# WasifurRahman/BERT_multimodal_transformer

Measured on AMD Instinct MI355X. Metric: train samples/sec MAG-BERT MOSI seq_len=50, higher is better.
Workload: dtype bf16; 1 GPU; MAG-BERT bert-base-uncased, MOSI dims (V=47, A=74), batch 48/GPU, seq_len 50, full optimizer step (fwd+MSE+bwd+HF-AdamW+schedule+zero_grad; inputs resident in HBM), dropout on, random-init weights; global_batch=48, seq_len=50, parallelism=dp1, step_call=mb_bert_train_step, hipGraph replay

## Files before the change

bert_multimodal_transformer_amd/_lib.py:

```python
import ctypes as C
import os

_HERE = os.path.dirname(os.path.abspath(__file__))
LIB_PATH = os.path.join(os.environ.get("MB_LIB_DIR") or os.path.join(_HERE, "lib"), "libmagbert_hip.so")

DT_F32, DT_BF16 = 0, 1
GEMM_NT, GEMM_NN, GEMM_TN = 0, 1, 2
EPI_BIAS, EPI_BIAS_GELU, EPI_BIAS_DROP_RES, EPI_ADD_RES, EPI_DGELU, EPI_ACCUM_F32, EPI_BIAS_F32 = range(7)
EPI_BIAS_RELU, EPI_BIAS_SWISH, EPI_BIAS_GELU_NEW, EPI_BIAS_MISH = 7, 8, 9, 10
ACT_GELU, ACT_RELU, ACT_SWISH, ACT_GELU_NEW, ACT_MISH = range(5)
ACTIVATIONS = {"gelu": ACT_GELU, "relu": ACT_RELU, "swish": ACT_SWISH, "silu": ACT_SWISH, "gelu_new": ACT_GELU_NEW, "mish": ACT_MISH}
ACT_EPILOGUE = {ACT_GELU: EPI_BIAS_GELU, ACT_RELU: EPI_BIAS_RELU, ACT_SWISH: EPI_BIAS_SWISH, ACT_GELU_NEW: EPI_BIAS_GELU_NEW,
                ACT_MISH: EPI_BIAS_MISH}


def activation_code(name, field):
    if isinstance(name, str) and name in ACTIVATIONS:
        return ACTIVATIONS[name]
    raise NotImplementedError("%s=%r: the feed-forward activations built are %s (and silu = swish)"
                              % (field, name, ", ".join(n for n in ACTIVATIONS if n != "silu")))


class DropKey(C.Structure):
    _fields_ = [("k0", C.c_uint32), ("k1", C.c_uint32), ("thresh", C.c_uint32), ("scale", C.c_float)]


class BertEngineConfig(C.Structure):
    _fields_ = [("vocab_size", C.c_int), ("hidden_size", C.c_int), ("num_layers", C.c_int), ("num_heads", C.c_int),
                ("intermediate_size", C.c_int), ("max_position", C.c_int), ("type_vocab", C.c_int),
                ("num_labels", C.c_int), ("visual_dim", C.c_int), ("acoustic_dim", C.c_int), ("pad_token_id", C.c_int),
                ("layer_norm_eps", C.c_float), ("mag_layer_norm_eps", C.c_float), ("beta_shift", C.c_float),
                ("hidden_dropout", C.c_float), ("attn_dropout", C.c_float), ("mag_dropout", C.c_float),
                ("dtype", C.c_int), ("max_batch", C.c_int), ("max_seq", C.c_int), ("injection_index", C.c_int),
                ("hidden_act", C.c_int)]
    POSITIONAL = tuple(n for n, _ in _fields_ if n != "injection_index") + ("injection_index",)

    def __init__(self, *args, **kw):
        if len(args) > len(self.POSITIONAL):
            raise TypeError("too many initializers")
        super().__init__()
        for name, value in zip(self.POSITIONAL, args):
            setattr(self, name, value)
        for name, value in kw.items():
            if name not in self.POSITIONAL:
                raise TypeError("BertEngineConfig has no field %r" % name)
            setattr(self, name, value)


class XlnetEngineConfig(C.Structure):
    _fields_ = [("vocab_size", C.c_int), ("d_model", C.c_int), ("n_layer", C.c_int), ("n_head", C.c_int), ("d_inner", C.c_int),
                ("num_labels", C.c_int), ("visual_dim", C.c_int), ("acoustic_dim", C.c_int), ("injection_index", C.c_int),
                ("layer_norm_eps", C.c_float), ("mag_layer_norm_eps", C.c_float), ("beta_shift", C.c_float),
                ("dropout", C.c_float), ("summary_last_dropout", C.c_float), ("mag_dropout", C.c_float),
                ("dtype", C.c_int), ("max_batch", C.c_int), ("max_seq", C.c_int), ("ff_activation", C.c_int)]


_vp, _i, _f, _sz, _u64, _u32 = C.c_void_p, C.c_int, C.c_float, C.c_size_t, C.c_uint64, C.c_uint32
_dk = C.POINTER(DropKey)

PROTOTYPES = {
    "mb_error_string": (C.c_char_p, [_i]),
    "mb_version": (_i, []),
    "mb_make_dropkey": (None, [_u64, _u64, _u32, _f, _dk]),
    "mb_gemm": (_i, [_i, _i, _i, _i, _i, _i, _vp, _i, _vp, _i, _vp, _i, _vp, _vp, _vp, _vp, _i, _f, _dk, _i, _i, _vp]),
    "mb_gemm_grouped_wgrad": (_i, [_i, _i, _vp, _vp, _i, _vp, _vp, _vp, _vp, _vp, _vp, _i, _vp]),
    "mb_narrow": (_i, [_i, _vp, _vp, _sz, _vp]),
    "mb_widen": (_i, [_i, _vp, _vp, _sz, _vp]),
    "mb_layernorm_forward": (_i, [_i, _vp, _vp, _vp, _f, _vp, _vp, _vp, _i, _i, _dk, _vp]),
    "mb_layernorm_backward": (_i, [_i, _vp, _vp, _vp, _vp, _vp, _vp, _vp, _vp, _vp, _vp, _i, _i, _dk, _dk, _vp]),
    "mb_embed_forward": (_i, [_i, _vp, _vp, _vp, _vp, _vp, _vp, _vp, _f, _vp, _vp, _vp, _i, _i, _i, _dk, _vp]),
    "mb_embed_backward": (_i, [_i, _vp, _vp, _vp, _vp, _vp, _vp, _vp, _vp, _vp, _vp, _vp, _vp, _vp, _vp, _vp, _i, _i, _i,
                               _i, _dk, _vp]),
    "mb_attention_forward": (_i, [_i, _vp, _vp, _vp, _i, _i, _i, _dk, _vp]),
    "mb_attention_backward": (_i, [_i, _vp, _vp, _vp, _vp, _i, _i, _i, _dk, _vp]),
    "mb_attention_resident_forward": (_i, [_i, _vp, _vp, _vp, _i, _i, _i, _dk, _vp, _vp, _vp]),
    "mb_attention_resident_backward": (_i, [_i, _vp, _vp, _vp, _vp, _vp, _i, _i, _i, _dk, _vp, _vp]),
    "mb_attention_tiled_stats_bytes": (_sz, [_i, _i, _i]),
    "mb_attention_tiled_forward": (_i, [_i, _vp, _vp, _vp, _vp, _i, _i, _i, _dk, _vp, _vp, _vp]),
    "mb_attention_tiled_backward": (_i, [_i, _vp, _vp, _vp, _vp, _vp, _vp, _vp, _i, _i, _i, _dk, _vp, _vp]),
    "mb_mag_workspace_bytes": (_sz, [_i, _i, _i, _i, _i]),
    "mb_mag_forward": (_i, [_i] + [_vp] * 13 + [_f, _dk, _vp, _vp, _i, _i, _i, _i, _vp]),
    "mb_mag_backward": (_i, [_i] + [_vp] * 11 + [_f, _dk] + [_vp] * 14 + [_i, _i, _i, _i, _vp]),
    "mb_adamw_step": (_i, [_vp, _vp, _vp, _vp, _vp, _sz, _sz, _sz, _sz, _f, _f, _f, _f, _f, _i, _i, _f, _i, _vp]),
    "mb_bert_create": (_i, [C.POINTER(BertEngineConfig), C.POINTER(_vp)]),
    "mb_bert_destroy": (None, [_vp]),
    "mb_bert_num_tensors": (_i, [_vp]),
    "mb_bert_tensor_info": (_i, [_vp, _i, C.c_char_p, _i, C.POINTER(_sz), C.POINTER(_sz), C.POINTER(_i),
                                 C.POINTER(C.c_int64), C.POINTER(_i)]),
    "mb_bert_param_count": (_sz, [_vp]),
    "mb_bert_decay_count": (_sz, [_vp]),
    "mb_bert_shadow_range": (None, [_vp, C.POINTER(_sz), C.POINTER(_sz)]),
    "mb_bert_workspace_bytes": (_sz, [_vp]),
    "mb_bert_bind": (_i, [_vp, _vp, _vp, _vp, _vp, _sz]),
    "mb_bert_sync_weights": (_i, [_vp, _vp]),
    "mb_bert_forward": (_i, [_vp, _vp, _vp, _vp, _vp, _vp, _vp, _i, _i, _i, _u64, _u64, _vp, _vp, _vp, _vp]),
    "mb_bert_backward": (_i, [_vp, _vp, _vp, _f, _i, _i, _vp]),
    "mb_bert_sequence_output": (_vp, [_vp]),
    "mb_bert_pooled_output": (_vp, [_vp]),
    "mb_bert_hidden_state": (_vp, [_vp, _i]),
    "mb_bert_set_attention_output": (_i, [_vp, _vp]),
    "mb_debug_gemm_ex": (_i, [_i, _i, _i, _i, _i, _i, _vp, _i, _vp, _i, _vp, _i, _vp, _vp, _vp, _vp, _i, _f, _dk, _i, _i,
                              _i, _sz, _i, _i, _vp, _i, _vp, _vp, _vp, _vp, _vp, _sz, _i, _i, _f, _f, _f, _f, _f, _i, _i, _f, _vp,
                              C.POINTER(_i), _vp]),
    "mb_debug_gemm_grouped_ex": (_i, [_i, _i, _vp, _vp, _i, _vp, _vp, _vp, _vp, _vp, _vp, _vp, _vp, _i, _i, _vp, _vp, _vp, _vp, _vp,
                                      _sz, _i, _i, _f, _f, _f, _f, _f, _i, _i, _f, _vp, _vp]),
    "mb_debug_gemm_last_kernel": (_i, [C.c_char_p, _i]),
    "mb_debug_gemm_trace": (_i, [_vp, _i]),
    "mb_debug_attention_trace": (_i, [_vp, _i]),
    "mb_xlnet_attention_probs": (_vp, [_vp, _i, C.POINTER(_i)]),
    "mb_xlnet_attention_probs_into": (_i, [_vp, _i, _vp, _vp]),
    "mb_xlnet_attention_tiled_stats_bytes": (_sz, [_i, _i, _i]),
    "mb_xlnet_attention_tiled_scratch_bytes": (_sz, [_i, _i, _i, _i]),
    "mb_xlnet_attention_tiled_forward": (_i, [_i] + [_vp] * 10 + [_i, _i, _i, _dk, _vp, _vp, _i, _vp, _vp]),
    "mb_xlnet_attention_tiled_backward": (_i, [_i] + [_vp] * 19 + [_i, _i, _i, _dk, _vp, _vp, _vp]),
    "mb_xlnet_attention_forward": (_i, [_i] + [_vp] * 11 + [_i, _i, _i, _dk, _vp, _vp, _i, _vp]),
    "mb_xlnet_attention_backward": (_i, [_i] + [_vp] * 20 + [_i, _i, _i, _dk, _vp, _vp, _vp]),
    "mb_xlnet_set_head_mask": (_i, [_vp, _vp]),
    "mb_xlnet_set_perm_mask": (_i, [_vp, _vp]),
    "mb_xlnet_set_mems": (_i, [_vp, _vp, _i]),
    "mb_xlnet_query_stream_scratch_bytes": (_sz, [_vp, _i, _i, _i]),
    "mb_xlnet_query_stream_state_bytes": (_sz, [_vp, _i, _i]),
    "mb_xlnet_query_stream": (_i, [_vp, _vp, _i, _vp, _sz, _vp, _vp]),
    "mb_bert_mark_grads_zero": (_i, [_vp, _i]),
    "mb_xlnet_mark_grads_zero": (_i, [_vp, _i]),
    "mb_bert_distrust_word_stamps": (_i, [_vp]),
    "mb_bert_word_skip_updates": (_sz, [_vp]),
    "mb_bert_materialize_grads": (_i, [_vp, _vp]),
    "mb_xlnet_materialize_grads": (_i, [_vp, _vp]),
    "mb_bert_grads_stale": (_i, [_vp]),
    "mb_xlnet_grads_stale": (_i, [_vp]),
    "mb_bert_set_head_mask": (_i, [_vp, _vp]),
    "mb_bert_set_inputs_embeds": (_i, [_vp, _vp]),
    "mb_bert_set_position_ids": (_i, [_vp, _vp]),
    "mb_bert_inputs_embeds_grad": (_vp, [_vp]),
    "mb_bert_backward_outputs": (_i, [_vp, _vp, _vp, _vp]),
    "mb_bert_stage_grad_ranges": (_i, [_vp, _i, C.POINTER(_sz), C.POINTER(_sz), _i]),
    "mb_bert_train_step": (_i, [_vp, _vp, _vp, _vp, _vp, _vp, _vp, _i, _i, _u64, _u64, _vp, _vp, _vp, _vp, _vp, _f, _f, _f, _f, _f,
                                _i, _i, _f, _f, _i, _vp]),
    "mb_bert_stage_forward": (_i, [_vp, _vp, _vp, _vp, _vp, _vp, _vp, _i, _i, _u64, _u64, _vp, _vp, _vp, _i, _vp]),
    "mb_bert_stage_backward": (_i, [_vp, _f, _i, _i, _vp]),
    "mb_bert_staged_input_ids": (_vp, [_vp]),
    "mb_bert_load_batch": (_i, [_vp, _vp, _vp, _vp, _vp, _vp, _vp, _i, _i, C.POINTER(_vp), _vp]),
    "mb_bert_graph_stats": (_i, [_vp, C.POINTER(_sz), C.POINTER(_sz)]),
    "mb_bert_set_profiling": (_i, [_vp, _i]),
    "mb_bert_profile_wgrad_us": (_i, [_vp, C.POINTER(_f)]),
    "mb_bert_profile_adamw_us": (_i, [_vp, C.POINTER(_f)]),
    "mb_xlnet_set_inputs_embeds": (_i, [_vp, _vp]),
    "mb_xlnet_inputs_embeds_grad": (_vp, [_vp]),
    "mb_xlnet_model_output": (_vp, [_vp, _vp]),
    "mb_xlnet_backward_outputs": (_i, [_vp, _vp, _vp]),
    "mb_xlnet_set_profiling": (_i, [_vp, _i]),
    "mb_xlnet_profile_wgrad_us": (_i, [_vp, C.POINTER(_f)]),
    "mb_xlnet_profile_adamw_us": (_i, [_vp, C.POINTER(_f)]),
    "mb_xlnet_create": (_i, [C.POINTER(XlnetEngineConfig), C.POINTER(_vp)]),
    "mb_xlnet_destroy": (None, [_vp]),
    "mb_xlnet_num_tensors": (_i, [_vp]),
    "mb_xlnet_tensor_info": (_i, [_vp, _i, C.c_char_p, _i, C.POINTER(_sz), C.POINTER(_sz), C.POINTER(_i),
                                  C.POINTER(C.c_int64), C.POINTER(_i)]),
    "mb_xlnet_param_count": (_sz, [_vp]),
    "mb_xlnet_decay_count": (_sz, [_vp]),
    "mb_xlnet_shadow_range": (None, [_vp, C.POINTER(_sz), C.POINTER(_sz)]),
    "mb_xlnet_workspace_bytes": (_sz, [_vp]),
    "mb_xlnet_bind": (_i, [_vp, _vp, _vp, _vp, _vp, _sz]),
    "mb_xlnet_sync_weights": (_i, [_vp, _vp]),
    "mb_xlnet_forward": (_i, [_vp, _vp, _vp, _vp, _vp, _vp, _vp, _i, _i, _i, _u64, _u64, _vp, _vp, _vp, _vp]),
    "mb_xlnet_backward": (_i, [_vp, _vp, _vp, _f, _i, _i, _vp]),
    "mb_xlnet_sequence_output": (_vp, [_vp]),
    "mb_xlnet_hidden_state": (_vp, [_vp, _i]),
    "mb_xlnet_train_step": (_i, [_vp, _vp, _vp, _vp, _vp, _vp, _vp, _i, _i, _u64, _u64, _vp, _vp, _vp, _vp, _vp, _f, _f, _f, _f, _f,
                                 _i, _i, _f, _f, _i, _vp]),
    "mb_xlnet_load_batch": (_i, [_vp, _vp, _vp, _vp, _vp, _vp, _vp, _i, _i, C.POINTER(_vp), _vp]),
    "mb_xlnet_graph_stats": (_i, [_vp, C.POINTER(_sz), C.POINTER(_sz)]),
    "mb_xlnet_trainable_count": (_sz, [_vp]),
    "mb_bert_set_update_map": (_i, [_vp, _i, _i, _vp, _vp]),
    "mb_bert_set_update_decay": (_i, [_vp, _i, _vp]),
    "mb_bert_set_update_values": (_i, [_vp, _i, _vp, _vp, _vp, _vp, _vp, _vp]),
    "mb_bert_update_stats": (_i, [_vp, C.POINTER(_sz), C.POINTER(_sz), C.POINTER(_i)]),
    "mb_bert_set_update_frozen": (_i, [_vp, _i, _vp]),
    "mb_bert_freeze_stats": (_i, [_vp, C.POINTER(_sz), C.POINTER(_i), C.POINTER(_i)]),
    "mb_xlnet_set_update_frozen": (_i, [_vp, _i, _vp]),
    "mb_xlnet_freeze_stats": (_i, [_vp, C.POINTER(_sz), C.POINTER(_i), C.POINTER(_i)]),
    "mb_xlnet_set_update_map": (_i, [_vp, _i, _i, _vp, _vp]),
    "mb_xlnet_set_update_decay": (_i, [_vp, _i, _vp]),
    "mb_xlnet_set_update_values": (_i, [_vp, _i, _vp, _vp, _vp, _vp, _vp, _vp]),
    "mb_xlnet_update_stats": (_i, [_vp, C.POINTER(_sz), C.POINTER(_sz), C.POINTER(_i)]),
    "mb_grad_clip_scratch_bytes": (_sz, [_sz]),
    "mb_grad_clip_coef": (_i, [_vp, _sz, _f, _f, _vp, _vp, _vp]),
    "mb_bert_set_grad_clip": (_i, [_vp, _f]),
    "mb_bert_grad_clip_stats": (_i, [_vp, C.POINTER(_f), C.POINTER(_f), _vp]),
    "mb_xlnet_set_grad_clip": (_i, [_vp, _f]),
    "mb_xlnet_grad_clip_stats": (_i, [_vp, C.POINTER(_f), C.POINTER(_f), _vp]),
    "mb_xlnet_stage_grad_ranges": (_i, [_vp, _i, C.POINTER(_sz), C.POINTER(_sz), _i]),
    "mb_comm_unique_id": (_i, [_vp]),
    "mb_comm_create_rccl": (_i, [_vp, _i, _i, C.POINTER(_vp)]),
    "mb_comm_create_callbacks": (_i, [_i, _i, _vp, _vp, _vp, C.POINTER(_vp)]),
    "mb_comm_destroy": (None, [_vp]),
    "mb_comm_rank": (_i, [_vp]),
    "mb_comm_world": (_i, [_vp]),
    "mb_comm_stream": (_vp, [_vp]),
    "mb_comm_scratch_bytes": (_sz, [_i, _i, _sz, _i, _i, _i]),
    "mb_comm_bind_scratch": (_i, [_vp, _vp, _sz, _i, _sz, _i, _i, _i]),
    "mb_comm_all_reduce": (_i, [_vp, _vp, _sz, _vp]),
    "mb_comm_exchange_rows": (_i, [_vp, _vp, _vp, _i, _vp]),
    "mb_comm_set_row_exchange": (_i, [_vp, _i]),
    "mb_comm_set_sharding": (_i, [_vp, _i]),
    "mb_comm_sharding": (_i, [_vp]),
    "mb_comm_join": (_i, [_vp, _vp]),
    "mb_comm_gather_shards": (_i, [_vp, _vp, _i, _vp]),
    "mb_comm_shard_slices": (_i, [_vp, C.POINTER(_sz), _i]),
    "mb_comm_set_timing": (_i, [_vp, _i]),
    "mb_comm_exposed_ms": (_i, [_vp, C.POINTER(_f)]),
    "mb_comm_stats": (_i, [_vp, C.POINTER(_sz), C.POINTER(_sz)]),
    "mb_comm_last_error": (C.c_char_p, []),
    "mb_bert_train_step_dp": (_i, [_vp, _vp, _vp, _vp, _vp, _vp, _vp, _i, _i, _u64, _u64, _vp, _vp, _vp, _vp, _vp, _f, _f, _f, _f, _f,
                                   _i, _i, _f, _f, _i, _vp, _vp]),
    "mb_xlnet_train_step_dp": (_i, [_vp, _vp, _vp, _vp, _vp, _vp, _vp, _i, _i, _u64, _u64, _vp, _vp, _vp, _vp, _vp, _f, _f, _f, _f, _f,
                                    _i, _i, _f, _f, _i, _vp, _vp]),
}

ALL_REDUCE_CB = C.CFUNCTYPE(C.c_int, C.c_void_p, C.c_void_p, C.c_size_t, C.c_int, C.c_void_p)
ALL_GATHER_CB = C.CFUNCTYPE(C.c_int, C.c_void_p, C.c_void_p, C.c_size_t, C.c_void_p)

_lib = None


class MagbertError(RuntimeError):
    pass


def lib():
    global _lib
    if _lib is None:
        if not os.path.exists(LIB_PATH):
            raise MagbertError(
                "libmagbert_hip.so not found at %s -- build it with `python -c 'import __graft_entry__ as g; g.build()'` "
                "(hipcc --offload-arch=gfx950).  There is no CPU fallback." % LIB_PATH)
        h = C.CDLL(LIB_PATH)
        for name, (res, args) in PROTOTYPES.items():
            fn = getattr(h, name)
            fn.restype = res
            fn.argtypes = args
        _lib = h
    return _lib


def check(code):
    if code != 0:
        msg = lib().mb_error_string(code).decode()
        if code == 1005 or 2000 <= code < 2100:
            msg += ": " + (lib().mb_comm_last_error() or b"").decode()
        raise MagbertError("%s (code %d)" % (msg, code))


def ptr(t):
    return None if t is None else C.c_void_p(t.data_ptr())


def make_dropkey(seed, step, site, p):
    k = DropKey()
    lib().mb_make_dropkey(int(seed) & (2**64 - 1), int(step), int(site), float(p), C.byref(k))
    return k


def no_drop():
    return DropKey(0, 0, 0, 1.0)
```

bert_multimodal_transformer_amd/csrc/engine.hip:

```cpp
#include "dp_step.h"

struct LayerOff { size_t wqkv, wo, w1, w2, bqkv, bo, ln1w, ln1b, b1, b2, ln2w, ln2b; };
struct LayerWs { size_t qkv, ctx, s1, st1, y1, u, g, s2, st2, stats; };

struct mb_bert_engine : StepMixin {
    mb_bert_config c;
    std::vector<TensorInfo> tensors;
    std::vector<LayerOff> lo;
    size_t word, pos, type, emb_lnw, emb_lnb, wp, bp, wc, bc;
    size_t mag_whv, mag_wha, mag_wv, mag_wa, mag_bhv, mag_bha, mag_bv, mag_ba, mag_lnw, mag_lnb;
    size_t n_params, n_decay, sh_begin, sh_end;
    size_t n_update_end() const { return n_params; }
    int n_layers() const { return c.num_layers; }
    size_t layer_begin(int l) const { return lo[l].wqkv; }
    size_t layers_end() const { return wp; }
    int width() const { return c.hidden_size; }
    size_t layer_end(int l) const { return l + 1 < c.num_layers ? lo[l + 1].wqkv : wp; }
    bool embed_all_frozen() const { return range_frozen(word, mag_whv) && range_frozen(emb_lnw, bp); }
    WordSkip word_skip(char* w) const {
        if (!(stamp_off != 0 && stamp_enable && idcnt_enable)) return {};
        return WordSkip{stamp_table(w), stamp_state(w), word, word + (size_t)c.vocab_size * c.hidden_size, (uint32_t)c.hidden_size};
    }
    MagWs mw;
    size_t ws_mag, ws_emb, ws_emb_st, ws_head_z, ws_head_pooled, ws_logits;
    std::vector<size_t> ws_x;
    size_t ws_pre = 0;
    int mag_nblk = 0;
    std::vector<LayerWs> lw;
    size_t ws_ds[2], ws_dzd[2], ws_ds2[2], ws_dzd2[2], ws_du[2], ws_dqkv[2];
    size_t ws_dxa, ws_dxb, ws_dctx, ws_dsum, ws_dz, ws_lnp_a, ws_lnp_b;
    size_t lnp_stride = 0;
    int lnp_nblk = 0;
    size_t ws_ids, ws_seg, ws_mask, ws_labels;
    size_t ws_bytes;
    float* P = nullptr; float* G = nullptr; char* SH = nullptr; char* ws = nullptr;
    const int64_t* ids = nullptr; const int64_t* seg = nullptr; const int64_t* mask = nullptr;
    int B = 0, L = 0, training = 0;
    int padT = -1;
    int prefetch = 1;
    int pf_qkv = 0;
    RideOpts ride_opts;
    int ride_blocks = 0;
    float* ride_m = nullptr; float* ride_v = nullptr;
    size_t ride_cursor = 0;
    long ride_params = 0;
    int group_wgrad = 256;
    bool grouped = false;
    float* attn_out = nullptr;
    const float* head_mask = nullptr;
    const float* emb_in = nullptr;
    const int64_t* pos_ids = nullptr;
    bool ran_forward = false;

    bool ws_zeroed = false;
    uint64_t seed = 0, step = 0;
    float* logits = nullptr;

    size_t add(const std::string& name, std::vector<int64_t> shape, int decay, size_t& cursor) {
        TensorInfo t;
        t.name = name; t.ndim = (int)shape.size(); t.decay = decay; t.numel = 1;
        for (int i = 0; i < 4; ++i) t.shape[i] = i < t.ndim ? shape[i] : 1;
        for (auto s : shape) t.numel *= (size_t)s;
        t.off = cursor;
        cursor = align_up(cursor + t.numel, 64);
        tensors.push_back(t);
        return t.off;
    }
    const void* W(size_t off) const {
        return c.dtype == DT_BF16 ? (const void*)(SH + off * 2) : (const void*)(P + off);
    }
    DropKey key(uint32_t site, float p) const { return step_key(ws, training != 0, seed, step, site, p); }
    float* attn_stats(const LayerWs& w) const { return c.max_seq > 128 ? (float*)(ws + w.stats) : nullptr; }
};

static void build_layout(mb_bert_engine* e) {
    const mb_bert_config& c = e->c;
    const int64_t H = c.hidden_size, I = c.intermediate_size, V = c.visual_dim, A = c.acoustic_dim;
    size_t cur = 0;
    e->lo.resize(c.num_layers);
    char buf[128];
    auto nm = [&](int l, const char* s) { snprintf(buf, sizeof buf, "bert.encoder.layer.%d.%s", l, s); return std::string(buf); };
    e->sh_begin = 0;
    for (int l = 0; l < c.num_layers; ++l) {
        LayerOff& o = e->lo[l];
        o.wqkv = e->add(nm(l, "attention.self.query.weight"), {H, H}, 1, cur);
        e->add(nm(l, "attention.self.key.weight"), {H, H}, 1, cur);
        e->add(nm(l, "attention.self.value.weight"), {H, H}, 1, cur);
        o.wo = e->add(nm(l, "attention.output.dense.weight"), {H, H}, 1, cur);
        o.w1 = e->add(nm(l, "intermediate.dense.weight"), {I, H}, 1, cur);
        o.w2 = e->add(nm(l, "output.dense.weight"), {H, I}, 1, cur);
    }
    e->wp = e->add("bert.pooler.dense.weight", {H, H}, 1, cur);
    e->sh_end = cur;
    e->word = e->add("bert.embeddings.word_embeddings.weight", {c.vocab_size, H}, 1, cur);
    e->pos = e->add("bert.embeddings.position_embeddings.weight", {c.max_position, H}, 1, cur);
    e->type = e->add("bert.embeddings.token_type_embeddings.weight", {c.type_vocab, H}, 1, cur);
    e->mag_whv = e->add("bert.MAG.W_hv.weight", {H, V + H}, 1, cur);
    e->mag_wha = e->add("bert.MAG.W_ha.weight", {H, A + H}, 1, cur);
    e->mag_wv = e->add("bert.MAG.W_v.weight", {H, V}, 1, cur);
    e->mag_wa = e->add("bert.MAG.W_a.weight", {H, A}, 1, cur);
    e->wc = e->add("classifier.weight", {c.num_labels, H}, 1, cur);
    e->n_decay = cur;
    for (int l = 0; l < c.num_layers; ++l) {
        LayerOff& o = e->lo[l];
        o.bqkv = e->add(nm(l, "attention.self.query.bias"), {H}, 0, cur);
        e->add(nm(l, "attention.self.key.bias"), {H}, 0, cur);
        e->add(nm(l, "attention.self.value.bias"), {H}, 0, cur);
        o.bo = e->add(nm(l, "attention.output.dense.bias"), {H}, 0, cur);
        o.ln1w = e->add(nm(l, "attention.output.LayerNorm.weight"), {H}, 0, cur);
        o.ln1b = e->add(nm(l, "attention.output.LayerNorm.bias"), {H}, 0, cur);
        o.b1 = e->add(nm(l, "intermediate.dense.bias"), {I}, 0, cur);
        o.b2 = e->add(nm(l, "output.dense.bias"), {H}, 0, cur);
        o.ln2w = e->add(nm(l, "output.LayerNorm.weight"), {H}, 0, cur);
        o.ln2b = e->add(nm(l, "output.LayerNorm.bias"), {H}, 0, cur);
    }
    e->emb_lnw = e->add("bert.embeddings.LayerNorm.weight", {H}, 0, cur);
    e->emb_lnb = e->add("bert.embeddings.LayerNorm.bias", {H}, 0, cur);
    e->bp = e->add("bert.pooler.dense.bias", {H}, 0, cur);
    e->mag_bhv = e->add("bert.MAG.W_hv.bias", {H}, 0, cur);
    e->mag_bha = e->add("bert.MAG.W_ha.bias", {H}, 0, cur);
    e->mag_bv = e->add("bert.MAG.W_v.bias", {H}, 0, cur);
    e->mag_ba = e->add("bert.MAG.W_a.bias", {H}, 0, cur);
    e->mag_lnw = e->add("bert.MAG.LayerNorm.weight", {H}, 0, cur);
    e->mag_lnb = e->add("bert.MAG.LayerNorm.bias", {H}, 0, cur);
    e->bc = e->add("classifier.bias", {c.num_labels}, 0, cur);
    e->n_params = cur;

    const size_t es = esize(c.dtype);
    const size_t T = align_up((size_t)c.max_batch * c.max_seq, 64);
    Carver w;
    e->mw.init(c.dtype, (int)T, (int)H, (int)V, (int)A);
    e->ws_mag = w.take(e->mw.bytes);
    e->pk_vis = e->ws_mag + e->mw.vp; e->pk_aco = e->ws_mag + e->mw.ap; e->pk_Vp = e->mw.Vp; e->pk_Ap = e->mw.Ap; e->pk_dtype = c.dtype;
    e->ws_emb = w.take(T * H * es);
    e->ws_emb_st = w.take(2 * T * 4);
    e->ws_x.resize(c.num_layers + 1);
    for (int l = 0; l <= c.num_layers; ++l) e->ws_x[l] = w.take(T * H * es);
    e->ws_pre = c.injection_index >= 1 ? w.take(T * H * es) : 0;
    e->lw.resize(c.num_layers);
    for (int l = 0; l < c.num_layers; ++l) {
        LayerWs& x = e->lw[l];
        x.qkv = w.take(T * 3 * H * es); x.ctx = w.take(T * H * es); x.s1 = w.take(T * H * es); x.st1 = w.take(2 * T * 4);
        x.y1 = w.take(T * H * es); x.u = w.take(T * I * es); x.g = w.take(T * I * es); x.s2 = w.take(T * H * es);
        x.st2 = w.take(2 * T * 4);
        x.stats = c.max_seq > 128 ? w.take(tiled_stats_floats(c.max_batch, c.max_seq, c.num_heads) * 4) : 0;
    }
    e->ws_head_z = w.take((size_t)c.max_batch * H * 4);
    e->ws_head_pooled = w.take((size_t)c.max_batch * H * 4);
    e->ws_logits = w.take((size_t)c.max_batch * c.num_labels * 4);
    e->ws_dxa = w.take(T * H * es); e->ws_dxb = w.take(T * H * es);
    for (int k = 0; k < 2; ++k) {
        e->ws_ds[k] = w.take(T * H * es); e->ws_dzd[k] = w.take(T * H * es); e->ws_ds2[k] = w.take(T * H * es);
        e->ws_dzd2[k] = w.take(T * H * es); e->ws_du[k] = w.take(T * I * es); e->ws_dqkv[k] = w.take(T * 3 * H * es);
    }
    e->ws_dctx = w.take(T * H * es); e->ws_dsum = w.take(T * H * 4); e->ws_dz = w.take((size_t)c.max_batch * H * es);
    e->lnp_stride = ln_partials_floats((int)T, (int)H);
    {
        const size_t emb = (size_t)c.max_seq * ((c.max_batch + 7) / 8) * 3 * H;
        if (emb > e->lnp_stride) e->lnp_stride = emb;
    }
    e->ws_lnp_a = w.take(e->lnp_stride * 4 * (c.num_layers + 2)); e->ws_lnp_b = w.take(e->lnp_stride * 4 * (c.num_layers + 2));
    e->carve_step(w, T, (int)V, (int)A, c.max_batch, c.num_labels, SITE_LAYER0 + 4 * c.num_layers);
    e->idcnt_off = w.take((size_t)c.vocab_size * 4);
    e->idcnt_enable = env_on("MB_EMBED_UNIQUE", true);
    e->stamp_rows = (size_t)c.vocab_size;
    e->stamp_off = w.take(((size_t)c.vocab_size + 2) * 4);
    e->stamp_enable = env_on("MB_ADAMW_SKIP_ZERO_ROWS", true);
    e->one_sweep = env_on("MB_ADAMW_ONE_SWEEP", true);
    if (e->deterministic) {
        e->det_begin = e->wp; e->det_end = e->n_params;
        e->ws_det = w.take((e->det_end - e->det_begin) * sizeof(long long));
    }
    e->ws_bytes = w.off;
}

static int prepare_pass(mb_bert_engine* e, int T, hipStream_t st) {
    const mb_bert_config& c = e->c;
    const int H = c.hidden_size, I = c.intermediate_size, dt = c.dtype;
    char* ws = e->ws;
    const int Tp = (int)align_up((size_t)T, 64);
    if (!e->ws_zeroed) { CK((int)hipMemsetAsync(ws, 0, e->ws_bytes, st)); e->ws_zeroed = true; e->padT = T; }
    if (e->padT != T && Tp > T) {
        const size_t es = esize(dt);
        auto zp = [&](size_t off, size_t cols) {
            return (int)hipMemsetAsync(ws + off + (size_t)T * cols * es, 0, (size_t)(Tp - T) * cols * es, st);
        };
        CK(zp(e->ws_emb, H));
        if (c.injection_index >= 1) CK(zp(e->ws_pre, H));
        CK(mag_clear_pad_rows(dt, ws + e->ws_mag, e->mw, T, H, st));
        for (int k = 0; k < 2; ++k) {
            CK(zp(e->ws_ds[k], H)); CK(zp(e->ws_dzd[k], H)); CK(zp(e->ws_ds2[k], H)); CK(zp(e->ws_dzd2[k], H));
            CK(zp(e->ws_du[k], I)); CK(zp(e->ws_dqkv[k], 3 * H));
        }
        for (int l = 0; l <= c.num_layers; ++l) CK(zp(e->ws_x[l], H));
        for (int l = 0; l < c.num_layers; ++l) { CK(zp(e->lw[l].ctx, H)); CK(zp(e->lw[l].y1, H)); CK(zp(e->lw[l].g, I)); }
    }
    e->padT = T;
    return MB_OK;
}

static AdamArgs adam_scalars(float lr, float beta1, float beta2, float eps, float weight_decay, int step, int correct_bias, float grad_scale) {
    AdamArgs a;
    a.lr = lr; a.beta1 = beta1; a.beta2 = beta2; a.eps = eps; a.weight_decay = weight_decay; a.grad_scale = grad_scale;
    double ss = lr;
    if (correct_bias) ss = (double)lr * sqrt(1.0 - pow((double)beta2, (double)step)) / (1.0 - pow((double)beta1, (double)step));
    a.step_size = (float)ss;
    return a;
}
static int debug_ride(AdamRide& r, float* p, float* g, float* m, float* v, void* shadow, size_t n4, int blocks, int zero_grad, const AdamArgs& a,
                      void* adam_dev, hipStream_t st) {
    r = AdamRide{};
    if (blocks == 0) return MB_OK;
    if (blocks < 0 || !p || !g || !m || !v || !adam_dev) return MB_ERR_ARG;
    if ((((uintptr_t)p | (uintptr_t)g | (uintptr_t)m | (uintptr_t)v) & 15) || ((uintptr_t)shadow & 7) || ((uintptr_t)adam_dev & 3)) return MB_ERR_SHAPE;
    CK((int)hipMemcpyAsync(adam_dev, &a, sizeof(AdamArgs), hipMemcpyHostToDevice, st));
    CK((int)hipStreamSynchronize(st));
    r.p = p; r.g = g; r.m = m; r.v = v; r.shadow = (bf16*)shadow; r.n4 = n4; r.dyn = (const AdamArgs*)adam_dev; r.blocks = blocks;
    r.zero_grad = zero_grad;
    return MB_OK;
}

extern "C" {

const char* mb_error_string(int code) {
    switch (code) {
        case MB_OK: return "ok";
        case MB_ERR_SHAPE: return "magbert: unsupported shape or alignment";
        case MB_ERR_MODE: return "magbert: unsupported layout/epilogue combination";
        case MB_ERR_DTYPE: return "magbert: unsupported dtype";
        case MB_ERR_ARG: return "magbert: invalid argument";
        case MB_ERR_COMM: return "magbert: gradient exchange unavailable (mb_comm_last_error())";
        default:
            if (code >= 2000 && code < 2100) return "magbert: RCCL call failed (mb_comm_last_error())"; return hipGetErrorString((hipError_t)code);
    }
}
int mb_version(void) { return 100; }

void mb_make_dropkey(uint64_t seed, uint64_t step, uint32_t site, float p, mb_dropkey* out) {
    DropKey k = make_key(seed, step, site, p);
    out->k0 = k.k0; out->k1 = k.k1; out->thresh = k.thresh; out->scale = k.scale;
}

static int abi_epilogue(int& epilogue, int layout, GemmArgs& a) {
    if (epilogue < MB_EPI_RELU || epilogue > MB_EPI_MISH) return MB_OK;
    if (layout != GEMM_NT) return MB_ERR_MODE;
    a.act = ACT_RELU + (epilogue - MB_EPI_RELU);
    epilogue = EPI_BIAS_ACT;
    return MB_OK;
}

int mb_gemm(int dtype, int layout, int epilogue, int M, int N, int K, const void* A, int lda, const void* B, int ldb,
            void* C, int ldc, void* C2, float* Cf, const float* bias, const void* R, int ldr, float alpha,
            const mb_dropkey* drop, int splits, int tile, void* stream) {
    GemmArgs a = {};
    a.A = A; a.B = B; a.M = M; a.N = N; a.K = K; a.lda = lda; a.ldb = ldb; a.C = C; a.ldc = ldc; a.C2 = C2; a.Cf = Cf;
    a.bias = bias; a.R = R; a.ldr = ldr; a.alpha = alpha; a.drop = dk(drop); a.kchunk = K; a.colsum = nullptr;
    if (epilogue == EPI_DGELU) { a.colsum = Cf; a.Cf = nullptr; }
    if (int e = abi_epilogue(epilogue, layout, a)) return e;
    return gemm_launch(dtype, layout, epilogue, a, splits, tile, (hipStream_t)stream);
}

int mb_debug_gemm_ex(int dtype, int layout, int epilogue, int M, int N, int K, const void* A, int lda, const void* B, int ldb,
                     void* C, int ldc, void* C2, float* Cf, const float* bias, const void* R, int ldr, float alpha,
                     const mb_dropkey* drop, int splits, int tile, int bseg, size_t bseg_stride, int cvalid, int overwrite,
                     long long* colsum_shadow, int fold, float* rp, float* rg, float* rm, float* rv, void* rshadow, size_t n4, int blocks,
                     int zero_grad, float lr, float beta1, float beta2, float eps, float weight_decay, int step, int correct_bias,
                     float grad_scale, void* adam_dev, int* ride_tiles, void* stream) {
    hipStream_t st = (hipStream_t)stream;
    GemmArgs a = {};
    a.A = A; a.B = B; a.M = M; a.N = N; a.K = K; a.lda = lda; a.ldb = ldb; a.C = C; a.ldc = ldc; a.C2 = C2; a.Cf = Cf;
    a.bias = bias; a.R = R; a.ldr = ldr; a.alpha = alpha; a.drop = dk(drop); a.kchunk = K; a.colsum = nullptr;
    if (epilogue == EPI_DGELU) { a.colsum = Cf; a.Cf = nullptr; }
    if (int e = abi_epilogue(epilogue, layout, a)) return e;
    a.bseg = bseg; a.bseg_stride = bseg_stride; a.cvalid = cvalid; a.overwrite = overwrite;
    if (colsum_shadow) {
        if (!a.colsum) return MB_ERR_ARG;
        a.acc = GradAcc{colsum_shadow, a.colsum};
    }
    if (ride_tiles) *ride_tiles = 0;
    AdamRide ride;
    if (int e = debug_ride(ride, rp, rg, rm, rv, rshadow, n4, blocks, zero_grad,
                           adam_scalars(lr, beta1, beta2, eps, weight_decay, step, correct_bias, grad_scale), adam_dev, st)) return e;
    if (ride.blocks > 0) {
        if (layout != GEMM_NN || splits > 1 || tile != 0) return MB_ERR_MODE;
        int per_cu = 0;
        const int tiles = gemm_nn_ride_tiles(dtype, epilogue, a, &per_cu);
        if (ride_tiles) *ride_tiles = tiles;
        CK(gemm_nn_ride_launch(dtype, epilogue, a, ride, st));
    } else {
        CK(gemm_launch(dtype, layout, epilogue, a, splits, tile, st));
    }
    if (colsum_shadow && fold) CK(grad_fold(a.acc, a.colsum, 0, (size_t)N, st));
    return MB_OK;
}

int mb_debug_gemm_grouped_ex(int dtype, int count, const int* M, const int* N, int K, const void* const* dY, const int* ldy,
                             const void* const* X, const int* ldx, float* const* dW, const int* ldw, const int* cvalid,
                             const int* overwrite, int tile, int stages, float* rp, float* rg, float* rm, float* rv, void* rshadow,
                             size_t n4, int blocks, int zero_grad, float lr, float beta1, float beta2, float eps, float weight_decay,
                             int step, int correct_bias, float grad_scale, void* adam_dev, void* stream) {
    hipStream_t st = (hipStream_t)stream;
    if (count < 1 || count > MB_MAX_GROUP || !M || !N || !dY || !X || !dW || !ldy || !ldx || !ldw) return MB_ERR_ARG;
    if (stages != 0 && stages != 4 && stages != 5) return MB_ERR_ARG;
    GemmArgs g[MB_MAX_GROUP];
    for (int i = 0; i < count; ++i) {
        g[i] = wgrad_args(M[i], N[i], K, dY[i], ldy[i], X[i], ldx[i], dW[i], ldw[i]);
        g[i].cvalid = cvalid ? cvalid[i] : 0;
        g[i].overwrite = overwrite ? overwrite[i] : 0;
    }
    if (!gemm_grouped_tn_ok(dtype, g, count, tile)) return MB_ERR_SHAPE;
    AdamRide ride;
    if (int e = debug_ride(ride, rp, rg, rm, rv, rshadow, n4, blocks, zero_grad,
                           adam_scalars(lr, beta1, beta2, eps, weight_decay, step, correct_bias, grad_scale), adam_dev, st)) return e;
    return gemm_grouped_tn_launch(dtype, g, count, tile, st, stages, ride.blocks > 0 ? &ride : nullptr);
}

int mb_debug_gemm_last_kernel(char* out, int cap) { return gemm_last_kernel(out, cap); }

int mb_debug_gemm_trace(unsigned long long* host_out, int max_blocks) { return gemm_trace_fetch(host_out, max_blocks); }
int mb_debug_attention_trace(unsigned long long* host_out, int max_blocks) { return attention_trace_fetch(host_out, max_blocks); }
int mb_gemm_grouped_wgrad(int dtype, int count, const int* M, const int* N, int K, const void* const* dY, const int* ldy,
                          const void* const* X, const int* ldx, float* const* dW, const int* ldw, int tile, void* stream) {
    if (count < 1 || count > MB_MAX_GROUP || !M || !N || !dY || !X || !dW || !ldy || !ldx || !ldw) return MB_ERR_ARG;
    GemmArgs g[MB_MAX_GROUP];
    for (int i = 0; i < count; ++i) g[i] = wgrad_args(M[i], N[i], K, dY[i], ldy[i], X[i], ldx[i], dW[i], ldw[i]);
    if (!gemm_grouped_tn_ok(dtype, g, count, tile)) return MB_ERR_SHAPE;
    return gemm_grouped_tn_launch(dtype, g, count, tile, (hipStream_t)stream);
}

int mb_narrow(int dtype, const float* src, void* dst, size_t n, void* stream) {
    if (!src || !dst) return MB_ERR_ARG;
    if (n % 4) return MB_ERR_SHAPE;
    return convert(dtype, src, dst, n, (hipStream_t)stream);
}
int mb_widen(int dtype, const void* src, float* dst, size_t n, void* stream) {
    if (!src || !dst) return MB_ERR_ARG;
    return widen(dtype, src, dst, n, (hipStream_t)stream);
}

int mb_layernorm_forward(int dtype, const void* x, const float* gamma, const float* beta, float eps, void* y, float* mean,
                         float* rstd, int rows, int H, const mb_dropkey* drop, void* stream) {
    return ln_forward(dtype, x, gamma, beta, eps, y, mean, rstd, rows, H, dk(drop), (hipStream_t)stream);
}
int mb_layernorm_backward(int dtype, const void* dy, const void* x, const float* gamma, const float* mean,
                          const float* rstd, void* dx, void* dx_drop, float* dgamma, float* dbeta, float* dbias, int rows,
                          int H, const mb_dropkey* drop_out, const mb_dropkey* drop_in, void* stream) {
    return ln_backward(dtype, dy, x, gamma, mean, rstd, dx, dx_drop, dgamma, dbeta, dbias, rows, H, dk(drop_out),
                       dk(drop_in), (hipStream_t)stream);
}
int mb_embed_forward(int dtype, const int64_t* ids, const int64_t* seg, const float* word, const float* pos,
                     const float* type, const float* gamma, const float* beta, float eps, void* out, float* mean,
                     float* rstd, int B, int L, int H, const mb_dropkey* drop, void* stream) {
    return embed_ln_forward(dtype, ids, seg, word, pos, type, gamma, beta, eps, out, mean, rstd, B, L, H, dk(drop),
                            (hipStream_t)stream);
}
int mb_embed_backward(int dtype, const void* dout, const int64_t* ids, const int64_t* seg, const float* word,
                      const float* pos, const float* type, const float* gamma, const float* mean, const float* rstd,
                      float* dsum_ws, float* dword, float* dpos, float* dtype_, float* dgamma, float* dbeta, int B, int L,
                      int H, int pad_id, const mb_dropkey* drop, void* stream) {
    return embed_ln_backward(dtype, dout, ids, seg, word, pos, type, gamma, mean, rstd, dsum_ws, dword, dpos, dtype_,
                             dgamma, dbeta, B, L, H, pad_id, dk(drop), (hipStream_t)stream);
}
int mb_attention_forward(int dtype, const void* qkv, const int64_t* mask, void* ctx, int B, int L, int nh,
                         const mb_dropkey* drop, void* stream) {
    if (L > 128) return MB_ERR_SHAPE;
    return attention_forward(dtype, qkv, mask, ctx, B, L, nh, dk(drop), (hipStream_t)stream);
}
int mb_attention_backward(int dtype, const void* qkv, const int64_t* mask, const void* dctx, void* dqkv, int B, int L,
                          int nh, const mb_dropkey* drop, void* stream) {
    static float* trace_dbias = nullptr;
    static int trace_on = -1;
    if (trace_on < 0) {
        const char* v = getenv("MB_ATTN_TRACE");
        trace_on = v ? atoi(v) : 0;
        if (trace_on && (hipMalloc(&trace_dbias, (size_t)3 * 64 * 64 * sizeof(float)) != hipSuccess ||
                         hipMemset(trace_dbias, 0, (size_t)3 * 64 * 64 * sizeof(float)) != hipSuccess)) trace_dbias = nullptr;
    }
    if (L > 128) return MB_ERR_SHAPE;
    return attention_backward(dtype, qkv, mask, nullptr, dctx, dqkv, (trace_on && nh <= 64) ? trace_dbias : nullptr, B, L, nh, dk(drop),
                              (hipStream_t)stream);
}
static int resident_check(int dtype, int B, int L, int nh, const DropKey& drop) {
    if (B < 1 || L < 1 || L > 128 || nh < 1 || (int64_t)B * nh > 0x7fffffff) return MB_ERR_SHAPE;
    if (drop.thresh != 0u && (uint64_t)B * nh * L * L >= ((uint64_t)1 << 32)) return MB_ERR_SHAPE;
    if (dtype != DT_BF16 && dtype != DT_F32) return MB_ERR_DTYPE;
    return MB_OK;
}
int mb_attention_resident_forward(int dtype, const void* qkv, const int64_t* mask, void* ctx, int B, int L, int nh,
                                  const mb_dropkey* drop, const float* head_scale, float* probs, void* stream) {
    if (int e = resident_check(dtype, B, L, nh, dk(drop))) return e;
    if (!qkv || !mask || !ctx) return MB_ERR_ARG;
    return attention_forward(dtype, qkv, mask, ctx, B, L, nh, dk(drop), (hipStream_t)stream, probs, head_scale);
}
int mb_attention_resident_backward(int dtype, const void* qkv, const int64_t* mask, const void* dctx, void* dqkv, float* dbias, int B,
                                   int L, int nh, const mb_dropkey* drop, const float* head_scale, void* stream) {
    if (int e = resident_check(dtype, B, L, nh, dk(drop))) return e;
    if (!qkv || !mask || !dctx || !dqkv) return MB_ERR_ARG;
    return attention_backward(dtype, qkv, mask, nullptr, dctx, dqkv, dbias, B, L, nh, dk(drop), (hipStream_t)stream, head_scale);
}
size_t mb_attention_tiled_stats_bytes(int B, int L, int nh) {
    return (B < 1 || L < 1 || nh < 1) ? 0 : tiled_stats_floats(B, L, nh) * sizeof(float);
}
int mb_attention_tiled_forward(int dtype, const void* qkv, const int64_t* mask, void* ctx, float* stats, int B, int L, int nh,
                               const mb_dropkey* drop, const float* head_scale, float* probs, void* stream) {
    return attention_tiled_forward(dtype, qkv, mask, ctx, stats, B, L, nh, dk(drop), (hipStream_t)stream, probs, head_scale);
}
int mb_attention_tiled_backward(int dtype, const void* qkv, const int64_t* mask, const void* ctx, const void* dctx, float* stats,
                                void* dqkv, float* dbias, int B, int L, int nh, const mb_dropkey* drop, const float* head_scale,
                                void* stream) {
    return attention_tiled_backward(dtype, qkv, mask, ctx, dctx, stats, dqkv, dbias, B, L, nh, dk(drop), (hipStream_t)stream, head_scale);
}

size_t mb_mag_workspace_bytes(int dtype, int T, int H, int V, int A) {
    MagWs w;
    w.init(dtype, T, H, V, A);
    return w.bytes;
}
int mb_mag_forward(int dtype, const void* text, const float* visual, const float* acoustic, const float* W_hv,
                   const float* b_hv, const float* W_ha, const float* b_ha, const float* W_v, const float* b_v,
                   const float* W_a, const float* b_a, const float* ln_w, const float* ln_b, float beta_shift,
                   const mb_dropkey* drop, void* out, void* ws, int T, int H, int V, int A, void* stream) {
    if (H % 256 || H < 256 || H > 1024 || V < 1 || A < 1) return MB_ERR_SHAPE;
    MagWs w;
    w.init(dtype, T, H, V, A);
    return mag_fwd_impl(dtype, text, visual, acoustic, W_hv, b_hv, W_ha, b_ha, W_v, b_v, W_a, b_a, ln_w, ln_b, 1e-5f,
                        beta_shift, dk(drop), out, (char*)ws, w, T, H, V, A, true, (hipStream_t)stream);
}
int mb_mag_backward(int dtype, const void* d_out, const void* text, const float* W_hv, const float* b_hv,
                    const float* W_ha, const float* b_ha, const float* W_v, const float* b_v, const float* W_a,
                    const float* b_a, const float* ln_w, float beta_shift, const mb_dropkey* drop, void* ws, void* d_text,
                    float* d_visual, float* d_acoustic, float* dW_hv, float* db_hv, float* dW_ha, float* db_ha,
                    float* dW_v, float* db_v, float* dW_a, float* db_a, float* dln_w, float* dln_b, int T, int H, int V,
                    int A, void* stream) {
    (void)W_hv; (void)W_ha; (void)W_v; (void)W_a;
    if (H % 256 || H < 256 || H > 1024) return MB_ERR_SHAPE;
    MagWs w;
    w.init(dtype, T, H, V, A);
    return mag_bwd_impl(dtype, d_out, text, b_hv, b_ha, b_v, b_a, ln_w, beta_shift, dk(drop), (char*)ws, w, d_text,
                        d_visual, d_acoustic, dW_hv, db_hv, dW_ha, db_ha, dW_v, db_v, dW_a, db_a, dln_w, dln_b, T, H, V, A,
                        false, (hipStream_t)stream);
}

int mb_adamw_step(float* p, float* g, float* m, float* v, void* shadow, size_t n, size_t n_decay, size_t sh_begin,
                  size_t sh_end, float lr, float beta1, float beta2, float eps, float weight_decay, int step,
                  int correct_bias, float grad_scale, int zero_grad, void* stream) {
    const AdamArgs a = adam_scalars(lr, beta1, beta2, eps, weight_decay, step, correct_bias, grad_scale);
    return adamw_step(p, g, m, v, shadow, n, n_decay, sh_begin, sh_end, a, zero_grad, (hipStream_t)stream);
}

size_t mb_grad_clip_scratch_bytes(size_t n) { return (size_t)grad_norm_blocks(n) * sizeof(double); }
int mb_grad_clip_coef(const float* g, size_t n, float max_norm, float grad_scale, void* scratch, float* out2, void* stream) {
    if (!scratch || !out2) return MB_ERR_ARG;
    CK(grad_sumsq(g, n, (double*)scratch, (hipStream_t)stream));
    return grad_clip_finalize((const double*)scratch, grad_norm_blocks(n), nullptr, max_norm, grad_scale, out2, ClipTables{}, (hipStream_t)stream);
}

int mb_bert_create(const mb_bert_config* cfg, mb_bert_engine** out) {
    if (!cfg || !out) return MB_ERR_ARG;
    const int Hc = cfg->hidden_size;
    if ((Hc != 256 && Hc != 512 && Hc != 768 && Hc != 1024) || cfg->num_heads * 64 != Hc || cfg->num_layers < 1) return MB_ERR_SHAPE;
    if (cfg->intermediate_size % 128 || cfg->max_seq < 1 || cfg->max_seq > 512 || cfg->max_batch < 1) return MB_ERR_SHAPE;
    if (cfg->max_seq > cfg->max_position || cfg->num_labels < 1) return MB_ERR_SHAPE;
    if (cfg->dtype != DT_F32 && cfg->dtype != DT_BF16) return MB_ERR_DTYPE;
    if (cfg->hidden_act < ACT_GELU || cfg->hidden_act > ACT_MISH) return MB_ERR_ARG;
    if (cfg->injection_index < 0 || cfg->injection_index >= cfg->num_layers) return MB_ERR_ARG;
    mb_bert_engine* e = new mb_bert_engine();
    e->c = *cfg;
    e->read_env();
    e->ride_opts.read_env();
    e->group_wgrad = env_int("MB_GROUP_WGRAD", e->group_wgrad);
    e->ride_blocks = env_int("MB_ADAMW_RIDE_BLOCKS", e->ride_blocks);
    e->ride_params = env_long("MB_ADAMW_RIDE_PARAMS", e->ride_params);
    e->prefetch = env_int("MB_PREFETCH", e->prefetch);
    e->pf_qkv = env_int("MB_PF_QKV", e->pf_qkv);
    if (e->group_wgrad == 256 && (cfg->dtype != DT_BF16 || cfg->hidden_size % 256 != 0 || cfg->intermediate_size % 256 != 0)) e->group_wgrad = 128;
    e->grouped = (e->group_wgrad == 64 || e->group_wgrad == 128 || e->group_wgrad == 256) && cfg->hidden_size % e->group_wgrad == 0 &&
                 cfg->intermediate_size % e->group_wgrad == 0;

    build_layout(e);
    e->ow_covers = e->grouped;
    e->stale_begin = e->lo[0].wqkv; e->stale_end = e->wp;
    *out = e;
    return MB_OK;
}
void mb_bert_destroy(mb_bert_engine* e) {
    if (!e) return;
    e->destroy_prof();
    e->drop_graphs();
    e->free_class_table();
    e->free_clip_buf();
    delete e;
}
int mb_bert_num_tensors(const mb_bert_engine* e) { return (int)e->tensors.size(); }
int mb_bert_tensor_info(const mb_bert_engine* e, int i, char* name, int name_cap, size_t* offset, size_t* numel, int* ndim,
                        int64_t* shape4, int* decay) {
    if (i < 0 || i >= (int)e->tensors.size()) return MB_ERR_ARG;
    const TensorInfo& t = e->tensors[i];
    if (name && name_cap > 0) { strncpy(name, t.name.c_str(), name_cap - 1); name[name_cap - 1] = 0; }
    if (offset) *offset = t.off;
    if (numel) *numel = t.numel;
    if (ndim) *ndim = t.ndim;
    if (shape4) for (int k = 0; k < 4; ++k) shape4[k] = t.shape[k];
    if (decay) *decay = t.decay;
    return MB_OK;
}
size_t mb_bert_param_count(const mb_bert_engine* e) { return e->n_params; }
size_t mb_bert_decay_count(const mb_bert_engine* e) { return e->n_decay; }
void mb_bert_shadow_range(const mb_bert_engine* e, size_t* b, size_t* en) { *b = e->sh_begin; *en = e->sh_end; }
size_t mb_bert_workspace_bytes(const mb_bert_engine* e) { return e->ws_bytes; }

int mb_bert_bind(mb_bert_engine* e, float* params, float* grads, void* shadow, void* workspace, size_t ws_bytes) {
    if (!params || !workspace || ws_bytes < e->ws_bytes) return MB_ERR_ARG;
    if (e->c.dtype == DT_BF16 && !shadow) return MB_ERR_ARG;
    e->P = params; e->G = grads; e->SH = (char*)shadow; e->ws = (char*)workspace;
    e->grads_zero = false;
    e->frz_dirty = true;
    e->stamp_live = e->word_zero = false; e->sweep_no = 1;
    e->ws_zeroed = false; e->padT = -1;
    e->drop_graphs();
    char* mws = e->ws + e->ws_mag;
    e->pkw = {e->P + e->mag_whv, e->P + e->mag_wha, e->P + e->mag_wv, e->P + e->mag_wa, mws + e->mw.We, mws + e->mw.Wv, mws + e->mw.Wa,
              MagDims{0, e->c.hidden_size, e->c.visual_dim, e->c.acoustic_dim, e->mw.Vp, e->mw.Ap}, e->c.dtype};
    return MB_OK;
}

int mb_bert_sync_weights(mb_bert_engine* e, void* stream) {
    hipStream_t st = (hipStream_t)stream;
    if (!e->P) return MB_ERR_ARG;
    if (e->c.dtype == DT_BF16)
        CK(convert(DT_BF16, e->P + e->sh_begin, e->SH + e->sh_begin * 2, e->sh_end - e->sh_begin, st));
    const mb_bert_config& c = e->c;
    MagDims d = {0, c.hidden_size, c.visual_dim, c.acoustic_dim, e->mw.Vp, e->mw.Ap};
    char* mws = e->ws + e->ws_mag;
    CK(mag_pack_weights(c.dtype, e->P + e->mag_whv, e->P + e->mag_wha, e->P + e->mag_wv, e->P + e->mag_wa, mws + e->mw.We,
                        mws + e->mw.Wv, mws + e->mw.Wa, d, st));
    return MB_OK;
}

static int bert_forward_range(mb_bert_engine* e, const int64_t* input_ids, const float* visual, const float* acoustic,
                              const int64_t* attention_mask, const int64_t* token_type_ids, const float* labels, int B, int L,
                              int training, uint64_t seed, uint64_t step, float* logits, float* loss, float* loss_run, void* stream,
                              int l0, int l1, bool first, bool last) {
    hipStream_t st = (hipStream_t)stream;
    const mb_bert_config& c = e->c;
    if (!e->P || !e->ws) return MB_ERR_ARG;
    if (B < 1 || B > c.max_batch || L < 1 || L > c.max_seq) return MB_ERR_SHAPE;
    if ((!input_ids && !e->emb_in) || !visual || !acoustic || !attention_mask || !token_type_ids || !logits) return MB_ERR_ARG;
    const int dt = c.dtype, H = c.hidden_size, I = c.intermediate_size, T = B * L, nh = c.num_heads;
    if (e->emb_in) input_ids = nullptr;
    e->ids = input_ids; e->seg = token_type_ids; e->mask = attention_mask; e->ran_forward = true;
    e->B = B; e->L = L; e->training = training; e->seed = seed; e->step = step; e->logits = logits;
    float* P = e->P;
    char* ws = e->ws;
    if (first && !e->capturing) CK(prepare_pass(e, T, st));
    const int inj = c.injection_index;
    if (first) CK(embed_ln_forward(dt, input_ids, token_type_ids, e->emb_in ? e->emb_in : P + e->word, P + e->pos, P + e->type, P + e->emb_lnw, P + e->emb_lnb,
                        c.layer_norm_eps, ws + (inj >= 1 ? e->ws_x[0] : e->ws_emb), (float*)(ws + e->ws_emb_st), (float*)(ws + e->ws_emb_st) + T, B, L,
                        H, e->key(SITE_EMB, c.hidden_dropout), st, e->pos_ids));
    auto mag = [&](const char* text, char* out) -> int {
        return mag_fwd_impl(dt, text, visual, acoustic, P + e->mag_whv, P + e->mag_bhv, P + e->mag_wha, P + e->mag_bha,
                            P + e->mag_wv, P + e->mag_bv, P + e->mag_wa, P + e->mag_ba, P + e->mag_lnw, P + e->mag_lnb,
                            c.mag_layer_norm_eps, c.beta_shift, e->key(SITE_MAG, c.mag_dropout), out, ws + e->ws_mag,
                            e->mw, T, H, c.visual_dim, c.acoustic_dim, !(e->in_step && e->packed_w), st, true, e->in_step && e->packed);
    };
    if (first && inj == 0) CK(mag(ws + e->ws_emb, ws + e->ws_x[0]));
    for (int l = l0; l < l1; ++l) {
        const LayerOff& o = e->lo[l];
        const LayerWs& w = e->lw[l];
        if (l == inj && inj >= 1) CK(mag(ws + e->ws_pre, ws + e->ws_x[l]));
        const char* x = ws + e->ws_x[l];
        CK(gemm(dt, GEMM_NT, EPI_BIAS, T, 3 * H, H, x, H, e->W(o.wqkv), H, ws + w.qkv, 3 * H, nullptr, nullptr, P + o.bqkv,
                nullptr, 0, kNoDrop, 1, 0, st));
        CK(attention_forward(dt, ws + w.qkv, attention_mask, ws + w.ctx, B, L, nh,
                             e->key(SITE_LAYER0 + 4 * l + 0, c.attn_dropout), st,
                             e->attn_out ? e->attn_out + (size_t)l * B * nh * L * L : nullptr,
                             e->head_mask ? e->head_mask + (size_t)l * nh : nullptr, e->attn_stats(w)));
        CK(gemm(dt, GEMM_NT, EPI_BIAS_DROP_RES, T, H, H, ws + w.ctx, H, e->W(o.wo), H, ws + w.s1, H, nullptr, nullptr,
                P + o.bo, x, H, e->key(SITE_LAYER0 + 4 * l + 1, c.hidden_dropout), 1, 0, st));
        const size_t wes = dt == DT_BF16 ? 2 : 4;
        const Prefetch pf1 = {e->prefetch ? e->W(o.w1) : nullptr, (size_t)2 * I * H * wes, nullptr};
        const Prefetch pf2 = {(e->prefetch && l + 1 < c.num_layers && (l + 1 < l1 || last)) ? e->W(e->lo[l + 1].wqkv) : nullptr, (size_t)4 * H * H * wes, nullptr};
        CK(ln_forward(dt, ws + w.s1, P + o.ln1w, P + o.ln1b, c.layer_norm_eps, ws + w.y1, (float*)(ws + w.st1),
                      (float*)(ws + w.st1) + T, T, H, kNoDrop, st, pf1));
        CK(gemm(dt, GEMM_NT, ffn_act_mode(c.hidden_act), T, I, H, ws + w.y1, H, e->W(o.w1), H, ws + w.u, I, ws + w.g, nullptr, P + o.b1,
                nullptr, 0, kNoDrop, 1, 0, st, 0, 0, GradAcc{}, c.hidden_act));
        CK(gemm(dt, GEMM_NT, EPI_BIAS_DROP_RES, T, H, I, ws + w.g, I, e->W(o.w2), I, ws + w.s2, H, nullptr, nullptr,
                P + o.b2, ws + w.y1, H, e->key(SITE_LAYER0 + 4 * l + 2, c.hidden_dropout), 1, 0, st));
        CK(ln_forward(dt, ws + w.s2, P + o.ln2w, P + o.ln2b, c.layer_norm_eps, ws + (l + 1 == inj ? e->ws_pre : e->ws_x[l + 1]), (float*)(ws + w.st2),
                      (float*)(ws + w.st2) + T, T, H, kNoDrop, st, pf2));
    }
    if (!last) return MB_OK;
    float* z = (float*)(ws + e->ws_head_z);
    CK(gemm(dt, GEMM_NT, EPI_BIAS_F32, B, H, H, ws + e->ws_x[c.num_layers], L * H, e->W(e->wp), H, nullptr, H, nullptr, z,
            P + e->bp, nullptr, 0, kNoDrop, 1, 64, st));
    if (loss && !(e->in_step && e->loss_cleared)) CK(zero_fill(loss, 4, st));
    CK(head_forward(z, P + e->wc, P + e->bc, labels, (float*)(ws + e->ws_head_pooled), logits, loss, loss_run, B, H,
                    c.num_labels, e->key(SITE_HEAD, c.hidden_dropout), st));
    return MB_OK;
}

int mb_bert_forward(mb_bert_engine* e, const int64_t* input_ids, const float* visual, const float* acoustic,
                    const int64_t* attention_mask, const int64_t* token_type_ids, const float* labels, int B, int L,
                    int training, uint64_t seed, uint64_t step, float* logits, float* loss, float* loss_run, void* stream) {
    return bert_forward_range(e, input_ids, visual, acoustic, attention_mask, token_type_ids, labels, B, L, training, seed, step, logits,
                              loss, loss_run, stream, 0, e->c.num_layers, true, true);
}

int mb_bert_backward(mb_bert_engine* e, const float* dlogits, const float* labels, float loss_scale, int stage_begin,
                     int stage_end, void* stream) {
    hipStream_t st = (hipStream_t)stream;
    const mb_bert_config& c = e->c;
    if (!e->G || !e->ran_forward) return MB_ERR_ARG;
    if (!e->in_step) e->stamp_live = e->word_zero = false;
    const int dt = c.dtype, H = c.hidden_size, I = c.intermediate_size, B = e->B, L = e->L, T = B * L, nh = c.num_heads;
    const int NL = c.num_layers;
    const int Tk = (int)align_up((size_t)T, 64);
    auto take_ride = [&](int l, size_t budget, int blocks) -> AdamRide {
        AdamRide r = {};
        if (!e->ride_m || !e->ride_v || l + 1 >= e->c.num_layers || blocks < 8 || e->ride_cursor <= e->lo[l + 1].wqkv) return r;
        size_t floor = e->lo[l + 1].wqkv;
        const AdamArgs* dyn = e->adam_state(e->ws);
        if (e->n_classes > 0) {
            size_t sb = 0; int cl = 0;
            if (!e->ride_segment(e->ride_cursor, floor, &sb, &cl)) return r;
            floor = std::max(floor, sb); dyn = e->class_state(e->ws) + cl;
        }
        size_t take = std::min(e->ride_cursor - floor, budget) / 1024 * 1024;
        const size_t re = e->ride_cursor, rb = re - take;
        const bool sh_ok = e->c.dtype != DT_BF16 || (e->sh_begin <= rb && re <= e->sh_end);
        if (take == 0 || rb % 4 || !sh_ok) return r;
        const bool keep = e->keep_in_step() && e->stale_begin <= rb && re <= e->stale_end;
        r = AdamRide{e->P + rb, e->G + rb, e->ride_m + rb, e->ride_v + rb, e->c.dtype == DT_BF16 ? (bf16*)(e->SH + rb * 2) : nullptr,
                     take / 4, dyn, blocks / 8 * 8, keep ? 0 : 1};
        e->ride_cursor = rb;
        return r;
    };
    if (stage_begin < 0) stage_begin = 0;
    if (stage_end > NL + 2) stage_end = NL + 2;
    if (stage_begin == 0) CK(e->begin_backward_pass(e->G, st));
    float* P = e->P; float* G = e->G;
    char* ws = e->ws;
    const bool hd = e->training && c.hidden_dropout > 0.f;
    const GradAcc acc = e->acc_of(ws, G);
    for (int stage = stage_begin; stage < stage_end; ++stage) {
        if (stage == 0) {
            CK(head_backward(dt, dlogits, e->logits, labels, loss_scale, (const float*)(ws + e->ws_head_pooled), P + e->wc,
                             ws + e->ws_dz, G + e->wc, G + e->bc, B, H, c.num_labels, e->key(SITE_HEAD, c.hidden_dropout),
                             st, acc, G + e->bp, ws + e->ws_dxa, (size_t)T * H * esize(dt)));
            const char* xf = ws + e->ws_x[NL];
            CK(gemm(dt, GEMM_TN, EPI_ACCUM_F32, H, H, B, ws + e->ws_dz, H, xf, L * H, nullptr, H, nullptr, G + e->wp, nullptr,
                    nullptr, 0, kNoDrop, 1, 64, st));
            CK(gemm(dt, GEMM_NN, EPI_ADD_RES, B, H, H, ws + e->ws_dz, H, e->W(e->wp), H, ws + e->ws_dxa, L * H, nullptr,
                    nullptr, nullptr, nullptr, 0, kNoDrop, 1, 64, st));
        } else if (stage <= NL) {
            const int l = NL - stage;
            const LayerOff& o = e->lo[l];
            const LayerWs& w = e->lw[l];
            char* dx = ws + e->ws_dxa;
            char* dy1 = ws + e->ws_dxb;
            const int par = l & 1;
            char* dsA = ws + e->ws_ds[par];
            char* dzdA = hd ? ws + e->ws_dzd[par] : dsA;
            char* dsB = ws + e->ws_ds2[par];
            char* dzdB = hd ? ws + e->ws_dzd2[par] : dsB;
            char* du = ws + e->ws_du[par];
            char* dqkv = ws + e->ws_dqkv[par];
            int nblk = 0;
            float* lnp_a = (float*)(ws + e->ws_lnp_a) + (size_t)l * e->lnp_stride;
            float* lnp_b = (float*)(ws + e->ws_lnp_b) + (size_t)l * e->lnp_stride;
            const bool defer_ln = e->in_step && !e->stage_mode && NL + 2 <= MB_LN_MAX_LAYERS;
            CK(ln_backward_partials(dt, dx, ws + w.s2, P + o.ln2w, (const float*)(ws + w.st2), (const float*)(ws + w.st2) + T, dsA,
                                    hd ? dzdA : nullptr, lnp_a, &nblk, T, H, e->key(SITE_LAYER0 + 4 * l + 2, c.hidden_dropout), st,
                                    Prefetch{e->prefetch ? e->W(o.w1) : nullptr, (size_t)2 * I * H * (dt == DT_BF16 ? 2 : 4), nullptr}));
            GemmArgs wg[4] = {wgrad_args(H, I, Tk, dzdA, H, ws + w.g, I, G + o.w2, I),
                              wgrad_args(I, H, Tk, du, I, ws + w.y1, H, G + o.w1, H),
                              wgrad_args(H, H, Tk, dzdB, H, ws + w.ctx, H, G + o.wo, H),
                              wgrad_args(3 * H, H, Tk, dqkv, 3 * H, ws + e->ws_x[l], H, G + o.wqkv, H)};
            const bool grouped = e->grouped;
            const bool wfrozen = e->skipping() && e->unwritten(o.wqkv, e->layer_end(l));
            if (wfrozen) ++e->frz_wgrad_skipped;
            if (grouped)
                for (GemmArgs& a : wg) a.overwrite = e->ow_pass ? 1 : 0;
            auto dgrad_ride = [&](int mode, int Mo, int No, int Ko, const void* dY, int ldy, const void* Wt, int ldw, void* dX, int ldx, const void* R, int ldr,
                                  float* colsum) -> int {
                return dgrad_with_riders(dt, mode, Mo, No, Ko, dY, ldy, Wt, ldw, dX, ldx, R, ldr, colsum, kNoDrop, acc, st, grouped && e->ride_m != nullptr,
                                         e->ride_opts, e->cu_count(), [&](size_t budget, int blocks) { return take_ride(l, budget, blocks); });
            };
            int wtile = e->group_wgrad;
            if (grouped && wtile == 256 && !gemm_grouped_tn_ok(dt, wg, 4, 256)) wtile = 128;
            if (grouped && !gemm_grouped_tn_ok(dt, wg, 4, wtile)) return MB_ERR_SHAPE;
            if (!grouped && !wfrozen) CK(wgrad(dt, H, I, Tk, dzdA, H, ws + w.g, I, G + o.w2, I, st));
            CK(dgrad_ride(EPI_DGELU, T, I, H, dzdA, H, e->W(o.w2), I, du, I, ws + w.u, I, G + o.b1));
            if (!grouped && !wfrozen) CK(wgrad(dt, I, H, Tk, du, I, ws + w.y1, H, G + o.w1, H, st));
            CK(dgrad_ride(EPI_ADD_RES, T, H, I, du, I, e->W(o.w1), H, dy1, H, dsA, H, nullptr));
            Prefetch pf_attn = {e->prefetch ? e->W(o.wqkv) : nullptr, (size_t)4 * H * H * (dt == DT_BF16 ? 2 : 4), nullptr};
            if (e->prefetch && e->pf_qkv > 0) {
                const size_t es = dt == DT_BF16 ? 2 : 4, qb = (size_t)T * 3 * H * es;
                pf_attn.p2 = ws + w.qkv;
                pf_attn.bytes2 = (w.ctx - w.qkv) - qb <= 4096 ? (w.ctx - w.qkv) + (size_t)T * H * es : qb;
                pf_attn.stride2 = (uint32_t)e->pf_qkv;
            }
            CK(ln_backward_partials(dt, dy1, ws + w.s1, P + o.ln1w, (const float*)(ws + w.st1), (const float*)(ws + w.st1) + T, dsB,
                                    hd ? dzdB : nullptr, lnp_b, &nblk, T, H, e->key(SITE_LAYER0 + 4 * l + 1, c.hidden_dropout), st,
                                    pf_attn));
            if (!grouped && !wfrozen) CK(wgrad(dt, H, H, Tk, dzdB, H, ws + w.ctx, H, G + o.wo, H, st));
            e->lnp_nblk = nblk;
            if (!defer_ln) {
                float* const dst6[6] = {G + o.ln2w, G + o.ln2b, G + o.b2, G + o.ln1w, G + o.ln1b, G + o.bo};
                CK(ln_reduce_partials(lnp_a, lnp_b, nblk, H, dst6, st, acc));
            }
            CK(gemm(dt, GEMM_NN, EPI_ADD_RES, T, H, H, dzdB, H, e->W(o.wo), H, ws + e->ws_dctx, H, nullptr, nullptr, nullptr,
                    nullptr, 0, kNoDrop, 1, 0, st));
            AdamRide ra = {};
            if (e->ride_opts.attn && grouped && e->ride_m && L <= 128) {
                int free_slots = attention_backward_free_slots(dt, L, B * nh, e->cu_count());
                if (e->ride_opts.attn_blocks > 0 && free_slots > 0) free_slots = e->ride_opts.attn_blocks;
                const int blocks = std::min(free_slots, 2 * e->cu_count()) / 8 * 8;
                if (blocks >= 8) {
                    const size_t budget = e->ride_opts.attn_params > 0 ? (size_t)e->ride_opts.attn_params
                                                                  : (L > 64 ? (size_t)blocks * 20480 : (size_t)1650 * (size_t)T);
                    ra = take_ride(l, budget / 1024 * 1024, blocks);
                }
            }
            CK(attention_backward(dt, ws + w.qkv, e->mask, ws + w.ctx, ws + e->ws_dctx, dqkv, G + o.bqkv, B, L, nh,
                                  e->key(SITE_LAYER0 + 4 * l + 0, c.attn_dropout), st,
                                  e->head_mask ? e->head_mask + (size_t)l * nh : nullptr, acc, ra.blocks ? &ra : nullptr,
                                  e->attn_stats(w)));
            AdamRide ride = {};
            if (grouped && !wfrozen) {
                int tiles = 0;
                const int bm = wtile == 256 ? 256 : wtile, bn = wtile == 256 ? 128 : wtile;
                for (const GemmArgs& a : wg) tiles += (a.M / bm) * (a.N / bn);
                const int slots = e->cu_count() * (wtile == 256 ? 1 : wtile == 128 ? 2 : 0);
                const size_t budget = e->ride_params > 0 ? (size_t)e->ride_params : std::min((size_t)1000 * (size_t)Tk, (size_t)1100000 + (size_t)590 * (size_t)Tk);
                ride = take_ride(l, budget, e->ride_blocks > 0 ? e->ride_blocks : (slots - tiles) / 8 * 8);
            }
            if (grouped) {
                if (e->prof) CK((int)hipEventRecord(e->pev[2 * l], st));
                if (!wfrozen) CK(gemm_grouped_tn_launch(dt, wg, 4, wtile, st, 0, ride.blocks ? &ride : nullptr));
                if (e->prof) CK((int)hipEventRecord(e->pev[2 * l + 1], st));
            } else if (!wfrozen) {
                CK(wgrad(dt, 3 * H, H, Tk, dqkv, 3 * H, ws + e->ws_x[l], H, G + o.wqkv, H, st));
            }
            CK(dgrad_ride(EPI_ADD_RES, T, H, 3 * H, dqkv, 3 * H, e->W(o.wqkv), H, dx, H, dsB, H, nullptr));
            if (l == c.injection_index && l >= 1) {
                int mblk = 0;
                CK(mag_bwd_impl(dt, dx, ws + e->ws_pre, P + e->mag_bhv, P + e->mag_bha, P + e->mag_bv, P + e->mag_ba,
                                P + e->mag_lnw, c.beta_shift, e->key(SITE_MAG, c.mag_dropout), ws + e->ws_mag, e->mw, dx, nullptr,
                                nullptr, G + e->mag_whv, G + e->mag_bhv, G + e->mag_wha, G + e->mag_bha, G + e->mag_wv,
                                G + e->mag_bv, G + e->mag_wa, G + e->mag_ba, G + e->mag_lnw, G + e->mag_lnb, T, H, c.visual_dim,
                                c.acoustic_dim, true, st, acc, true, (float*)(ws + e->ws_lnp_a) + (size_t)NL * e->lnp_stride,
                                (float*)(ws + e->ws_lnp_b) + (size_t)NL * e->lnp_stride, &mblk, e->ow_pass));
                e->mag_nblk = mblk;
                if (!defer_ln) {
                    float* const m6[6] = {G + e->mag_bhv, G + e->mag_bha, G + e->mag_bv, G + e->mag_ba, G + e->mag_lnw, G + e->mag_lnb};
                    CK(ln_reduce_partials((const float*)(ws + e->ws_lnp_a) + (size_t)NL * e->lnp_stride,
                                          (const float*)(ws + e->ws_lnp_b) + (size_t)NL * e->lnp_stride, mblk, H, m6, st, acc));
                }
            }
        } else {
            const bool mag_here = c.injection_index == 0;
            char* dx = ws + e->ws_dxa;
            char* de = mag_here ? ws + e->ws_dxb : dx;
            const bool defer_ln = e->in_step && !e->stage_mode && NL + 2 <= MB_LN_MAX_LAYERS && NL > 0;
            float* mpa = (float*)(ws + e->ws_lnp_a) + (size_t)NL * e->lnp_stride;
            float* mpb = (float*)(ws + e->ws_lnp_b) + (size_t)NL * e->lnp_stride;
            int mblk = e->mag_nblk;
            if (mag_here)
            CK(mag_bwd_impl(dt, dx, ws + e->ws_emb, P + e->mag_bhv, P + e->mag_bha, P + e->mag_bv, P + e->mag_ba,
                            P + e->mag_lnw, c.beta_shift, e->key(SITE_MAG, c.mag_dropout), ws + e->ws_mag, e->mw, de, nullptr,
                            nullptr, G + e->mag_whv, G + e->mag_bhv, G + e->mag_wha, G + e->mag_bha, G + e->mag_wv,
                            G + e->mag_bv, G + e->mag_wa, G + e->mag_ba, G + e->mag_lnw, G + e->mag_lnb, T, H, c.visual_dim,
                            c.acoustic_dim, true, st, acc, true, mpa, mpb, &mblk, e->ow_pass));
            int eblk = 0;
            const bool word_frozen = e->skipping() && e->unwritten(e->word, e->pos);
            const bool emb_frozen = e->skipping() && e->unwritten(e->word, e->mag_whv) && e->unwritten(e->emb_lnw, e->bp);
            if (emb_frozen) e->frz_embed_skipped = 1;
            else
            CK(embed_ln_backward(dt, de, e->ids, e->seg, e->ids ? P + e->word : e->emb_in, P + e->pos, P + e->type, P + e->emb_lnw,
                                 (const float*)(ws + e->ws_emb_st), (const float*)(ws + e->ws_emb_st) + T,
                                 (float*)(ws + e->ws_dsum), (e->ids && !word_frozen) ? G + e->word : nullptr, G + e->pos, G + e->type, G + e->emb_lnw,
                                 G + e->emb_lnb, B, L, H, c.pad_token_id, e->key(SITE_EMB, c.hidden_dropout), st, e->pos_ids, acc,
                                 (float*)(ws + e->ws_lnp_a) + (size_t)(NL + 1) * e->lnp_stride, &eblk,
                                 (float*)(ws + e->ws_lnp_b) + (size_t)(NL + 1) * e->lnp_stride,
                                 (e->in_step && e->counted && e->ids && !e->emb_in) ? (int*)(ws + e->idcnt_off) : nullptr));
            {
                const int first = defer_ln ? 0 : NL;
                LnReduceDst dst = {};
                for (int k = first; k < NL; ++k) {
                    const LayerOff& ok = e->lo[k];
                    float* const d6[6] = {G + ok.ln2w, G + ok.ln2b, G + ok.b2, G + ok.ln1w, G + ok.ln1b, G + ok.bo};
                    for (int q = 0; q < 6; ++q) dst.d[k - first][q] = d6[q];
                }
                float* const m6[6] = {G + e->mag_bhv, G + e->mag_bha, G + e->mag_bv, G + e->mag_ba, G + e->mag_lnw, G + e->mag_lnb};
                if (mag_here || defer_ln) for (int q = 0; q < 6; ++q) dst.d[NL - first][q] = m6[q];
                dst.nblk[NL - first] = mblk; dst.nblk[NL + 1 - first] = eblk;
                if (!emb_frozen) { dst.d[NL + 1 - first][0] = G + e->emb_lnw; dst.d[NL + 1 - first][1] = G + e->emb_lnb; }
                if (e->pos_ids == nullptr && !emb_frozen) {
                    dst.d[NL + 1 - first][2] = G + e->type; dst.d[NL + 1 - first][3] = G + e->type + H;
                }
                CK(ln_reduce_partials_layers((const float*)(ws + e->ws_lnp_a) + (size_t)first * e->lnp_stride,
                                             (const float*)(ws + e->ws_lnp_b) + (size_t)first * e->lnp_stride, e->lnp_stride, NL + 2 - first,
                                             e->lnp_nblk, H, dst, st, acc));
            }
            CK(grad_fold(acc, G, e->det_begin, e->det_end, st));
        }
    }
    return MB_OK;
}


static int enqueue_step(mb_bert_engine* e, int B, int L, float* logits, float* loss, float* loss_run, float* m, float* v,
                        float loss_scale, hipStream_t st) {
    char* ws = e->ws;
    const int NL = e->c.num_layers;
    const float* lab = (const float*)(ws + e->ws_in_lab);
    float* keep_attn = e->attn_out;
    e->attn_out = nullptr;
    struct Restore { mb_bert_engine* e; float* p; ~Restore() { e->attn_out = p; } } restore{e, keep_attn};
    if (e->head_mask || e->emb_in || e->pos_ids) return MB_ERR_MODE;
    CK(mb_bert_forward(e, (const int64_t*)(ws + e->ws_in_ids), (const float*)(ws + e->ws_in_vis), (const float*)(ws + e->ws_in_aco),
                       (const int64_t*)(ws + e->ws_in_mask), (const int64_t*)(ws + e->ws_in_seg), lab, B, L, 1, 0, 0, logits, loss,
                       loss_run, st));
    const bool clip = e->clip_step && m && v;
    const bool ride = e->ride_opts.ride && m && v && e->grouped && NL > 1 && e->lo[0].wqkv == 0 && !e->prof &&
                      (e->group_wgrad == 128 || e->group_wgrad == 256) && !clip;
    e->ride_m = ride ? m : nullptr; e->ride_v = ride ? v : nullptr;
    e->ride_cursor = e->wp;
    e->begin_step_marks();
    if (e->skipping()) {
        for (int l = 0; l < NL; ++l) if (e->range_frozen(e->lo[l].wqkv, e->layer_end(l))) e->note_unwritten(e->lo[l].wqkv, e->layer_end(l));
        if (e->embed_all_frozen()) { e->note_unwritten(e->word, e->mag_whv); e->note_unwritten(e->emb_lnw, e->bp); }
        else if (e->range_frozen(e->word, e->pos)) e->note_unwritten(e->word, e->pos);
    }
    const int rb = mb_bert_backward(e, nullptr, lab, loss_scale, 0, NL + 2, st);
    e->ride_m = e->ride_v = nullptr;
    CK(rb);
    if (m && v) CK(enqueue_update(e, m, v, ride, clip, st));
    return MB_OK;
}

int mb_bert_set_update_map(mb_bert_engine* e, int n_classes, int n_segments, const size_t* boundaries, const int* classes) {
    if (!e) return MB_ERR_ARG;
    return e->set_update_map(e->tensors, e->n_params, n_classes, n_segments, boundaries, classes);
}
int mb_bert_set_update_decay(mb_bert_engine* e, int n_segments, const uint8_t* no_decay) {
    if (!e) return MB_ERR_ARG;
    return e->set_update_decay(n_segments, no_decay);
}
int mb_bert_set_update_values(mb_bert_engine* e, int n_classes, const float* lr, const float* beta1, const float* beta2, const float* eps,
                              const float* weight_decay, const int* correct_bias) {
    if (!e) return MB_ERR_ARG;
    return e->set_update_values(n_classes, lr, beta1, beta2, eps, weight_decay, correct_bias);
}
int mb_bert_set_update_frozen(mb_bert_engine* e, int n_segments, const uint8_t* frozen) {
    if (!e) return MB_ERR_ARG;
    return e->set_update_frozen(n_segments, frozen);
}
int mb_bert_freeze_stats(const mb_bert_engine* e, size_t* frozen_elems, int* wgrad_launches_skipped, int* embed_skipped) {
    if (!e) return MB_ERR_ARG;
    return e->freeze_stats(frozen_elems, wgrad_launches_skipped, embed_skipped);
}
int mb_bert_update_stats(const mb_bert_engine* e, size_t* ridden, size_t* swept, int* segments) {
    if (!e) return MB_ERR_ARG;
    return e->update_stats(ridden, swept, segments);
}
int mb_bert_set_grad_clip(mb_bert_engine* e, float max_norm) {
    if (!e) return MB_ERR_ARG;
    return e->set_grad_clip(max_norm);
}
int mb_bert_grad_clip_stats(mb_bert_engine* e, float* norm, float* coef, void* stream) {
    if (!e) return MB_ERR_ARG;
    return e->grad_clip_stats(norm, coef, (hipStream_t)stream);
}

int mb_bert_train_step(mb_bert_engine* e, const int64_t* input_ids, const float* visual, const float* acoustic,
                       const int64_t* attention_mask, const int64_t* token_type_ids, const float* labels, int B, int L,
                       uint64_t seed, uint64_t step, float* logits, float* loss, float* loss_run, float* m, float* v, float lr,
                       float beta1, float beta2, float eps, float weight_decay, int opt_step, int correct_bias, float grad_scale,
                       float loss_scale, int mode, void* stream) {
    hipStream_t st = (hipStream_t)stream;
    if (!e || !e->P || !e->G || !e->ws) return MB_ERR_ARG;
    const mb_bert_config& c = e->c;
    if (B < 1 || B > c.max_batch || L < 1 || L > c.max_seq) return MB_ERR_SHAPE;
    if (!input_ids || !visual || !acoustic || !attention_mask || !token_type_ids || !labels || !logits || !loss) return MB_ERR_ARG;
    if ((m == nullptr) != (v == nullptr) || (mode != 1 && mode != 2)) return MB_ERR_ARG;
    const int T = B * L;
    char* ws = e->ws;
    e->training = 1;
    CK(prepare_pass(e, T, st));
    return train_step_impl(e, ws, c.visual_dim, c.acoustic_dim, c.num_labels, input_ids, visual, acoustic, attention_mask, token_type_ids,
                           labels, B, L, seed, step, logits, loss, loss_run, m, v, lr, beta1, beta2, eps, weight_decay, opt_step,
                           correct_bias, grad_scale, loss_scale, mode, e->prof, st,
                           [&](int, float* lg, float* ls, float* lr_, float* m_, float* v_, float sc, hipStream_t s) {
                               return enqueue_step(e, B, L, lg, ls, lr_, m_, v_, sc, s);
                           });
}

int mb_bert_train_step_dp(mb_bert_engine* e, const int64_t* input_ids, const float* visual, const float* acoustic,
                          const int64_t* attention_mask, const int64_t* token_type_ids, const float* labels, int B, int L,
                          uint64_t seed, uint64_t step, float* logits, float* loss, float* loss_run, float* m, float* v, float lr,
                          float beta1, float beta2, float eps, float weight_decay, int opt_step, int correct_bias, float grad_scale,
                          float loss_scale, int mode, void* stream, mb_comm* comm) {
    hipStream_t st = (hipStream_t)stream;
    if (e && e->n_classes > 0) return MB_ERR_MODE;
    if (e && e->clip_max > 0.f) return MB_ERR_MODE;
    if (!e || !e->P || !e->G || !e->ws || !comm) return MB_ERR_ARG;
    const mb_bert_config& c = e->c;
    if (B < 1 || B > c.max_batch || L < 1 || L > c.max_seq) return MB_ERR_SHAPE;
    if (!input_ids || !visual || !acoustic || !attention_mask || !token_type_ids || !labels || !logits || !loss) return MB_ERR_ARG;
    if (!m || !v || (mode != 1 && mode != 2)) return MB_ERR_ARG;
    if (!e->grouped) return MB_ERR_MODE;
    char* ws = e->ws;
    const float* lab = (const float*)(ws + e->ws_in_lab);
    return train_step_dp(
        e, input_ids, visual, acoustic, attention_mask, token_type_ids, labels, B, L, seed, step, logits, loss, loss_run, m, v, lr, beta1, beta2,
        eps, weight_decay, opt_step, correct_bias, grad_scale, loss_scale, mode, st, comm,
        [&](int T, hipStream_t s) { return prepare_pass(e, T, s); },
        [&](int l0, int l1, bool first, bool last, float* lg, float* ls, float* lr_, hipStream_t s) {
            float* keep_attn = e->attn_out;
            e->attn_out = nullptr;
            struct Restore { mb_bert_engine* e; float* p; ~Restore() { e->attn_out = p; } } restore{e, keep_attn};
            if (e->head_mask || e->emb_in || e->pos_ids) return (int)MB_ERR_MODE;
            return bert_forward_range(e, (const int64_t*)(ws + e->ws_in_ids), (const float*)(ws + e->ws_in_vis), (const float*)(ws + e->ws_in_aco),
                                      (const int64_t*)(ws + e->ws_in_mask), (const int64_t*)(ws + e->ws_in_seg), lab, B, L, 1, 0, 0, lg, ls, lr_, s,
                                      l0, l1, first, last);
        },
        [&](int stage_begin, int stage_end, float loss_scale_, hipStream_t s) {
            return mb_bert_backward(e, nullptr, lab, loss_scale_, stage_begin, stage_end, s);
        });
}

int mb_bert_stage_forward(mb_bert_engine* e, const int64_t* input_ids, const float* visual, const float* acoustic,
                          const int64_t* attention_mask, const int64_t* token_type_ids, const float* labels, int B, int L,
                          uint64_t seed, uint64_t step, float* logits, float* loss, float* loss_run, int mode, void* stream) {
    hipStream_t st = (hipStream_t)stream;
    if (!e || !e->P || !e->G || !e->ws) return MB_ERR_ARG;
    const mb_bert_config& c = e->c;
    if (B < 1 || B > c.max_batch || L < 1 || L > c.max_seq) return MB_ERR_SHAPE;
    if (!input_ids || !visual || !acoustic || !attention_mask || !token_type_ids || !labels || !logits || !loss) return MB_ERR_ARG;
    if (mode != 1 && mode != 2) return MB_ERR_ARG;
    if (e->head_mask || e->emb_in || e->pos_ids) return MB_ERR_MODE;
    if (e->prof) mode = 2;
    char* ws = e->ws;
    e->training = 1;
    CK(prepare_pass(e, B * L, st));
    PrologueArgs pa = {};
    e->fill_copies(pa, ws, input_ids, visual, acoustic, attention_mask, token_type_ids, labels, B, L, c.visual_dim, c.acoustic_dim, c.num_labels);
    pa.seed = seed; pa.step = step; pa.keys = e->key_state(ws); pa.nsites = e->nsites;
    CK(step_prologue(pa, st));
    float* keep_attn = e->attn_out;
    e->attn_out = nullptr;
    struct Restore { mb_bert_engine* e; float* p; ~Restore() { e->attn_out = p; } } restore{e, keep_attn};
    return e->run_stage_graph(B, L, -1, 0, logits, loss, loss_run, 0.f, mode, st, [&](hipStream_t s) {
        return mb_bert_forward(e, (const int64_t*)(ws + e->ws_in_ids), (const float*)(ws + e->ws_in_vis), (const float*)(ws + e->ws_in_aco),
                               (const int64_t*)(ws + e->ws_in_mask), (const int64_t*)(ws + e->ws_in_seg), (const float*)(ws + e->ws_in_lab), B, L, 1,
                               0, 0, logits, loss, loss_run, s);
    });
}
int mb_bert_stage_backward(mb_bert_engine* e, float loss_scale, int stage, int mode, void* stream) {
    hipStream_t st = (hipStream_t)stream;
    if (!e || !e->G || !e->ran_forward || !e->training) return MB_ERR_ARG;
    if (stage < 0 || stage > e->c.num_layers + 1 || (mode != 1 && mode != 2)) return MB_ERR_ARG;
    if (e->prof) mode = 2;
    if (stage == 0) CK(e->begin_backward_pass(e->G, st));
    const float* lab = (const float*)(e->ws + e->ws_in_lab);
    return e->run_stage_graph(e->B, e->L, stage, e->ow_pass ? 1 : 0, e->logits, nullptr, nullptr, loss_scale, mode, st, [&](hipStream_t s) {
        return mb_bert_backward(e, nullptr, lab, loss_scale, stage, stage + 1, s);
    });
}

const int64_t* mb_bert_staged_input_ids(const mb_bert_engine* e) { return (e && e->ws) ? (const int64_t*)(e->ws + e->ws_in_ids) : nullptr; }

int mb_bert_load_batch(mb_bert_engine* e, const int64_t* input_ids, const float* visual, const float* acoustic,
                       const int64_t* attention_mask, const int64_t* token_type_ids, const float* labels, int B, int L,
                       const void** staged6, void* stream) {
    hipStream_t st = (hipStream_t)stream;
    if (!e || !e->ws || !staged6) return MB_ERR_ARG;
    const mb_bert_config& c = e->c;
    if (B < 1 || B > c.max_batch || L < 1 || L > c.max_seq) return MB_ERR_SHAPE;
    if (!input_ids || !visual || !acoustic || !attention_mask || !token_type_ids) return MB_ERR_ARG;
    const int T = B * L;
    char* ws = e->ws;
    CK(prepare_pass(e, T, st));
    PrologueArgs pa = {};
    e->fill_copies(pa, ws, input_ids, visual, acoustic, attention_mask, token_type_ids, labels, B, L, c.visual_dim, c.acoustic_dim,
                   c.num_labels);
    CK(step_prologue(pa, st));
    e->staged(ws, labels != nullptr, staged6);
    return MB_OK;
}

int mb_bert_graph_stats(const mb_bert_engine* e, size_t* captures, size_t* launches) {
    if (!e) return MB_ERR_ARG;
    if (captures) *captures = e->graph_captures;
    if (launches) *launches = e->graph_launches;
    return MB_OK;
}

int mb_bert_set_profiling(mb_bert_engine* e, int on) {
    if (!e) return MB_ERR_ARG;
    return e->set_profiling(on, e->c.num_layers);
}
int mb_bert_profile_wgrad_us(mb_bert_engine* e, float* avg_us) {
    if (!e || !e->grouped) return MB_ERR_ARG;
    return e->prof_span_us(0, e->c.num_layers, avg_us);
}
int mb_bert_profile_adamw_us(mb_bert_engine* e, float* us) {
    if (!e) return MB_ERR_ARG;
    return e->prof_span_us(2 * e->c.num_layers, 1, us);
}

const void* mb_bert_hidden_state(const mb_bert_engine* e, int i) {
    if (!e || !e->ws || i < 0 || i > e->c.num_layers) return nullptr;
    return e->ws + e->ws_x[i];
}
int mb_bert_set_attention_output(mb_bert_engine* e, float* probs) {
    if (!e) return MB_ERR_ARG;
    e->attn_out = probs;
    return MB_OK;
}
int mb_bert_mark_grads_zero(mb_bert_engine* e, int known_zero) {
    if (!e) return MB_ERR_ARG;
    e->grads_zero = known_zero != 0;
    if (!known_zero) e->stamp_live = e->word_zero = false;
    if (!known_zero) e->frz_dirty = true;
    if (known_zero) e->grads_stale = false;
    return MB_OK;
}
int mb_bert_distrust_word_stamps(mb_bert_engine* e) {
    if (!e) return MB_ERR_ARG;
    e->stamp_live = e->word_zero = false;
    e->frz_dirty = true;
    return MB_OK;
}
size_t mb_bert_word_skip_updates(const mb_bert_engine* e) { return e ? e->skip_updates : 0; }
int mb_bert_materialize_grads(mb_bert_engine* e, void* stream) {
    if (!e) return MB_ERR_ARG;
    return e->materialize_grads(e->G, (hipStream_t)stream);
}
int mb_bert_grads_stale(const mb_bert_engine* e) { return e && e->grads_stale ? 1 : 0; }
int mb_bert_set_head_mask(mb_bert_engine* e, const float* head_mask) {
    if (!e) return MB_ERR_ARG;
    e->head_mask = head_mask;
    return MB_OK;
}
int mb_bert_set_inputs_embeds(mb_bert_engine* e, const float* inputs_embeds) {
    if (!e) return MB_ERR_ARG;
    e->emb_in = inputs_embeds;
    return MB_OK;
}
int mb_bert_set_position_ids(mb_bert_engine* e, const int64_t* position_ids) {
    if (!e) return MB_ERR_ARG;
    e->pos_ids = position_ids;
    return MB_OK;
}
const float* mb_bert_inputs_embeds_grad(const mb_bert_engine* e) {
    if (!e || !e->ws || !e->ran_forward) return nullptr;
    return (const float*)(e->ws + e->ws_dsum);
}
int mb_bert_backward_outputs(mb_bert_engine* e, const void* d_sequence_output, const void* d_pooler_preact, void* stream) {
    hipStream_t st = (hipStream_t)stream;
    if (!e || !e->G || !e->ran_forward) return MB_ERR_ARG;
    CK(e->begin_backward_pass(e->G, st));
    const mb_bert_config& c = e->c;
    const int dt = c.dtype, H = c.hidden_size, B = e->B, L = e->L, T = B * L, NL = c.num_layers;
    char* ws = e->ws;
    const size_t bytes = (size_t)T * H * esize(dt);
    if (d_sequence_output) CK((int)hipMemcpyAsync(ws + e->ws_dxa, d_sequence_output, bytes, hipMemcpyDeviceToDevice, st));
    else CK(zero_fill(ws + e->ws_dxa, bytes, st));
    if (d_pooler_preact) {
        const char* xf = ws + e->ws_x[NL];
        CK(gemm(dt, GEMM_TN, EPI_ACCUM_F32, H, H, B, d_pooler_preact, H, xf, L * H, nullptr, H, nullptr, e->G + e->wp, nullptr, nullptr, 0,
                kNoDrop, 1, 64, st));
        CK(colsum(dt, d_pooler_preact, H, e->G + e->bp, B, H, st, e->acc_of(ws, e->G)));
        CK(gemm(dt, GEMM_NN, EPI_ADD_RES, B, H, H, d_pooler_preact, H, e->W(e->wp), H, ws + e->ws_dxa, L * H, nullptr, nullptr, nullptr,
                ws + e->ws_dxa, L * H, kNoDrop, 1, 64, st));
    }
    return MB_OK;
}

const void* mb_bert_sequence_output(const mb_bert_engine* e) { return e->ws ? e->ws + e->ws_x[e->c.num_layers] : nullptr; }
const float* mb_bert_pooled_output(const mb_bert_engine* e) { return e->ws ? (const float*)(e->ws + e->ws_head_pooled) : nullptr; }

int mb_bert_stage_grad_ranges(const mb_bert_engine* e, int stage, size_t* offs, size_t* lens, int cap) {
    const int NL = e->c.num_layers;
    std::vector<std::pair<size_t, size_t>> r;
    auto span = [&](size_t a, size_t b) { r.push_back({a, b - a}); };
    if (stage == 0) {
        span(e->wp, e->sh_end);
        span(e->wc, e->n_decay);
        span(e->bp, e->mag_bhv);
        span(e->bc, e->n_params);
    } else if (stage <= NL) {
        const int l = NL - stage;
        const LayerOff& o = e->lo[l];
        span(o.wqkv, l + 1 < NL ? e->lo[l + 1].wqkv : e->wp);
        span(o.bqkv, l + 1 < NL ? e->lo[l + 1].bqkv : e->emb_lnw);
    } else if (stage == NL + 1) {
        span(e->word, e->wc);
        span(e->emb_lnw, e->bp);
        span(e->mag_bhv, e->bc);
    } else return -1;
    int n = 0;
    for (auto& p : r) { if (n < cap) { offs[n] = p.first; lens[n] = p.second; } ++n; }
    return n;
}

}
```

bert_multimodal_transformer_amd/csrc/head.hip:

```cpp
#include <algorithm>
#include "kernels.h"

namespace mb {

template <int CH>
__global__ void __launch_bounds__(256) head_fwd_kernel(const float* __restrict__ z, const float* __restrict__ Wc,
                                                       const float* __restrict__ bc, const float* __restrict__ labels,
                                                       float* __restrict__ pooled, float* __restrict__ logits, float* loss,
                                                       float* loss_run, int B, int nl, DropKey drop) {
    drop.resolve();
    constexpr int H = CH * 256;
    __shared__ float lsum[4];
    const int lane = threadIdx.x & 63, wave = threadIdx.x >> 6;
    const int b = blockIdx.x * 4 + wave;
    const bool valid = b < B;
    float mine = 0.f;
    if (valid) {
        f32x4 pd[CH];
#pragma unroll
        for (int c = 0; c < CH; ++c) {
            const int col = (c * 64 + lane) * 4;
            f32x4 t = *(const f32x4*)(z + (size_t)b * H + col);
#pragma unroll
            for (int r = 0; r < 4; ++r) t[r] = tanhf(t[r]);
            *(f32x4*)(pooled + (size_t)b * H + col) = t;
            const uint32_t idx = (uint32_t)b * H + col;
#pragma unroll
            for (int r = 0; r < 4; ++r) pd[c][r] = t[r] * drop_mult(drop, idx + r);
        }
        float mx = -3.0e38f, se = 0.f, tgt = 0.f;
        const int y = (labels && nl > 1) ? (int)labels[b] : -1;
        for (int k = 0; k < nl; ++k) {
            float s = 0.f;
#pragma unroll
            for (int c = 0; c < CH; ++c) {
                const f32x4 w = *(const f32x4*)(Wc + (size_t)k * H + (c * 64 + lane) * 4);
                const f32x4 t = pd[c] * w;
                s += (t[0] + t[1]) + (t[2] + t[3]);
            }
            s = wave_sum(s) + bc[k];
            if (lane == 0) {
                logits[(size_t)b * nl + k] = s;
                if (labels && nl == 1) {
                    const float d = s - labels[b];
                    mine += d * d / (float)B;
                } else if (labels) {
                    const float nm = fmaxf(mx, s);
                    se = se * __expf(mx - nm) + __expf(s - nm);
                    mx = nm;
                    if (k == y) tgt = s;
                }
            }
        }
        if (lane == 0 && labels && nl > 1) mine = (mx + __logf(se) - tgt) / (float)B;
    }
    if (labels == nullptr || (loss == nullptr && loss_run == nullptr)) return;
    if (lane == 0) lsum[wave] = mine;
    __syncthreads();
    if (threadIdx.x == 0) {
        const float t = (lsum[0] + lsum[1]) + (lsum[2] + lsum[3]);
        if (loss) atomicAdd(loss, t);
        if (loss_run) atomicAdd(loss_run, t);
    }
}

template <class T, int CH>
__global__ void __launch_bounds__(256) head_bwd_kernel(const float* __restrict__ dlogits, const float* __restrict__ logits,
                                                       const float* __restrict__ labels, float loss_scale,
                                                       const float* __restrict__ pooled, const float* __restrict__ Wc,
                                                       T* __restrict__ dz, float* dWc, float* dbc, int B, int nl,
                                                       DropKey drop, GradAcc acc, float* dbp, u32x4* __restrict__ zero_p,
                                                       size_t zero_n16, int nb) {
    if ((int)blockIdx.x >= nb) {
        const u32x4 z = {0u, 0u, 0u, 0u};
        for (size_t i = (size_t)(blockIdx.x - nb) * 256 + threadIdx.x; i < zero_n16; i += (size_t)(gridDim.x - nb) * 256) zero_p[i] = z;
        return;
    }
    drop.resolve();
    constexpr int H = CH * 256;
    __shared__ float wsum[4][H];
    __shared__ float bsum[4];
    const int lane = threadIdx.x & 63, wave = threadIdx.x >> 6;
    const int b = blockIdx.x * 4 + wave;
    const bool valid = b < B;
    const int bb = valid ? b : 0;
    f32x4 dpd[CH], pl[CH], dm[CH];
#pragma unroll
    for (int c = 0; c < CH; ++c) {
        const int col = (c * 64 + lane) * 4;
        dpd[c] = f32x4{0.f, 0.f, 0.f, 0.f};
        pl[c] = *(const f32x4*)(pooled + (size_t)bb * H + col);
        const uint32_t idx = (uint32_t)bb * H + col;
#pragma unroll
        for (int r = 0; r < 4; ++r) dm[c][r] = drop_mult(drop, idx + r);
    }
    float lse = 0.f;
    int y = -1;
    if (valid && !dlogits && nl > 1) {
        float mx = -3.0e38f;
        for (int k = 0; k < nl; ++k) mx = fmaxf(mx, logits[(size_t)b * nl + k]);
        float se = 0.f;
        for (int k = 0; k < nl; ++k) se += __expf(logits[(size_t)b * nl + k] - mx);
        lse = mx + __logf(se);
        y = (int)labels[b];
    }
    for (int k = 0; k < nl; ++k) {
        float dl = 0.f;
        if (valid) {
            if (dlogits) dl = dlogits[(size_t)b * nl + k];
            else if (nl == 1) dl = 2.0f * (logits[b] - labels[b]) / (float)B * loss_scale;
            else dl = (__expf(logits[(size_t)b * nl + k] - lse) - (k == y ? 1.0f : 0.0f)) / (float)B * loss_scale;
        }
#pragma unroll
        for (int c = 0; c < CH; ++c) {
            const int col = (c * 64 + lane) * 4;
            dpd[c] += dl * *(const f32x4*)(Wc + (size_t)k * H + col);
            if (dWc) *(f32x4*)(&wsum[wave][col]) = dl * pl[c] * dm[c];
        }
        if (lane == 0) bsum[wave] = dl;
        if (dWc || dbc) {
            __syncthreads();
            if (dWc)
                for (int col = threadIdx.x; col < H; col += 256)
                    grad_add(acc, dWc + (size_t)k * H + col, (wsum[0][col] + wsum[1][col]) + (wsum[2][col] + wsum[3][col]));
            if (dbc && threadIdx.x == 0) grad_add(acc, dbc + k, (bsum[0] + bsum[1]) + (bsum[2] + bsum[3]));
            __syncthreads();
        }
    }
#pragma unroll
    for (int c = 0; c < CH; ++c) {
        const int col = (c * 64 + lane) * 4;
        const f32x4 d = dpd[c] * dm[c] * (1.0f - pl[c] * pl[c]);
        if (valid) store4(dz + (size_t)b * H + col, d);
        if (dbp) *(f32x4*)(&wsum[wave][col]) = d;
    }
    if (dbp) {
        __syncthreads();
        for (int col = threadIdx.x; col < H; col += 256)
            grad_add(acc, dbp + col, (wsum[0][col] + wsum[1][col]) + (wsum[2][col] + wsum[3][col]));
    }
}

int head_forward(const float* z, const float* Wc, const float* bc, const float* labels, float* pooled, float* logits,
                 float* loss, float* loss_run, int B, int H, int nl, DropKey drop, hipStream_t st) {
    if (H != 256 && H != 512 && H != 768 && H != 1024) return MB_ERR_SHAPE;
    if (B <= 0) return MB_OK;
#define MB_HEAD_FWD(CH) hipLaunchKernelGGL((head_fwd_kernel<CH>), dim3((B + 3) / 4), dim3(256), 0, st, z, Wc, bc, labels, pooled, logits, loss, \
                                           loss_run, B, nl, drop)
    switch (H / 256) { case 1: MB_HEAD_FWD(1); break; case 2: MB_HEAD_FWD(2); break; case 3: MB_HEAD_FWD(3); break; default: MB_HEAD_FWD(4); break; }
#undef MB_HEAD_FWD
    return (int)hipGetLastError();
}

int head_backward(int dtype, const float* dlogits, const float* logits, const float* labels, float loss_scale,
                  const float* pooled, const float* Wc, void* dz, float* dWc, float* dbc, int B, int H, int nl,
                  DropKey drop, hipStream_t st, GradAcc acc, float* dbp, void* zero_p, size_t zero_bytes) {
    if (H != 256 && H != 512 && H != 768 && H != 1024) return MB_ERR_SHAPE;
    if (B <= 0) return MB_OK;
    if (!dlogits && !(logits && labels)) return MB_ERR_ARG;
    if (zero_bytes % 16 || ((uintptr_t)zero_p & 15)) return MB_ERR_SHAPE;
    const int nb = (B + 3) / 4;
    const size_t n16 = zero_p ? zero_bytes / 16 : 0;
    const int zb = n16 ? (int)std::min<size_t>((n16 + 1023) / 1024, 512) : 0;
    if (dtype != DT_BF16 && dtype != DT_F32) return MB_ERR_DTYPE;
#define MB_HEAD_BWD(T, CH) hipLaunchKernelGGL((head_bwd_kernel<T, CH>), dim3(nb + zb), dim3(256), 0, st, dlogits, logits, labels, loss_scale, \
                                              pooled, Wc, (T*)dz, dWc, dbc, B, nl, drop, acc, dbp, (u32x4*)zero_p, n16, nb)
#define MB_HEAD_BWD_CH(CH) do { if (dtype == DT_BF16) MB_HEAD_BWD(bf16, CH); else MB_HEAD_BWD(float, CH); } while (0)
    switch (H / 256) { case 1: MB_HEAD_BWD_CH(1); break; case 2: MB_HEAD_BWD_CH(2); break; case 3: MB_HEAD_BWD_CH(3); break; default: MB_HEAD_BWD_CH(4); break; }
#undef MB_HEAD_BWD_CH
#undef MB_HEAD_BWD
    return (int)hipGetLastError();
}

}
```

bert_multimodal_transformer_amd/csrc/kernels.h:

```cpp
#pragma once
#include <cstdio>
#include <cstdlib>
#include "common.h"

namespace mb {

enum {
    MB_OK = 0,
    MB_ERR_SHAPE = 1001,
    MB_ERR_MODE = 1002,
    MB_ERR_DTYPE = 1003,
    MB_ERR_ARG = 1004,
    MB_ERR_COMM = 1005,
};

inline void ck_trace(const char* expr, const char* file, int line, int code) {
    static int on = -1;
    if (on < 0) { const char* v = getenv("MB_CK_TRACE"); on = (v && atoi(v)) ? 1 : 0; }
    if (on) fprintf(stderr, "[magbert] %s:%d: %s -> %d\n", file, line, expr, code);
}

enum { GEMM_NT = 0,
       GEMM_NN = 1,
       GEMM_TN = 2 };

enum { EPI_BIAS = 0,
       EPI_BIAS_GELU = 1,
       EPI_BIAS_DROP_RES = 2,
       EPI_ADD_RES = 3,
       EPI_DGELU = 4,
       EPI_ACCUM_F32 = 5,
       EPI_BIAS_F32 = 6,
       EPI_BIAS_ACT = 7 };

struct AdamArgs {
    float lr, beta1, beta2, eps, weight_decay, step_size;
    float grad_scale;
};

struct GemmArgs {
    const void* A; const void* B;
    int M, N, K, lda, ldb;
    void* C; int ldc;
    int act;
    void* C2;
    float* Cf;
    const float* bias;
    float* colsum;
    const void* R; int ldr;
    float alpha;
    DropKey drop;
    int kchunk;
    int dbg;
    int reg_m, reg_n, tpr_m, tpr_n;
    int overwrite;
    int cvalid;
    unsigned long long* trace;
    int bseg; size_t bseg_stride;
    GradAcc acc;
};
int gemm_trace_fetch(unsigned long long* host_out, int max_blocks);
int gemm_last_kernel(char* out, int cap);

int gemm_launch(int dtype, int layout, int mode, const GemmArgs& a, int splits, int tile, hipStream_t st);

#define MB_MAX_GROUP 8
struct AdamRide {
    float *p, *g, *m, *v;
    bf16* shadow;
    size_t n4;
    const AdamArgs* dyn;
    int blocks;
    int zero_grad;
};
void gemm_log_ride(const AdamRide& r);
struct GroupedGemmArgs {
    GemmArgs g[MB_MAX_GROUP];
    int first[MB_MAX_GROUP + 1];
    int count;
    int chunk;
    AdamRide ride;
};
int gemm_nn_ride_tiles(int dtype, int mode, const GemmArgs& a, int* per_cu);
int gemm_nn_ride_launch(int dtype, int mode, const GemmArgs& a, const AdamRide& ride, hipStream_t st);
int gemm_grouped_tn_ok(int dtype, const GemmArgs* probs, int count, int tile);
int gemm_grouped_tn_launch(int dtype, const GemmArgs* probs, int count, int tile, hipStream_t st, int stages = 0,
                           const AdamRide* ride = nullptr);

int ln_forward(int dtype, const void* x, const float* gamma, const float* beta, float eps, void* y,
               float* mean, float* rstd, int rows, int H, DropKey drop, hipStream_t st,
               Prefetch pf = {nullptr, 0, nullptr});
int ln_backward(int dtype, const void* dy, const void* x, const float* gamma, const float* mean, const float* rstd,
                void* dx, void* dx_drop, float* dgamma, float* dbeta, float* dbias,
                int rows, int H, DropKey drop_out, DropKey drop_in, hipStream_t st);
int grad_fold(GradAcc acc, float* g, size_t begin, size_t end, hipStream_t st);
size_t ln_partials_floats(int rows, int H);
int ln_backward_partials(int dtype, const void* dy, const void* x, const float* gamma, const float* mean, const float* rstd,
                         void* dx, void* dx_drop, float* partials, int* nblk, int rows, int H, DropKey drop_in, hipStream_t st,
                         Prefetch pf = {nullptr, 0, nullptr});
int ln_reduce_partials(const float* partials_a, const float* partials_b, int nblk, int H, float* const* dst6, hipStream_t st, GradAcc acc = {});
#define MB_LN_MAX_LAYERS 32
struct LnReduceDst { float* d[MB_LN_MAX_LAYERS][6]; int nblk[MB_LN_MAX_LAYERS]; };
int ln_reduce_partials_layers(const float* partials_a, const float* partials_b, size_t layer_stride, int layers, int nblk, int H,
                              const LnReduceDst& dst, hipStream_t st, GradAcc acc = {});

int embed_ln_forward(int dtype, const int64_t* ids, const int64_t* seg, const float* word, const float* pos,
                     const float* type, const float* gamma, const float* beta, float eps, void* out,
                     float* mean, float* rstd, int B, int L, int H, DropKey drop, hipStream_t st,
                     const int64_t* pos_ids = nullptr);
int embed_ln_backward(int dtype, const void* dout, const int64_t* ids, const int64_t* seg, const float* word,
                      const float* pos, const float* type, const float* gamma, const float* mean, const float* rstd,
                      float* dsum_ws, float* dword, float* dpos, float* dtype_, float* dgamma, float* dbeta,
                      int B, int L, int H, int pad_id, DropKey drop, hipStream_t st, const int64_t* pos_ids = nullptr, GradAcc acc = {},
                      float* part = nullptr, int* nblk = nullptr,
                      float* part_b = nullptr,
                      int* id_count = nullptr);

int colsum(int dtype, const void* x, int ldx, float* out, int rows, int cols, hipStream_t st, GradAcc acc = {});

int pack_pad(int dtype, const float* src, int cols, void* dst, int cols_pad, int rows, hipStream_t st);
int convert(int dtype, const float* src, void* dst, size_t n, hipStream_t st);
int widen(int dtype, const void* src, float* dst, size_t n, hipStream_t st);

struct MagDims { int T, H, V, A, Vp, Ap; };
int mag_pack_weights(int dtype, const float* W_hv, const float* W_ha, const float* W_v, const float* W_a,
                     void* We, void* Wv, void* Wa, MagDims d, hipStream_t st);
int mag_unpack_wgrads(const float* dWe, const float* dWv, const float* dWa, float* dW_hv, float* dW_ha,
                      float* dW_v, float* dW_a, MagDims d, hipStream_t st);
int mag_gate_forward(int dtype, const void* e, const void* Ze, const void* Zv, const void* Za,
                     const float* b_hv, const float* b_ha, const float* b_v, const float* b_a,
                     const float* gamma, const float* beta, float ln_eps, float beta_shift,
                     void* out, float* mean, float* rstd, MagDims d, DropKey drop, hipStream_t st);
int mag_gate_backward(int dtype, const void* dout, const void* e, const void* Ze, const void* Zv, const void* Za,
                      const float* b_hv, const float* b_ha, const float* b_v, const float* b_a,
                      const float* gamma, const float* mean, const float* rstd, float beta_shift,
                      void* de, void* dZe, void* dZv, void* dZa,
                      float* db_hv, float* db_ha, float* db_v, float* db_a, float* dgamma, float* dbeta,
                      MagDims d, DropKey drop, hipStream_t st, GradAcc acc = {},
                      float* part_a = nullptr, float* part_b = nullptr, int* nblk = nullptr);

int attention_forward(int dtype, const void* qkv, const int64_t* mask, void* ctx, int B, int L, int nh,
                      DropKey drop, hipStream_t st, float* probs = nullptr, const float* head_scale = nullptr,
                      float* stats = nullptr);
int attention_backward(int dtype, const void* qkv, const int64_t* mask, const void* ctx, const void* dctx,
                       void* dqkv, float* dbias, int B, int L, int nh, DropKey drop, hipStream_t st,
                       const float* head_scale = nullptr, GradAcc acc = {},
                       const struct AdamRide* ride = nullptr,
                       float* stats = nullptr);
size_t tiled_stats_floats(int B, int L, int nh);
int attention_tiled_forward(int dtype, const void* qkv, const int64_t* mask, void* ctx, float* stats, int B, int L, int nh,
                            DropKey drop, hipStream_t st, float* probs = nullptr, const float* head_scale = nullptr);
int attention_tiled_backward(int dtype, const void* qkv, const int64_t* mask, const void* ctx, const void* dctx, float* stats,
                             void* dqkv, float* dbias, int B, int L, int nh, DropKey drop, hipStream_t st,
                             const float* head_scale = nullptr, GradAcc acc = {}, const struct AdamRide* ride = nullptr);
int attention_backward_free_slots(int dtype, int L, int nblk, int cus);
int attention_trace_fetch(unsigned long long* host_out, int max_blocks);

int xlnet_attention_forward(int dtype, const void* qkv, const void* kr, const float* r_w_bias, const float* r_r_bias,
                            const float* r_s_bias, const float* seg_embed, const int64_t* seg, const int64_t* mask, void* vec,
                            void* psave, int B, int L, int nh, DropKey drop, hipStream_t st, const float* head_scale = nullptr,
                            const uint8_t* perm = nullptr,
                            int gstream = 0,
                            float* stats = nullptr);
int xlnet_attention_backward(int dtype, const void* qkv, const void* kr, const float* r_w_bias, const float* r_r_bias,
                             const float* r_s_bias, const float* seg_embed, const int64_t* seg, const int64_t* mask,
                             const void* psave, const void* dvec, void* gsave, void* dqkv, void* dkr, float* d_rwb,
                             float* d_rrb, float* d_rsb, float* d_seg, int B, int L, int nh, DropKey drop, hipStream_t st,
                             const float* head_scale = nullptr,
                             GradAcc acc = {},
                             const struct AdamRide* ride_q = nullptr, const struct AdamRide* ride_kv = nullptr,
                             const void* vec = nullptr, const float* stats = nullptr, void* pdsave = nullptr,
                             const uint8_t* perm = nullptr);
int xlnet_attention_backward_free_slots(int dtype, int L, int nblk, int cus);
size_t xlnet_tiled_stats_floats(int B, int L, int nh);
size_t xlnet_tiled_scratch_elems(int B, int L, int nh);
int xlnet_attention_tiled_forward(int dtype, const void* qkv, const void* kr, const float* r_w_bias, const float* r_r_bias,
                                  const float* r_s_bias, const float* seg_embed, const int64_t* seg, const int64_t* mask, void* vec,
                                  float* stats, int B, int L, int nh, DropKey drop, hipStream_t st, const float* head_scale = nullptr,
                                  const uint8_t* perm = nullptr, int gstream = 0, float* probs = nullptr);
int xlnet_attention_tiled_backward(int dtype, const void* qkv, const void* kr, const float* r_w_bias, const float* r_r_bias,
                                   const float* r_s_bias, const float* seg_embed, const int64_t* seg, const int64_t* mask,
                                   const void* vec, const void* dvec, const float* stats, void* gsave, void* pdsave, void* dqkv, void* dkr,
                                   float* d_rwb, float* d_rrb, float* d_rsb, float* d_seg, int B, int L, int nh, DropKey drop,
                                   hipStream_t st, const float* head_scale = nullptr, const uint8_t* perm = nullptr, GradAcc acc = {});
int gather_drop_forward(int dtype, const int64_t* ids, const float* word, void* out, int rows, int H, DropKey drop, hipStream_t st);
int gather_drop_backward(int dtype, const void* dout, const int64_t* ids, float* dword, int rows, int H, DropKey drop, hipStream_t st, GradAcc acc = {});
int add_f32(float* dst, const float* src, size_t n, hipStream_t st);
int drop_rows(int dtype, const void* x, void* y, int rows, int H, DropKey drop, hipStream_t st);
int xlnet_pos_emb(int dtype, void* out, int B, int L, int H, DropKey drop, hipStream_t st);
int last_token_forward(int dtype, const void* x, void* xs, int B, int L, int H, DropKey drop, hipStream_t st);
int last_token_backward(int dtype, const void* dxs, void* dx, int B, int L, int H, DropKey drop, hipStream_t st);
int xlnet_broadcast_row(int dtype, const float* row, void* out, int rows, int H, hipStream_t st);
int xlnet_map_query(int dtype, const float* tm, const void* qg, const void* qkv_h, void* qkv_g, int B, int M, int L, int H, hipStream_t st);
int xlnet_unmap_vec(int dtype, const float* tm, const void* vec, void* vecg, int B, int M, int L, int H, hipStream_t st);

int head_forward(const float* z, const float* Wc, const float* bc, const float* labels, float* pooled,
                 float* logits, float* loss, float* loss_run, int B, int H, int nl, DropKey drop, hipStream_t st);
int head_backward(int dtype, const float* dlogits, const float* logits, const float* labels, float loss_scale,
                  const float* pooled, const float* Wc, void* dz, float* dWc, float* dbc,
                  int B, int H, int nl, DropKey drop, hipStream_t st, GradAcc acc = {}, float* dbp = nullptr,
                  void* zero_p = nullptr, size_t zero_bytes = 0);

int adamw_step(float* p, float* g, float* m, float* v, void* shadow, size_t n, size_t n_decay,
               size_t sh_begin, size_t sh_end, AdamArgs a, int zero_grad, hipStream_t st, const AdamArgs* dyn = nullptr,
               size_t keep_begin = 0, size_t keep_end = 0);
struct WordSkip { const uint32_t* stamp; const uint32_t* state; size_t begin, end; uint32_t row_len; };
#define MB_CLASSES_MAX 32
#define MB_SEGMENTS_MAX 128
#define MB_SWEEP_PIECES_MAX (MB_SEGMENTS_MAX + 2)
#define MB_PIECE_CLEAR 0xff
struct AdamPieces { uint32_t begin4[MB_SWEEP_PIECES_MAX], start4[MB_SWEEP_PIECES_MAX + 1]; uint8_t slot[MB_SWEEP_PIECES_MAX]; int count, clear_first; };
int adamw_sweep(float* p, float* g, float* m, float* v, void* shadow, const AdamPieces& r, size_t sh_begin, size_t sh_end,
                size_t keep_begin, size_t keep_end, const AdamArgs* cls, const WordSkip& skip, hipStream_t st);

unsigned grad_norm_blocks(size_t n);
int grad_sumsq(const float* g, size_t n, double* partial, hipStream_t st);
int grad_sumsq_pieces(const float* g, const AdamPieces& r, double* partial, unsigned* blocks, hipStream_t st);
struct ClipTables { AdamArgs* tab[2]; int count[2]; };
int grad_clip_finalize(const double* partial, unsigned blocks, const float* dyn, float max_norm, float grad_scale, float* out2,
                       const ClipTables& t, hipStream_t st);

#define MB_PROLOGUE_MAX_COPIES 8
struct PrologueArgs {
    const uint32_t* src[MB_PROLOGUE_MAX_COPIES]; uint32_t* dst[MB_PROLOGUE_MAX_COPIES]; uint32_t dwords[MB_PROLOGUE_MAX_COPIES];
    int ncopies;
    uint64_t seed, step;
    uint32_t* keys; int nsites;
    AdamArgs adam[2]; AdamArgs* adam_dst;
    AdamArgs cls[MB_CLASSES_MAX]; AdamArgs* cls_dst; int ncls;
    float clip[2]; float* clip_dst;
    uint32_t* zero_dw;
    struct PackJob { const float* src; void* dst; int rows, cols, pitch, dtype; } pack[2];
    int npack;
    const int64_t* ids; int n_ids; int* id_count;
    uint32_t* stamp; uint32_t* stamp_state; uint32_t stamp_no, stamp_on;
    struct MagPackW { const float* W_hv; const float* W_ha; const float* W_v; const float* W_a; void* We; void* Wv; void* Wa; MagDims d; int dtype; } magw;
    int copy_blocks;
};
static_assert(sizeof(PrologueArgs) <= 2048, "PrologueArgs travels as kernel arguments (4 KB limit)");
int step_prologue(const PrologueArgs& a, hipStream_t st);
#define MB_ZERO_MAX 8
struct ZeroRanges {
    uint32_t* p[MB_ZERO_MAX]; size_t ndw[MB_ZERO_MAX]; int n;
    void add(void* ptr, size_t bytes) { if (bytes && n < MB_ZERO_MAX) { p[n] = (uint32_t*)ptr; ndw[n] = bytes / 4; ++n; } }
    bool full() const { return n >= MB_ZERO_MAX; }
};
int zero_fill(void* p, size_t bytes, hipStream_t st);
int zero_fill_ranges(const ZeroRanges& z, hipStream_t st);

}
```

bert_multimodal_transformer_amd/csrc/rowops.hip:

```cpp
#include <algorithm>
#include "kernels.h"
#include "mag_pack.h"

namespace mb {

template <int CH>
struct RowStat {
    static __device__ __forceinline__ void compute(const f32x4 (&v)[CH], float eps, float& mu, float& rs) {
        constexpr float invH = 1.0f / (CH * 256);
        float s = 0.f;
#pragma unroll
        for (int c = 0; c < CH; ++c) s += (v[c][0] + v[c][1]) + (v[c][2] + v[c][3]);
        mu = wave_sum(s) * invH;
        float q = 0.f;
#pragma unroll
        for (int c = 0; c < CH; ++c) {
#pragma unroll
            for (int r = 0; r < 4; ++r) { const float d = v[c][r] - mu; q += d * d; }
        }
        rs = 1.0f / sqrtf(wave_sum(q) * invH + eps);
    }
};

template <class T, int CH>
__global__ void __launch_bounds__(256) ln_fwd_kernel(const T* __restrict__ x, const float* __restrict__ gamma,
                                                     const float* __restrict__ beta, float eps, T* __restrict__ y,
                                                     float* __restrict__ mean, float* __restrict__ rstd, int rows,
                                                     DropKey drop, Prefetch pf) {
    drop.resolve();
    constexpr int H = CH * 256;
    const int lane = threadIdx.x & 63, wave = threadIdx.x >> 6;
    const int row = blockIdx.x * 4 + wave;
    if (row >= rows) return;
    f32x4 v[CH];
#pragma unroll
    for (int c = 0; c < CH; ++c) v[c] = load4(x + (size_t)row * H + (c * 64 + lane) * 4);
    float mu, rs;
    RowStat<CH>::compute(v, eps, mu, rs);
    f32x4 g[CH], bt[CH];
#pragma unroll
    for (int c = 0; c < CH; ++c) {
        g[c] = *(const f32x4*)(gamma + (c * 64 + lane) * 4);
        bt[c] = *(const f32x4*)(beta + (c * 64 + lane) * 4);
    }
    u32x4 pfv[4];
    prefetch_issue<4>(pf, gamma, pfv);
#pragma unroll
    for (int c = 0; c < CH; ++c) {
        const int col = (c * 64 + lane) * 4;
        f32x4 o = (v[c] - mu) * rs * g[c] + bt[c];
        const uint32_t idx = (uint32_t)row * H + col;
#pragma unroll
        for (int r = 0; r < 4; ++r) o[r] *= drop_mult(drop, idx + r);
        store4(y + (size_t)row * H + col, o);
    }
    if (lane == 0) { mean[row] = mu; rstd[row] = rs; }
    prefetch_retire<4>(pf, pfv);
}

#ifndef MB_LN_RPW
#define MB_LN_RPW 2
#endif
#ifndef MB_LN_NWV
#define MB_LN_NWV 8
#endif
constexpr int LN_RPW = MB_LN_RPW;

template <int CH, int NQ>
__device__ __forceinline__ void block_colsum_atomic(f32x4 (&part)[NQ][CH], float* const (&dst)[NQ], float* lds, GradAcc acc = {nullptr, nullptr}) {
    constexpr int H = CH * 256;
    const int lane = threadIdx.x & 63, wave = threadIdx.x >> 6;
#pragma unroll
    for (int q = 0; q < NQ; ++q)
#pragma unroll
        for (int c = 0; c < CH; ++c) *(f32x4*)(lds + (wave * NQ + q) * H + (c * 64 + lane) * 4) = part[q][c];
    __syncthreads();
    for (int i = threadIdx.x; i < NQ * H; i += 256) {
        const int q = i / H, col = i % H;
        if (dst[q] == nullptr) continue;
        const float s = lds[(0 * NQ + q) * H + col] + lds[(1 * NQ + q) * H + col] + lds[(2 * NQ + q) * H + col] +
                        lds[(3 * NQ + q) * H + col];
        grad_add(acc, dst[q] + col, s);
    }
}

template <class T, int CH, int RPW, bool PARTIAL, int NWV = 4>
__global__ void __launch_bounds__(NWV * 64) ln_bwd_kernel(const T* __restrict__ dy, const T* __restrict__ x,
                                                     const float* __restrict__ gamma, const float* __restrict__ mean,
                                                     const float* __restrict__ rstd, T* __restrict__ dx,
                                                     T* __restrict__ dx_drop, float* dgamma, float* dbeta, float* dbias,
                                                     int rows, DropKey drop_out, DropKey drop_in, Prefetch pf) {
    drop_out.resolve();
    drop_in.resolve();
    constexpr int H = CH * 256;
    constexpr float invH = 1.0f / H;
    constexpr int SL = NWV > 8 ? 8 : NWV;
    __shared__ float lds[SL * 3 * H];
    const int lane = threadIdx.x & 63, wave = threadIdx.x >> 6;
    f32x4 part[3][CH];
#pragma unroll
    for (int q = 0; q < 3; ++q)
#pragma unroll
        for (int c = 0; c < CH; ++c) part[q][c] = f32x4{0.f, 0.f, 0.f, 0.f};
    f32x4 g[CH];
#pragma unroll
    for (int c = 0; c < CH; ++c) g[c] = *(const f32x4*)(gamma + (c * 64 + lane) * 4);
    for (int i = 0; i < RPW; ++i) {
        const int row = (blockIdx.x * NWV + wave) * RPW + i;
        if (row >= rows) break;
        const float mu = mean[row], rs = rstd[row];
        f32x4 dyv[CH], xh[CH];
        float s1 = 0.f, s2 = 0.f;
#pragma unroll
        for (int c = 0; c < CH; ++c) {
            const int col = (c * 64 + lane) * 4;
            dyv[c] = load4(dy + (size_t)row * H + col);
            const uint32_t idx = (uint32_t)row * H + col;
#pragma unroll
            for (int r = 0; r < 4; ++r) dyv[c][r] *= drop_mult(drop_out, idx + r);
            xh[c] = (load4(x + (size_t)row * H + col) - mu) * rs;
            const f32x4 dxh = dyv[c] * g[c];
            s1 += (dxh[0] + dxh[1]) + (dxh[2] + dxh[3]);
            const f32x4 t = dxh * xh[c];
            s2 += (t[0] + t[1]) + (t[2] + t[3]);
        }
        const float m1 = wave_sum(s1) * invH, m2 = wave_sum(s2) * invH;
#pragma unroll
        for (int c = 0; c < CH; ++c) {
            const int col = (c * 64 + lane) * 4;
            f32x4 d = (dyv[c] * g[c] - m1 - xh[c] * m2) * rs;
            store4(dx + (size_t)row * H + col, d);
            part[0][c] += dyv[c] * xh[c];
            part[1][c] += dyv[c];
            if (dx_drop) {
                const uint32_t idx = (uint32_t)row * H + col;
#pragma unroll
                for (int r = 0; r < 4; ++r) d[r] *= drop_mult(drop_in, idx + r);
                store4(dx_drop + (size_t)row * H + col, d);
            }
            part[2][c] += d;
        }
    }
    u32x4 pfv[8];
    prefetch_issue<8>(pf, gamma, pfv);
    if constexpr (PARTIAL) {
        if constexpr (NWV > SL) {
            if (wave >= SL) {
#pragma unroll
                for (int q = 0; q < 3; ++q)
#pragma unroll
                    for (int c = 0; c < CH; ++c) *(f32x4*)(lds + ((wave - SL) * 3 + q) * H + (c * 64 + lane) * 4) = part[q][c];
            }
            __syncthreads();
            if (wave < SL) {
#pragma unroll
                for (int q = 0; q < 3; ++q)
#pragma unroll
                    for (int c = 0; c < CH; ++c) part[q][c] += *(const f32x4*)(lds + (wave * 3 + q) * H + (c * 64 + lane) * 4);
            }
            __syncthreads();
        }
        if (wave < SL) {
#pragma unroll
            for (int q = 0; q < 3; ++q)
#pragma unroll
                for (int c = 0; c < CH; ++c) *(f32x4*)(lds + (wave * 3 + q) * H + (c * 64 + lane) * 4) = part[q][c];
        }
        __syncthreads();
        float* slab = dgamma + (size_t)blockIdx.x * 3 * H;
        for (int i = threadIdx.x; i < 3 * H; i += NWV * 64) {
            const int q = i / H, col = i % H;
            float t = 0.f;
#pragma unroll
            for (int w = 0; w < SL; ++w) t += lds[(w * 3 + q) * H + col];
            slab[i] = t;
        }
    } else {
        float* const dst[3] = {dgamma, dbeta, dbias};
        static_assert(PARTIAL || NWV == 4, "block_colsum_atomic sums four waves");
        block_colsum_atomic<CH, 3>(part, dst, lds);
    }    prefetch_retire<8>(pf, pfv);
}

__global__ void __launch_bounds__(256) ln_reduce_kernel(const float* __restrict__ pa, const float* __restrict__ pb, int nblk,
                                                        int H, float* d0, float* d1, float* d2, float* d3, float* d4,
                                                        float* d5, GradAcc acc) {
    const int q = blockIdx.y;
    const int col = blockIdx.x * 64 + (threadIdx.x & 63);
    const int part = (threadIdx.x >> 6) + 4 * blockIdx.z;
    const int nparts = 4 * gridDim.z;
    __shared__ float red[4][64];
    float* dsts[6] = {d0, d1, d2, d3, d4, d5};
    float* dst = dsts[q];
    const float* src = q < 3 ? pa : pb;
    float s = 0.f;
    if (dst != nullptr && src != nullptr && col < H) {
        const int qq = q % 3;
        for (int b = part; b < nblk; b += nparts) s += src[((size_t)b * 3 + qq) * H + col];
    }
    red[threadIdx.x >> 6][threadIdx.x & 63] = s;
    __syncthreads();
    if ((threadIdx.x >> 6) == 0 && dst != nullptr && src != nullptr && col < H)
        grad_add(acc, dst + col, red[0][threadIdx.x] + red[1][threadIdx.x] + red[2][threadIdx.x] + red[3][threadIdx.x]);
}

__global__ void __launch_bounds__(256) ln_reduce_layers_kernel(const float* __restrict__ pa, const float* __restrict__ pb,
                                                               size_t layer_stride, int nblk_all, int H, LnReduceDst dst, GradAcc acc) {
    const int q = blockIdx.y;
    const int layer = blockIdx.z >> 3;
    const int nblk = dst.nblk[layer] > 0 ? dst.nblk[layer] : nblk_all;
    const int col = (blockIdx.x * 64 + (threadIdx.x & 63)) * 4;
    const int part = (threadIdx.x >> 6) + 4 * (blockIdx.z & 7);
    constexpr int nparts = 32;
    __shared__ f32x4 red[4][64];
    float* out = dst.d[layer][q];
    const float* src = (q < 3 ? pa : pb) + (size_t)layer * layer_stride;
    f32x4 s = {0.f, 0.f, 0.f, 0.f};
    if (out != nullptr && col < H) {
        const int qq = q % 3;
        for (int b = part; b < nblk; b += nparts) s += *(const f32x4*)(src + ((size_t)b * 3 + qq) * H + col);
    }
    red[threadIdx.x >> 6][threadIdx.x & 63] = s;
    __syncthreads();
    if ((threadIdx.x >> 6) == 0 && out != nullptr && col < H) {
        const f32x4 t = red[0][threadIdx.x] + red[1][threadIdx.x] + red[2][threadIdx.x] + red[3][threadIdx.x];
#pragma unroll
        for (int r = 0; r < 4; ++r) grad_add(acc, out + col + r, t[r]);
    }
}

template <class T, int CH>
__global__ void __launch_bounds__(256) embed_fwd_kernel(const int64_t* __restrict__ ids, const int64_t* __restrict__ seg,
                                                        const float* __restrict__ word, const float* __restrict__ pos,
                                                        const float* __restrict__ type, const float* __restrict__ gamma,
                                                        const float* __restrict__ beta, float eps, T* __restrict__ out,
                                                        float* __restrict__ mean, float* __restrict__ rstd, int rows, int L,
                                                        DropKey drop, const int64_t* __restrict__ pos_ids) {
    drop.resolve();
    constexpr int H = CH * 256;
    const int lane = threadIdx.x & 63, wave = threadIdx.x >> 6;
    const int row = blockIdx.x * 4 + wave;
    if (row >= rows) return;
    const size_t id = ids ? (size_t)ids[row] : (size_t)row, sg = (size_t)seg[row], l = pos_ids ? (size_t)pos_ids[row] : (size_t)(row % L);
    f32x4 v[CH];
#pragma unroll
    for (int c = 0; c < CH; ++c) {
        const int col = (c * 64 + lane) * 4;
        v[c] = *(const f32x4*)(word + id * H + col) + *(const f32x4*)(pos + l * H + col) +
               *(const f32x4*)(type + sg * H + col);
    }
    float mu, rs;
    RowStat<CH>::compute(v, eps, mu, rs);
#pragma unroll
    for (int c = 0; c < CH; ++c) {
        const int col = (c * 64 + lane) * 4;
        const f32x4 g = *(const f32x4*)(gamma + col), b = *(const f32x4*)(beta + col);
        f32x4 o = (v[c] - mu) * rs * g + b;
        const uint32_t idx = (uint32_t)row * H + col;
#pragma unroll
        for (int r = 0; r < 4; ++r) o[r] *= drop_mult(drop, idx + r);
        store4(out + (size_t)row * H + col, o);
    }
// ... 121 lines not shown
            gg[c] = *(const f32x4*)(gamma + col);
            const f32x4 dxh = dyv[c] * gg[c];
            s1 += (dxh[0] + dxh[1]) + (dxh[2] + dxh[3]);
            const f32x4 t = dxh * xh[c];
            s2 += (t[0] + t[1]) + (t[2] + t[3]);
        }
        const float m1 = wave_sum(s1) * invH, m2 = wave_sum(s2) * invH;
#pragma unroll
        for (int c = 0; c < CH; ++c) {
            const int col = (c * 64 + lane) * 4;
            const f32x4 d = (dyv[c] * gg[c] - m1 - xh[c] * m2) * rs;
            if (ids == nullptr) *(f32x4*)(dsum_ws + (size_t)row * H + col) = d;
            if (dword != nullptr && (int)id != pad_id) {
                if (uniq) {
                    f32x4* gp = (f32x4*)(dword + id * H + col);
                    *gp = *gp + d;
                } else {
#pragma unroll
                    for (int r = 0; r < 4; ++r) grad_add(acc, dword + id * H + col + r, d[r]);
                }
            }
            part[0][c] += dyv[c] * xh[c];
            part[1][c] += dyv[c];
            part[4][c] += d;
            if (sg == 0) part[2][c] += d;
            else if (sg == 1) part[3][c] += d;
            else {
#pragma unroll
                for (int r = 0; r < 4; ++r) grad_add(acc, dtype_ + sg * H + col + r, d[r]);
            }
        }
        if (id_count != nullptr && ids != nullptr && lane == 0) id_count[id] = 0;
    }
#pragma unroll
    for (int q = 0; q < 5; ++q)
#pragma unroll
        for (int c = 0; c < CH; ++c) *(f32x4*)(lds + (wave * 5 + q) * H + (c * 64 + lane) * 4) = part[q][c];
    __syncthreads();
    float* slab_a = part_a + (size_t)blockIdx.x * 3 * H;
    float* slab_b = part_b + (size_t)blockIdx.x * 3 * H;
    for (int i = threadIdx.x; i < 5 * H; i += 256) {
        const int q = i / H, col = i % H;
        const float t = lds[(0 * 5 + q) * H + col] + lds[(1 * 5 + q) * H + col] + lds[(2 * 5 + q) * H + col] + lds[(3 * 5 + q) * H + col];
        if (q < 3) slab_a[q * H + col] = t;
        else if (q == 3) slab_b[col] = t;
        else grad_add(acc, dpos + (size_t)l * H + col, t);
    }
}

__global__ void __launch_bounds__(256) embed_pos_type_kernel(const float* __restrict__ dsum_ws, const int64_t* __restrict__ seg,
                                                             float* dpos, float* dtype_, int B, int L, int H,
                                                             const int64_t* __restrict__ pos_ids, GradAcc acc) {
    const int l = blockIdx.x;
    {
        const int col = blockIdx.y * 256 + threadIdx.x;
        if (col >= H) return;
        float ap = 0.f, a0 = 0.f, a1 = 0.f;
        for (int b0 = 0; b0 < B; b0 += 8) {
            float d[8];
            int64_t sg[8], pp[8];
#pragma unroll
            for (int u = 0; u < 8; ++u) {
                const int b = b0 + u;
                const bool ok = b < B;
                const int t = (ok ? b : 0) * L + l;
                d[u] = ok ? dsum_ws[(size_t)t * H + col] : 0.f;
                sg[u] = ok ? seg[t] : 0;
                pp[u] = (ok && pos_ids) ? pos_ids[t] : -1;
            }
#pragma unroll
            for (int u = 0; u < 8; ++u) {
                if (pp[u] >= 0) grad_add(acc, dpos + (size_t)pp[u] * H + col, d[u]);
                else ap += d[u];
                if (sg[u] == 0) a0 += d[u];
                else if (sg[u] == 1) a1 += d[u];
                else grad_add(acc, dtype_ + (size_t)sg[u] * H + col, d[u]);
            }
        }
        if (!pos_ids) dpos[(size_t)l * H + col] += ap;
        grad_add(acc, dtype_ + col, a0);
        grad_add(acc, dtype_ + H + col, a1);
    }
}

template <class T>
__global__ void __launch_bounds__(256) colsum_kernel(const T* __restrict__ x, int ldx, float* out, int rows, int cols,
                                                     int rows_per_block, GradAcc gacc) {
    __shared__ f32x4 lds[4][64];
    const int lane = threadIdx.x & 63, wave = threadIdx.x >> 6;
    const int col = (blockIdx.x * 64 + lane) * 4;
    const int r0 = blockIdx.y * rows_per_block, r1 = min(rows, r0 + rows_per_block);
    f32x4 acc = {0.f, 0.f, 0.f, 0.f};
    if (col < cols)
        for (int r = r0 + wave; r < r1; r += 4) acc += load4(x + (size_t)r * ldx + col);
    lds[wave][lane] = acc;
    __syncthreads();
    if (wave == 0 && col < cols) {
        const f32x4 s = lds[0][lane] + lds[1][lane] + lds[2][lane] + lds[3][lane];
#pragma unroll
        for (int r = 0; r < 4; ++r) grad_add(gacc, out + col + r, s[r]);
    }
}

template <class T>
__global__ void pack_pad_kernel(const float* __restrict__ src, int cols, T* __restrict__ dst, int cols_pad, size_t total) {
    const size_t i = (size_t)blockIdx.x * 256 + threadIdx.x;
    if (i >= total) return;
    const size_t r = i / cols_pad;
    const int c = (int)(i % cols_pad);
    dst[i] = from_f<T>(c < cols ? src[r * cols + c] : 0.f);
}

template <class T>
__global__ void convert_kernel(const float* __restrict__ src, T* __restrict__ dst, size_t n4) {
    for (size_t i = (size_t)blockIdx.x * 256 + threadIdx.x; i < n4; i += (size_t)gridDim.x * 256)
        store4(dst + i * 4, *(const f32x4*)(src + i * 4));
}

template <class T>
__global__ void widen_kernel(const T* __restrict__ src, float* __restrict__ dst, size_t n4) {
    for (size_t i = (size_t)blockIdx.x * 256 + threadIdx.x; i < n4; i += (size_t)gridDim.x * 256)
        *(f32x4*)(dst + i * 4) = load4(src + i * 4);
}

#define MB_DISPATCH_T(dtype, ...)                                  \
    if ((dtype) == DT_BF16) { typedef bf16 T; __VA_ARGS__ }        \
    else if ((dtype) == DT_F32) { typedef float T; __VA_ARGS__ }   \
    else return MB_ERR_DTYPE;
#define MB_DISPATCH_CH(H, ...)                                     \
    if ((H) == 768) { constexpr int CH = 3; __VA_ARGS__ }          \
    else if ((H) == 1024) { constexpr int CH = 4; __VA_ARGS__ }    \
    else if ((H) == 512) { constexpr int CH = 2; __VA_ARGS__ }     \
    else if ((H) == 256) { constexpr int CH = 1; __VA_ARGS__ }     \
    else return MB_ERR_SHAPE;

int ln_forward(int dtype, const void* x, const float* gamma, const float* beta, float eps, void* y, float* mean,
               float* rstd, int rows, int H, DropKey drop, hipStream_t st, Prefetch pf) {
    if (rows <= 0) return MB_OK;
    MB_DISPATCH_T(dtype, MB_DISPATCH_CH(H, {
        hipLaunchKernelGGL((ln_fwd_kernel<T, CH>), dim3((rows + 3) / 4), dim3(256), 0, st, (const T*)x, gamma, beta, eps,
                           (T*)y, mean, rstd, rows, drop, pf);
    }))
    return (int)hipGetLastError();
}

int ln_backward(int dtype, const void* dy, const void* x, const float* gamma, const float* mean, const float* rstd,
                void* dx, void* dx_drop, float* dgamma, float* dbeta, float* dbias, int rows, int H, DropKey drop_out,
                DropKey drop_in, hipStream_t st) {
    if (rows <= 0) return MB_OK;
    constexpr int RPW = 4;
    MB_DISPATCH_T(dtype, MB_DISPATCH_CH(H, {
        hipLaunchKernelGGL((ln_bwd_kernel<T, CH, RPW, false>), dim3((rows + 4 * RPW - 1) / (4 * RPW)), dim3(256), 0, st,
                           (const T*)dy, (const T*)x, gamma, mean, rstd, (T*)dx, (T*)dx_drop, dgamma, dbeta, dbias, rows,
                           drop_out, drop_in, Prefetch{nullptr, 0, nullptr});
    }))
    return (int)hipGetLastError();
}

size_t ln_partials_floats(int rows, int H) { return (size_t)((rows + 4 * LN_RPW - 1) / (4 * LN_RPW)) * 3 * H; }

constexpr int LN_NWV = MB_LN_NWV;
int ln_backward_partials(int dtype, const void* dy, const void* x, const float* gamma, const float* mean, const float* rstd,
                         void* dx, void* dx_drop, float* partials, int* nblk, int rows, int H, DropKey drop_in,
                         hipStream_t st, Prefetch pf) {
    if (rows <= 0) { *nblk = 0; return MB_OK; }
    const int nb = (rows + LN_NWV * LN_RPW - 1) / (LN_NWV * LN_RPW);
    *nblk = nb;
    const DropKey nodrop = {0u, 0u, 0u, 1.0f};
    MB_DISPATCH_T(dtype, MB_DISPATCH_CH(H, {
        hipLaunchKernelGGL((ln_bwd_kernel<T, CH, LN_RPW, true, LN_NWV>), dim3(nb), dim3(LN_NWV * 64), 0, st, (const T*)dy, (const T*)x, gamma,
                           mean, rstd, (T*)dx, (T*)dx_drop, partials, (float*)nullptr, (float*)nullptr, rows, nodrop, drop_in, pf);
    }))
    return (int)hipGetLastError();
}

int ln_reduce_partials(const float* pa, const float* pb, int nblk, int H, float* const* d, hipStream_t st, GradAcc acc) {
    if (nblk <= 0) return MB_OK;
    hipLaunchKernelGGL(ln_reduce_kernel, dim3((H + 63) / 64, 6, 8), dim3(256), 0, st, pa, pb, nblk, H, d[0], d[1], d[2], d[3], d[4],
                       d[5], acc);
    return (int)hipGetLastError();
}

int ln_reduce_partials_layers(const float* pa, const float* pb, size_t layer_stride, int layers, int nblk, int H,
                              const LnReduceDst& dst, hipStream_t st, GradAcc acc) {
    if (nblk <= 0 || layers <= 0) return MB_OK;
    if (layers > MB_LN_MAX_LAYERS) return MB_ERR_SHAPE;
    if (H % 4) return MB_ERR_SHAPE;
    hipLaunchKernelGGL(ln_reduce_layers_kernel, dim3((H + 255) / 256, 6, 8 * layers), dim3(256), 0, st, pa, pb, layer_stride, nblk, H, dst, acc);
    return (int)hipGetLastError();
}

int embed_ln_forward(int dtype, const int64_t* ids, const int64_t* seg, const float* word, const float* pos,
                     const float* type, const float* gamma, const float* beta, float eps, void* out, float* mean,
                     float* rstd, int B, int L, int H, DropKey drop, hipStream_t st, const int64_t* pos_ids) {
    const int rows = B * L;
    if (rows <= 0) return MB_OK;
    MB_DISPATCH_T(dtype, MB_DISPATCH_CH(H, {
        hipLaunchKernelGGL((embed_fwd_kernel<T, CH>), dim3((rows + 3) / 4), dim3(256), 0, st, ids, seg, word, pos, type,
                           gamma, beta, eps, (T*)out, mean, rstd, rows, L, drop, pos_ids);
    }))
    return (int)hipGetLastError();
}

int embed_ln_backward(int dtype, const void* dout, const int64_t* ids, const int64_t* seg, const float* word,
                      const float* pos, const float* type, const float* gamma, const float* mean, const float* rstd,
                      float* dsum_ws, float* dword, float* dpos, float* dtype_, float* dgamma, float* dbeta, int B, int L,
                      int H, int pad_id, DropKey drop, hipStream_t st, const int64_t* pos_ids, GradAcc acc, float* part, int* nblk,
                      float* part_b, int* id_count) {
    const int rows = B * L;
    if (nblk) *nblk = (rows + 4 * LN_RPW - 1) / (4 * LN_RPW);
    if (rows <= 0) return MB_OK;
    if (part != nullptr && part_b != nullptr && pos_ids == nullptr) {
        if (nblk) *nblk = L * ((B + 7) / 8);
        MB_DISPATCH_T(dtype, MB_DISPATCH_CH(H, {
            hipLaunchKernelGGL((embed_bwd_fused_kernel<T, CH>), dim3(L * ((B + 7) / 8)), dim3(256), 0, st, (const T*)dout, ids, seg, word,
                               pos, type, gamma, mean, rstd, dsum_ws, dword, dpos, dtype_, part, part_b, B, L, pad_id, drop, acc, id_count);
        }))
        return (int)hipGetLastError();
    }
    if (part != nullptr) {
        MB_DISPATCH_T(dtype, MB_DISPATCH_CH(H, {
            hipLaunchKernelGGL((embed_bwd_kernel<T, CH, LN_RPW, true>), dim3((rows + 4 * LN_RPW - 1) / (4 * LN_RPW)), dim3(256), 0, st,
                               (const T*)dout, ids, seg, word, pos, type, gamma, mean, rstd, dsum_ws, dword, part, (float*)nullptr,
                               rows, L, pad_id, drop, pos_ids, acc, id_count);
        }))
    } else {
    constexpr int RPW = 4;
    MB_DISPATCH_T(dtype, MB_DISPATCH_CH(H, {
        hipLaunchKernelGGL((embed_bwd_kernel<T, CH, RPW, false>), dim3((rows + 4 * RPW - 1) / (4 * RPW)), dim3(256), 0, st,
                           (const T*)dout, ids, seg, word, pos, type, gamma, mean, rstd, dsum_ws, dword, dgamma, dbeta,
                           rows, L, pad_id, drop, pos_ids, acc, id_count);
    }))
    }
    hipLaunchKernelGGL(embed_pos_type_kernel, dim3(L, (H + 255) / 256), dim3(256), 0, st, dsum_ws, seg, dpos, dtype_, B, L, H, pos_ids, acc);
    return (int)hipGetLastError();
}

int colsum(int dtype, const void* x, int ldx, float* out, int rows, int cols, hipStream_t st, GradAcc acc) {
    if (rows <= 0 || cols <= 0) return MB_OK;
    if (cols % 4) return MB_ERR_SHAPE;
    const int cblocks = (cols + 255) / 256;
    int rblocks = (512 + cblocks - 1) / cblocks;
    if (rblocks > (rows + 15) / 16) rblocks = (rows + 15) / 16;
    if (rblocks < 1) rblocks = 1;
    const int rpb = (rows + rblocks - 1) / rblocks;
    rblocks = (rows + rpb - 1) / rpb;
    MB_DISPATCH_T(dtype, {
        hipLaunchKernelGGL((colsum_kernel<T>), dim3(cblocks, rblocks), dim3(256), 0, st, (const T*)x, ldx, out, rows,
                           cols, rpb, acc);
    })
    return (int)hipGetLastError();
}

int pack_pad(int dtype, const float* src, int cols, void* dst, int cols_pad, int rows, hipStream_t st) {
    const size_t total = (size_t)rows * cols_pad;
    if (total == 0) return MB_OK;
    MB_DISPATCH_T(dtype, {
        hipLaunchKernelGGL((pack_pad_kernel<T>), dim3((unsigned)((total + 255) / 256)), dim3(256), 0, st, src, cols,
                           (T*)dst, cols_pad, total);
    })
    return (int)hipGetLastError();
}

int convert(int dtype, const float* src, void* dst, size_t n, hipStream_t st) {
    if (n == 0) return MB_OK;
    if (n % 4) return MB_ERR_SHAPE;
    const size_t n4 = n / 4;
    unsigned grid = (unsigned)((n4 + 255) / 256);
    if (grid > 4096) grid = 4096;
    MB_DISPATCH_T(dtype, { hipLaunchKernelGGL((convert_kernel<T>), dim3(grid), dim3(256), 0, st, src, (T*)dst, n4); })
    return (int)hipGetLastError();
}

int widen(int dtype, const void* src, float* dst, size_t n, hipStream_t st) {
    if (n == 0) return MB_OK;
    if (n % 4) return MB_ERR_SHAPE;
    const size_t n4 = n / 4;
    unsigned grid = (unsigned)((n4 + 255) / 256);
    if (grid > 4096) grid = 4096;
    MB_DISPATCH_T(dtype, { hipLaunchKernelGGL((widen_kernel<T>), dim3(grid), dim3(256), 0, st, (const T*)src, dst, n4); })
    return (int)hipGetLastError();
}


__global__ void __launch_bounds__(256) zero_fill_kernel(const ZeroRanges z) {
    const size_t tid = (size_t)blockIdx.x * 256 + threadIdx.x, nth = (size_t)gridDim.x * 256;
#pragma unroll 1
    for (int r = 0; r < z.n; ++r) {
        uint32_t* __restrict__ p = z.p[r];
        const size_t ndw = z.ndw[r];
        if (((uintptr_t)p & 15) == 0) {
            const size_t n4 = ndw / 4;
            const u32x4 zero = {0u, 0u, 0u, 0u};
            for (size_t i = tid; i < n4; i += nth) ((u32x4*)p)[i] = zero;
            for (size_t i = n4 * 4 + tid; i < ndw; i += nth) p[i] = 0u;
        } else {
            for (size_t i = tid; i < ndw; i += nth) p[i] = 0u;
        }
    }
}
int zero_fill_ranges(const ZeroRanges& z, hipStream_t st) {
    if (z.n < 0 || z.n > MB_ZERO_MAX) return MB_ERR_ARG;
    size_t most = 0;
    ZeroRanges c = {};
    for (int r = 0; r < z.n; ++r) {
        if (z.ndw[r] == 0) continue;
        if (!z.p[r] || ((uintptr_t)z.p[r] & 3)) return MB_ERR_ARG;
        c.p[c.n] = z.p[r]; c.ndw[c.n] = z.ndw[r]; ++c.n;
        if (z.ndw[r] > most) most = z.ndw[r];
    }
    if (c.n == 0) return MB_OK;
    unsigned grid = (unsigned)((most / 4 + 255) / 256);
    if (grid < 1) grid = 1;
    if (grid > 1024) grid = 1024;
    hipLaunchKernelGGL(zero_fill_kernel, dim3(grid), dim3(256), 0, st, c);
    return (int)hipGetLastError();
}
int zero_fill(void* p, size_t bytes, hipStream_t st) {
    if (bytes == 0) return MB_OK;
    if (!p || (bytes & 3)) return MB_ERR_ARG;
    ZeroRanges z = {};
    z.n = 1; z.p[0] = (uint32_t*)p; z.ndw[0] = bytes / 4;
    return zero_fill_ranges(z, st);
}

// ... 145 lines not shown
```

include/magbert_hip.h:

```cpp
#ifndef MAGBERT_HIP_H
#define MAGBERT_HIP_H
#include <stddef.h>
#include <stdint.h>

#ifdef __cplusplus
extern "C" {
#endif

#define MB_DT_F32 0
#define MB_DT_BF16 1

typedef struct { uint32_t k0, k1, thresh; float scale; } mb_dropkey;

const char* mb_error_string(int code);
int mb_version(void);
void mb_make_dropkey(uint64_t seed, uint64_t step, uint32_t site, float p, mb_dropkey* out);


enum { MB_EPI_RELU = 7, MB_EPI_SWISH = 8, MB_EPI_GELU_NEW = 9, MB_EPI_MISH = 10 };
enum { MB_ACT_GELU = 0, MB_ACT_RELU = 1, MB_ACT_SWISH = 2, MB_ACT_GELU_NEW = 3, MB_ACT_MISH = 4 };
int mb_gemm(int dtype, int layout, int epilogue, int M, int N, int K, const void* A, int lda, const void* B, int ldb,
            void* C, int ldc, void* C2, float* Cf, const float* bias, const void* R, int ldr, float alpha,
            const mb_dropkey* drop, int splits, int tile, void* stream);

int mb_debug_gemm_trace(unsigned long long* host_out, int max_blocks);
int mb_debug_attention_trace(unsigned long long* host_out, int max_blocks);

int mb_debug_gemm_ex(int dtype, int layout, int epilogue, int M, int N, int K, const void* A, int lda, const void* B, int ldb,
                     void* C, int ldc, void* C2, float* Cf, const float* bias, const void* R, int ldr, float alpha,
                     const mb_dropkey* drop, int splits, int tile, int bseg, size_t bseg_stride, int cvalid, int overwrite,
                     long long* colsum_shadow, int fold, float* rp, float* rg, float* rm, float* rv, void* rshadow, size_t n4, int blocks,
                     int zero_grad, float lr, float beta1, float beta2, float eps, float weight_decay, int step, int correct_bias,
                     float grad_scale, void* adam_dev, int* ride_tiles, void* stream);
int mb_debug_gemm_grouped_ex(int dtype, int count, const int* M, const int* N, int K, const void* const* dY, const int* ldy,
                             const void* const* X, const int* ldx, float* const* dW, const int* ldw, const int* cvalid,
                             const int* overwrite, int tile, int stages, float* rp, float* rg, float* rm, float* rv, void* rshadow,
                             size_t n4, int blocks, int zero_grad, float lr, float beta1, float beta2, float eps, float weight_decay,
                             int step, int correct_bias, float grad_scale, void* adam_dev, void* stream);
int mb_debug_gemm_last_kernel(char* out, int cap);

int mb_gemm_grouped_wgrad(int dtype, int count, const int* M, const int* N, int K, const void* const* dY, const int* ldy,
                          const void* const* X, const int* ldx, float* const* dW, const int* ldw, int tile, void* stream);

int mb_narrow(int dtype, const float* src, void* dst, size_t n, void* stream);
int mb_widen(int dtype, const void* src, float* dst, size_t n, void* stream);

int mb_layernorm_forward(int dtype, const void* x, const float* gamma, const float* beta, float eps, void* y,
                         float* mean, float* rstd, int rows, int H, const mb_dropkey* drop, void* stream);
int mb_layernorm_backward(int dtype, const void* dy, const void* x, const float* gamma, const float* mean,
                          const float* rstd, void* dx, void* dx_drop, float* dgamma, float* dbeta, float* dbias,
                          int rows, int H, const mb_dropkey* drop_out, const mb_dropkey* drop_in, void* stream);

int mb_embed_forward(int dtype, const int64_t* ids, const int64_t* seg, const float* word, const float* pos,
                     const float* type, const float* gamma, const float* beta, float eps, void* out, float* mean,
                     float* rstd, int B, int L, int H, const mb_dropkey* drop, void* stream);
int mb_embed_backward(int dtype, const void* dout, const int64_t* ids, const int64_t* seg, const float* word,
                      const float* pos, const float* type, const float* gamma, const float* mean, const float* rstd,
                      float* dsum_ws, float* dword, float* dpos, float* dtype_, float* dgamma, float* dbeta, int B, int L,
                      int H, int pad_id, const mb_dropkey* drop, void* stream);

int mb_attention_forward(int dtype, const void* qkv, const int64_t* mask, void* ctx, int B, int L, int nh,
                         const mb_dropkey* drop, void* stream);
int mb_attention_backward(int dtype, const void* qkv, const int64_t* mask, const void* dctx, void* dqkv, int B, int L,
                          int nh, const mb_dropkey* drop, void* stream);
int mb_attention_resident_forward(int dtype, const void* qkv, const int64_t* mask, void* ctx, int B, int L, int nh,
                                  const mb_dropkey* drop, const float* head_scale, float* probs, void* stream);
int mb_attention_resident_backward(int dtype, const void* qkv, const int64_t* mask, const void* dctx, void* dqkv, float* dbias, int B,
                                   int L, int nh, const mb_dropkey* drop, const float* head_scale, void* stream);
size_t mb_attention_tiled_stats_bytes(int B, int L, int nh);
int mb_attention_tiled_forward(int dtype, const void* qkv, const int64_t* mask, void* ctx, float* stats, int B, int L, int nh,
                               const mb_dropkey* drop, const float* head_scale, float* probs, void* stream);
int mb_attention_tiled_backward(int dtype, const void* qkv, const int64_t* mask, const void* ctx, const void* dctx, float* stats,
                                void* dqkv, float* dbias, int B, int L, int nh, const mb_dropkey* drop, const float* head_scale,
                                void* stream);

size_t mb_mag_workspace_bytes(int dtype, int T, int H, int V, int A);
int mb_mag_forward(int dtype, const void* text, const float* visual, const float* acoustic, const float* W_hv,
                   const float* b_hv, const float* W_ha, const float* b_ha, const float* W_v, const float* b_v,
                   const float* W_a, const float* b_a, const float* ln_w, const float* ln_b, float beta_shift,
                   const mb_dropkey* drop, void* out, void* ws, int T, int H, int V, int A, void* stream);
int mb_mag_backward(int dtype, const void* d_out, const void* text, const float* W_hv, const float* b_hv,
                    const float* W_ha, const float* b_ha, const float* W_v, const float* b_v, const float* W_a,
                    const float* b_a, const float* ln_w, float beta_shift, const mb_dropkey* drop, void* ws,
                    void* d_text, float* d_visual, float* d_acoustic, float* dW_hv, float* db_hv, float* dW_ha,
                    float* db_ha, float* dW_v, float* db_v, float* dW_a, float* db_a, float* dln_w, float* dln_b,
                    int T, int H, int V, int A, void* stream);

int mb_adamw_step(float* p, float* g, float* m, float* v, void* shadow, size_t n, size_t n_decay, size_t sh_begin,
                  size_t sh_end, float lr, float beta1, float beta2, float eps, float weight_decay, int step,
                  int correct_bias, float grad_scale, int zero_grad, void* stream);

size_t mb_grad_clip_scratch_bytes(size_t n);
int mb_grad_clip_coef(const float* g, size_t n, float max_norm, float grad_scale, void* scratch, float* out2, void* stream);

typedef struct {
    int vocab_size, hidden_size, num_layers, num_heads, intermediate_size, max_position, type_vocab, num_labels;
    int visual_dim, acoustic_dim, pad_token_id;
    float layer_norm_eps, mag_layer_norm_eps, beta_shift;
    float hidden_dropout, attn_dropout, mag_dropout;
    int dtype;
    int max_batch, max_seq;
    int injection_index;
    int hidden_act;
} mb_bert_config;

typedef struct mb_bert_engine mb_bert_engine;

int mb_bert_create(const mb_bert_config* cfg, mb_bert_engine** out);
void mb_bert_destroy(mb_bert_engine* e);
int mb_bert_num_tensors(const mb_bert_engine* e);
int mb_bert_tensor_info(const mb_bert_engine* e, int i, char* name, int name_cap, size_t* offset, size_t* numel,
                        int* ndim, int64_t* shape4, int* decay);
size_t mb_bert_param_count(const mb_bert_engine* e);
size_t mb_bert_decay_count(const mb_bert_engine* e);
void mb_bert_shadow_range(const mb_bert_engine* e, size_t* begin, size_t* end);
size_t mb_bert_workspace_bytes(const mb_bert_engine* e);
int mb_bert_bind(mb_bert_engine* e, float* params, float* grads, void* shadow, void* workspace, size_t ws_bytes);
int mb_bert_sync_weights(mb_bert_engine* e, void* stream);

int mb_bert_forward(mb_bert_engine* e, const int64_t* input_ids, const float* visual, const float* acoustic,
                    const int64_t* attention_mask, const int64_t* token_type_ids, const float* labels, int B, int L,
                    int training, uint64_t seed, uint64_t step, float* logits, float* loss, float* loss_run,
                    void* stream);
int mb_bert_backward(mb_bert_engine* e, const float* dlogits, const float* labels, float loss_scale, int stage_begin,
                     int stage_end, void* stream);
const void* mb_bert_sequence_output(const mb_bert_engine* e);
const float* mb_bert_pooled_output(const mb_bert_engine* e);
const void* mb_bert_hidden_state(const mb_bert_engine* e, int i);
int mb_bert_set_attention_output(mb_bert_engine* e, float* probs);
int mb_bert_set_head_mask(mb_bert_engine* e, const float* head_mask);
int mb_bert_set_inputs_embeds(mb_bert_engine* e, const float* inputs_embeds);
int mb_bert_set_position_ids(mb_bert_engine* e, const int64_t* position_ids);
const float* mb_bert_inputs_embeds_grad(const mb_bert_engine* e);
int mb_bert_backward_outputs(mb_bert_engine* e, const void* d_sequence_output, const void* d_pooler_preact, void* stream);
int mb_bert_stage_grad_ranges(const mb_bert_engine* e, int stage, size_t* offs, size_t* lens, int cap);

int mb_bert_mark_grads_zero(mb_bert_engine* e, int known_zero);
int mb_bert_distrust_word_stamps(mb_bert_engine* e);
size_t mb_bert_word_skip_updates(const mb_bert_engine* e);
int mb_bert_materialize_grads(mb_bert_engine* e, void* stream);
int mb_bert_grads_stale(const mb_bert_engine* e);

int mb_bert_train_step(mb_bert_engine* e, const int64_t* input_ids, const float* visual, const float* acoustic,
                       const int64_t* attention_mask, const int64_t* token_type_ids, const float* labels, int B, int L,
                       uint64_t seed, uint64_t step, float* logits, float* loss, float* loss_run, float* m, float* v, float lr,
                       float beta1, float beta2, float eps, float weight_decay, int opt_step, int correct_bias, float grad_scale,
                       float loss_scale, int mode, void* stream);
int mb_bert_stage_forward(mb_bert_engine* e, const int64_t* input_ids, const float* visual, const float* acoustic,
                          const int64_t* attention_mask, const int64_t* token_type_ids, const float* labels, int B, int L,
                          uint64_t seed, uint64_t step, float* logits, float* loss, float* loss_run, int mode, void* stream);
int mb_bert_stage_backward(mb_bert_engine* e, float loss_scale, int stage, int mode, void* stream);
const int64_t* mb_bert_staged_input_ids(const mb_bert_engine* e);
int mb_bert_load_batch(mb_bert_engine* e, const int64_t* input_ids, const float* visual, const float* acoustic,
                       const int64_t* attention_mask, const int64_t* token_type_ids, const float* labels, int B, int L,
                       const void** staged6, void* stream);
int mb_bert_graph_stats(const mb_bert_engine* e, size_t* captures, size_t* launches);

#define MB_UPDATE_CLASSES_MAX 32
#define MB_UPDATE_SEGMENTS_MAX 128
int mb_bert_set_update_map(mb_bert_engine* e, int n_classes, int n_segments, const size_t* boundaries, const int* classes);
int mb_bert_set_update_decay(mb_bert_engine* e, int n_segments, const uint8_t* no_decay);
int mb_bert_set_update_values(mb_bert_engine* e, int n_classes, const float* lr, const float* beta1, const float* beta2, const float* eps,
                              const float* weight_decay, const int* correct_bias);
int mb_bert_update_stats(const mb_bert_engine* e, size_t* ridden, size_t* swept, int* segments);
int mb_bert_set_update_frozen(mb_bert_engine* e, int n_segments, const uint8_t* frozen);
int mb_bert_freeze_stats(const mb_bert_engine* e, size_t* frozen_elems, int* wgrad_launches_skipped, int* embed_skipped);

int mb_bert_set_grad_clip(mb_bert_engine* e, float max_norm);
int mb_bert_grad_clip_stats(mb_bert_engine* e, float* norm, float* coef, void* stream);

int mb_bert_set_profiling(mb_bert_engine* e, int on);
int mb_bert_profile_wgrad_us(mb_bert_engine* e, float* avg_us);
int mb_bert_profile_adamw_us(mb_bert_engine* e, float* us);

typedef struct {
    int vocab_size, d_model, n_layer, n_head, d_inner, num_labels;
    int visual_dim, acoustic_dim, injection_index;
    float layer_norm_eps, mag_layer_norm_eps, beta_shift;
    float dropout, summary_last_dropout, mag_dropout;
    int dtype;
    int max_batch, max_seq;
    int ff_activation;
} mb_xlnet_config;

typedef struct mb_xlnet_engine mb_xlnet_engine;

size_t mb_xlnet_attention_tiled_stats_bytes(int B, int L, int nh);
size_t mb_xlnet_attention_tiled_scratch_bytes(int dtype, int B, int L, int nh);
int mb_xlnet_attention_tiled_forward(int dtype, const void* qkv, const void* kr, const float* r_w_bias, const float* r_r_bias,
                                     const float* r_s_bias, const float* seg_embed, const int64_t* seg, const int64_t* mask, void* vec,
                                     float* stats, int B, int L, int nh, const mb_dropkey* drop, const float* head_scale,
                                     const uint8_t* perm, int gstream, float* probs, void* stream);
int mb_xlnet_attention_tiled_backward(int dtype, const void* qkv, const void* kr, const float* r_w_bias, const float* r_r_bias,
                                      const float* r_s_bias, const float* seg_embed, const int64_t* seg, const int64_t* mask,
                                      const void* vec, const void* dvec, const float* stats, void* gsave, void* pdsave, void* dqkv,
                                      void* dkr, float* d_rwb, float* d_rrb, float* d_rsb, float* d_seg, int B, int L, int nh,
                                      const mb_dropkey* drop, const float* head_scale, const uint8_t* perm, void* stream);
int mb_xlnet_attention_forward(int dtype, const void* qkv, const void* kr, const float* r_w_bias, const float* r_r_bias,
                               const float* r_s_bias, const float* seg_embed, const int64_t* seg, const int64_t* mask, void* vec,
                               void* psave, float* stats, int B, int L, int nh, const mb_dropkey* drop, const float* head_scale,
                               const uint8_t* perm, int gstream, void* stream);
int mb_xlnet_attention_backward(int dtype, const void* qkv, const void* kr, const float* r_w_bias, const float* r_r_bias,
                                const float* r_s_bias, const float* seg_embed, const int64_t* seg, const int64_t* mask,
                                const void* psave, const void* vec, const void* dvec, const float* stats, void* gsave, void* pdsave,
                                void* dqkv, void* dkr, float* d_rwb, float* d_rrb, float* d_rsb, float* d_seg, int B, int L, int nh,
                                const mb_dropkey* drop, const float* head_scale, const uint8_t* perm, void* stream);

int mb_xlnet_create(const mb_xlnet_config* cfg, mb_xlnet_engine** out);
void mb_xlnet_destroy(mb_xlnet_engine* e);
int mb_xlnet_num_tensors(const mb_xlnet_engine* e);
int mb_xlnet_tensor_info(const mb_xlnet_engine* e, int i, char* name, int name_cap, size_t* offset, size_t* numel,
                         int* ndim, int64_t* shape4, int* decay);
size_t mb_xlnet_param_count(const mb_xlnet_engine* e);
size_t mb_xlnet_decay_count(const mb_xlnet_engine* e);
void mb_xlnet_shadow_range(const mb_xlnet_engine* e, size_t* begin, size_t* end);
size_t mb_xlnet_workspace_bytes(const mb_xlnet_engine* e);
int mb_xlnet_bind(mb_xlnet_engine* e, float* params, float* grads, void* shadow, void* workspace, size_t ws_bytes);
int mb_xlnet_sync_weights(mb_xlnet_engine* e, void* stream);
int mb_xlnet_forward(mb_xlnet_engine* e, const int64_t* input_ids, const float* visual, const float* acoustic,
                     const int64_t* attention_mask, const int64_t* token_type_ids, const float* labels, int B, int L,
                     int training, uint64_t seed, uint64_t step, float* logits, float* loss, float* loss_run,
                     void* stream);
int mb_xlnet_backward(mb_xlnet_engine* e, const float* dlogits, const float* labels, float loss_scale, int stage_begin,
                      int stage_end, void* stream);
const void* mb_xlnet_sequence_output(const mb_xlnet_engine* e);
const void* mb_xlnet_hidden_state(const mb_xlnet_engine* e, int i);
const void* mb_xlnet_attention_probs(const mb_xlnet_engine* e, int layer, int* padded_len);
int mb_xlnet_attention_probs_into(mb_xlnet_engine* e, int layer, float* out, void* stream);
int mb_xlnet_set_head_mask(mb_xlnet_engine* e, const float* head_mask);
int mb_xlnet_set_perm_mask(mb_xlnet_engine* e, const uint8_t* perm);
size_t mb_xlnet_query_stream_scratch_bytes(const mb_xlnet_engine* e, int B, int M, int L);
size_t mb_xlnet_query_stream_state_bytes(const mb_xlnet_engine* e, int B, int M);
int mb_xlnet_query_stream(mb_xlnet_engine* e, const float* target_mapping, int M, void* scratch, size_t scratch_bytes,
                          float* logits_g, void* stream);
int mb_xlnet_set_mems(mb_xlnet_engine* e, const void* mems, int mlen);
int mb_xlnet_stage_grad_ranges(const mb_xlnet_engine* e, int stage, size_t* offs, size_t* lens, int cap);
int mb_xlnet_mark_grads_zero(mb_xlnet_engine* e, int known_zero);
int mb_xlnet_set_inputs_embeds(mb_xlnet_engine* e, const float* inputs_embeds);
const float* mb_xlnet_inputs_embeds_grad(const mb_xlnet_engine* e);
const void* mb_xlnet_model_output(mb_xlnet_engine* e, void* stream);
int mb_xlnet_backward_outputs(mb_xlnet_engine* e, const void* d_output, void* stream);
int mb_xlnet_set_profiling(mb_xlnet_engine* e, int on);
int mb_xlnet_profile_wgrad_us(mb_xlnet_engine* e, float* avg_us);
int mb_xlnet_profile_adamw_us(mb_xlnet_engine* e, float* us);
int mb_xlnet_materialize_grads(mb_xlnet_engine* e, void* stream);
int mb_xlnet_grads_stale(const mb_xlnet_engine* e);
int mb_xlnet_train_step(mb_xlnet_engine* e, const int64_t* input_ids, const float* visual, const float* acoustic,
                        const int64_t* attention_mask, const int64_t* token_type_ids, const float* labels, int B, int L,
                        uint64_t seed, uint64_t step, float* logits, float* loss, float* loss_run, float* m, float* v, float lr,
                        float beta1, float beta2, float eps, float weight_decay, int opt_step, int correct_bias, float grad_scale,
                        float loss_scale, int mode, void* stream);
int mb_xlnet_load_batch(mb_xlnet_engine* e, const int64_t* input_ids, const float* visual, const float* acoustic,
                        const int64_t* attention_mask, const int64_t* token_type_ids, const float* labels, int B, int L,
                        const void** staged6, void* stream);
int mb_xlnet_graph_stats(const mb_xlnet_engine* e, size_t* captures, size_t* launches);
size_t mb_xlnet_trainable_count(const mb_xlnet_engine* e);
int mb_xlnet_set_update_map(mb_xlnet_engine* e, int n_classes, int n_segments, const size_t* boundaries, const int* classes);
int mb_xlnet_set_update_decay(mb_xlnet_engine* e, int n_segments, const uint8_t* no_decay);
int mb_xlnet_set_update_values(mb_xlnet_engine* e, int n_classes, const float* lr, const float* beta1, const float* beta2, const float* eps,
                               const float* weight_decay, const int* correct_bias);
int mb_xlnet_update_stats(const mb_xlnet_engine* e, size_t* ridden, size_t* swept, int* segments);
int mb_xlnet_set_update_frozen(mb_xlnet_engine* e, int n_segments, const uint8_t* frozen);
int mb_xlnet_freeze_stats(const mb_xlnet_engine* e, size_t* frozen_elems, int* wgrad_launches_skipped, int* embed_skipped);
int mb_xlnet_set_grad_clip(mb_xlnet_engine* e, float max_norm);
int mb_xlnet_grad_clip_stats(mb_xlnet_engine* e, float* norm, float* coef, void* stream);

typedef struct mb_comm mb_comm;
typedef int (*mb_all_reduce_cb)(void* ctx, void* buf, size_t count, int dtype, void* stream);
typedef int (*mb_all_gather_cb)(void* ctx, void* buf, size_t bytes_per_rank, void* stream);
int mb_comm_unique_id(void* id128);
int mb_comm_create_rccl(const void* id128, int rank, int world, mb_comm** out);
int mb_comm_create_callbacks(int rank, int world, mb_all_reduce_cb all_reduce, mb_all_gather_cb all_gather, void* ctx, mb_comm** out);
void mb_comm_destroy(mb_comm* c);
int mb_comm_rank(const mb_comm* c);
int mb_comm_world(const mb_comm* c);
void* mb_comm_stream(const mb_comm* c);
size_t mb_comm_scratch_bytes(int world, int wire_dtype, size_t n_params, int vocab, int hidden, int capacity_rows);
int mb_comm_bind_scratch(mb_comm* c, void* scratch, size_t bytes, int wire_dtype, size_t n_params, int vocab, int hidden, int capacity_rows);
int mb_comm_all_reduce(mb_comm* c, float* buf, size_t count, void* stream);
int mb_comm_exchange_rows(mb_comm* c, float* table, const int64_t* ids, int T, void* stream);
int mb_comm_set_row_exchange(mb_comm* c, int rowwise);
int mb_comm_set_sharding(mb_comm* c, int on);
int mb_comm_sharding(const mb_comm* c);
int mb_comm_join(mb_comm* c, void* stream);
int mb_comm_gather_shards(mb_comm* c, void* base, int elem_bytes, void* stream);
int mb_comm_shard_slices(const mb_comm* c, size_t* begin_end_pairs, int max_pairs);
int mb_comm_set_timing(mb_comm* c, int on);
// ... 19 lines not shown
```

Measured before the change: 15390 samples/s.

## Restrict top-layer backward to CLS rows when only pooled output carries gradient

The loss gradient reaches the last encoder layer only through the CLS token via the pooler, so the top layer's FFN and attention-output backward can run over B rows instead of B*L. The change adds a strided LayerNorm-backward path, row-strided dgrad GEMMs, a gather kernel that packs CLS rows into padded scratch for the weight-gradient GEMMs, and zeroing of the context/residual gradient buffers in head backward. Attention backward and the QKV wgrad still run at full size. It cuts FLOPs and memory traffic in the top layer, at the cost of an extra gather launch, more code paths, and the risk of incorrect gradients if other rows ever carry gradient.

```diff
diff --git a/bert_multimodal_transformer_amd/_lib.py b/bert_multimodal_transformer_amd/_lib.py
--- a/bert_multimodal_transformer_amd/_lib.py
+++ b/bert_multimodal_transformer_amd/_lib.py
@@ -68,6 +68,7 @@
     "mb_widen": (_i, [_i, _vp, _vp, _sz, _vp]),
     "mb_layernorm_forward": (_i, [_i, _vp, _vp, _vp, _f, _vp, _vp, _vp, _i, _i, _dk, _vp]),
     "mb_layernorm_backward": (_i, [_i, _vp, _vp, _vp, _vp, _vp, _vp, _vp, _vp, _vp, _vp, _i, _i, _dk, _dk, _vp]),
+    "mb_layernorm_backward_rows": (_i, [_i, _vp, _vp, _vp, _vp, _vp, _vp, _vp, _vp, C.POINTER(_i), _i, _i, _i, _dk, _dk, _vp]),
     "mb_embed_forward": (_i, [_i, _vp, _vp, _vp, _vp, _vp, _vp, _vp, _f, _vp, _vp, _vp, _i, _i, _i, _dk, _vp]),
     "mb_embed_backward": (_i, [_i, _vp, _vp, _vp, _vp, _vp, _vp, _vp, _vp, _vp, _vp, _vp, _vp, _vp, _vp, _vp, _i, _i, _i,
                                _i, _dk, _vp]),
@@ -142,6 +143,8 @@
     "mb_bert_staged_input_ids": (_vp, [_vp]),
     "mb_bert_load_batch": (_i, [_vp, _vp, _vp, _vp, _vp, _vp, _vp, _i, _i, C.POINTER(_vp), _vp]),
     "mb_bert_graph_stats": (_i, [_vp, C.POINTER(_sz), C.POINTER(_sz)]),
+    "mb_bert_top_cls_stats": (_i, [_vp, C.POINTER(_i)]),
+    "mb_bert_top_scratch": (_i, [_vp, _i, C.POINTER(_sz), C.POINTER(_i)]),
     "mb_bert_set_profiling": (_i, [_vp, _i]),
     "mb_bert_profile_wgrad_us": (_i, [_vp, C.POINTER(_f)]),
     "mb_bert_profile_adamw_us": (_i, [_vp, C.POINTER(_f)]),
diff --git a/bert_multimodal_transformer_amd/csrc/engine.hip b/bert_multimodal_transformer_amd/csrc/engine.hip
--- a/bert_multimodal_transformer_amd/csrc/engine.hip
+++ b/bert_multimodal_transformer_amd/csrc/engine.hip
@@ -31,6 +31,14 @@
     size_t ws_dxa, ws_dxb, ws_dctx, ws_dsum, ws_dz, ws_lnp_a, ws_lnp_b;
     size_t lnp_stride = 0;
     int lnp_nblk = 0;
+    int top_cls = 1;
+    bool cls_grad = false;
+    int top_cls_taken = 0;
+    int top_cls_tile = 12872;
+    int top_cls_short_tile = 64;
+    int top_cls_wq_tile = 64, top_cls_wq_stages = 3;
+    int lnp_nblk_top = 0;
+    size_t ws_cls[6];
     size_t ws_ids, ws_seg, ws_mask, ws_labels;
     size_t ws_bytes;
     float* P = nullptr; float* G = nullptr; char* SH = nullptr; char* ws = nullptr;
@@ -160,6 +168,11 @@
         if (emb > e->lnp_stride) e->lnp_stride = emb;
     }
     e->ws_lnp_a = w.take(e->lnp_stride * 4 * (c.num_layers + 2)); e->ws_lnp_b = w.take(e->lnp_stride * 4 * (c.num_layers + 2));
+    {
+        const size_t Bk = align_up((size_t)c.max_batch, 64);
+        const size_t cols[6] = {(size_t)H, (size_t)I, (size_t)I, (size_t)H, (size_t)H, (size_t)H};
+        for (int k = 0; k < 6; ++k) e->ws_cls[k] = w.take(Bk * cols[k] * es);
+    }
     e->carve_step(w, T, (int)V, (int)A, c.max_batch, c.num_labels, SITE_LAYER0 + 4 * c.num_layers);
     e->idcnt_off = w.take((size_t)c.vocab_size * 4);
     e->idcnt_enable = env_on("MB_EMBED_UNIQUE", true);
@@ -348,6 +361,13 @@
     return ln_backward(dtype, dy, x, gamma, mean, rstd, dx, dx_drop, dgamma, dbeta, dbias, rows, H, dk(drop_out),
                        dk(drop_in), (hipStream_t)stream);
 }
+int mb_layernorm_backward_rows(int dtype, const void* dy, const void* x, const float* gamma, const float* mean, const float* rstd,
+                               void* dx, void* dx_drop, float* partials, int* nblk, int rows, int row_stride, int H,
+                               const mb_dropkey* drop_out, const mb_dropkey* drop_in, void* stream) {
+    if (!dy || !x || !gamma || !mean || !rstd || !dx || !partials || !nblk) return MB_ERR_ARG;
+    return ln_backward_partials(dtype, dy, x, gamma, mean, rstd, dx, dx_drop, partials, nblk, rows, H, dk(drop_in), (hipStream_t)stream,
+                                Prefetch{nullptr, 0, nullptr}, row_stride, dk(drop_out));
+}
 int mb_embed_forward(int dtype, const int64_t* ids, const int64_t* seg, const float* word, const float* pos,
                      const float* type, const float* gamma, const float* beta, float eps, void* out, float* mean,
                      float* rstd, int B, int L, int H, const mb_dropkey* drop, void* stream) {
@@ -473,6 +493,11 @@
     e->ride_params = env_long("MB_ADAMW_RIDE_PARAMS", e->ride_params);
     e->prefetch = env_int("MB_PREFETCH", e->prefetch);
     e->pf_qkv = env_int("MB_PF_QKV", e->pf_qkv);
+    e->top_cls = env_int("MB_TOP_CLS", e->top_cls);
+    e->top_cls_tile = env_int("MB_TOP_CLS_TILE", e->top_cls_tile);
+    e->top_cls_wq_tile = env_int("MB_TOP_CLS_WQ_TILE", e->top_cls_wq_tile) == 64 ? 64 : 128;
+    e->top_cls_wq_stages = env_int("MB_TOP_CLS_WQ_STAGES", e->top_cls_wq_stages);
+    e->top_cls_short_tile = env_int("MB_TOP_CLS_SHORT_TILE", e->top_cls_short_tile) == 64 ? 64 : 128;
     if (e->group_wgrad == 256 && (cfg->dtype != DT_BF16 || cfg->hidden_size % 256 != 0 || cfg->intermediate_size % 256 != 0)) e->group_wgrad = 128;
     e->grouped = (e->group_wgrad == 64 || e->group_wgrad == 128 || e->group_wgrad == 256) && cfg->hidden_size % e->group_wgrad == 0 &&
                  cfg->intermediate_size % e->group_wgrad == 0;
@@ -549,6 +574,7 @@
     const int dt = c.dtype, H = c.hidden_size, I = c.intermediate_size, T = B * L, nh = c.num_heads;
     if (e->emb_in) input_ids = nullptr;
     e->ids = input_ids; e->seg = token_type_ids; e->mask = attention_mask; e->ran_forward = true;
+    if (first) e->cls_grad = false;
     e->B = B; e->L = L; e->training = training; e->seed = seed; e->step = step; e->logits = logits;
     float* P = e->P;
     char* ws = e->ws;
@@ -606,6 +632,77 @@
                               loss, loss_run, stream, 0, e->c.num_layers, true, true);
 }
 
+static int top_backward_cls(mb_bert_engine* e, const GradAcc& acc, bool hd, bool defer_ln, hipStream_t st) {
+    const mb_bert_config& c = e->c;
+    const int dt = c.dtype, H = c.hidden_size, I = c.intermediate_size, B = e->B, L = e->L, T = B * L, nh = c.num_heads, NL = c.num_layers;
+    const int l = NL - 1, par = l & 1;
+    const int Tk = (int)align_up((size_t)T, 64), Bk = (int)align_up((size_t)B, 64);
+    const size_t es = esize(dt);
+    float* P = e->P; float* G = e->G; char* ws = e->ws;
+    const LayerOff& o = e->lo[l];
+    const LayerWs& w = e->lw[l];
+    char* dx = ws + e->ws_dxa;
+    char* dy1 = ws + e->ws_dxb;
+    char* dsA = ws + e->ws_ds[par];
+    char* dzdA = hd ? ws + e->ws_dzd[par] : dsA;
+    char* dsB = ws + e->ws_ds2[par];
+    char* dzdB = hd ? ws + e->ws_dzd2[par] : dsB;
+    char* du = ws + e->ws_du[par];
+    char* dqkv = ws + e->ws_dqkv[par];
+    float* lnp_a = (float*)(ws + e->ws_lnp_a) + (size_t)l * e->lnp_stride;
+    float* lnp_b = (float*)(ws + e->ws_lnp_b) + (size_t)l * e->lnp_stride;
+    const int tile = e->top_cls_tile;
+    int nblk = 0;
+    CK(ln_backward_partials(dt, dx, ws + w.s2, P + o.ln2w, (const float*)(ws + w.st2), (const float*)(ws + w.st2) + T, dsA,
+                            hd ? dzdA : nullptr, lnp_a, &nblk, B, H, e->key(SITE_LAYER0 + 4 * l + 2, c.hidden_dropout), st,
+                            Prefetch{nullptr, 0, nullptr}, L));
+    CK(gemm(dt, GEMM_NN, EPI_DGELU, B, I, H, dzdA, L * H, e->W(o.w2), I, du, L * I, nullptr, G + o.b1, nullptr, ws + w.u, L * I, kNoDrop, 1, 64,
+            st, 0, 0, acc));
+    CK(gemm(dt, GEMM_NN, EPI_ADD_RES, B, H, I, du, L * I, e->W(o.w1), H, dy1, L * H, nullptr, nullptr, nullptr, dsA, L * H, kNoDrop, 1, tile, st));
+    CK(ln_backward_partials(dt, dy1, ws + w.s1, P + o.ln1w, (const float*)(ws + w.st1), (const float*)(ws + w.st1) + T, dsB,
+                            hd ? dzdB : nullptr, lnp_b, &nblk, B, H, e->key(SITE_LAYER0 + 4 * l + 1, c.hidden_dropout), st,
+                            Prefetch{nullptr, 0, nullptr}, L));
+    e->lnp_nblk_top = nblk;
+    if (NL == 1) e->lnp_nblk = nblk;
+    if (!defer_ln) {
+        float* const dst6[6] = {G + o.ln2w, G + o.ln2b, G + o.b2, G + o.ln1w, G + o.ln1b, G + o.bo};
+        CK(ln_reduce_partials(lnp_a, lnp_b, nblk, H, dst6, st, acc));
+    }
+    CK(gemm(dt, GEMM_NN, EPI_ADD_RES, B, H, H, dzdB, L * H, e->W(o.wo), H, ws + e->ws_dctx, L * H, nullptr, nullptr, nullptr, nullptr, 0,
+            kNoDrop, 1, tile, st));
+    CK(attention_backward(dt, ws + w.qkv, e->mask, ws + w.ctx, ws + e->ws_dctx, dqkv, G + o.bqkv, B, L, nh,
+                          e->key(SITE_LAYER0 + 4 * l + 0, c.attn_dropout), st, e->head_mask ? e->head_mask + (size_t)l * nh : nullptr, acc,
+                          nullptr, e->attn_stats(w)));
+    const bool wfrozen = e->skipping() && e->unwritten(o.wqkv, e->layer_end(l));
+    if (wfrozen) ++e->frz_wgrad_skipped;
+    const bool grouped = e->grouped;
+    if (grouped && e->prof) CK((int)hipEventRecord(e->pev[2 * l], st));
+    if (!wfrozen) {
+        char* cdzdA = ws + e->ws_cls[0]; char* cg = ws + e->ws_cls[1]; char* cdu = ws + e->ws_cls[2];
+        char* cy1 = ws + e->ws_cls[3]; char* cdzdB = ws + e->ws_cls[4]; char* cctx = ws + e->ws_cls[5];
+        GatherRows gr = {};
+        gr.rows = B; gr.rows_pad = Bk;
+        gr.add(dzdA, cdzdA, H * es, (size_t)L * H * es); gr.add(ws + w.g, cg, I * es, (size_t)L * I * es);
+        gr.add(du, cdu, I * es, (size_t)L * I * es);     gr.add(ws + w.y1, cy1, H * es, (size_t)L * H * es);
+        gr.add(dzdB, cdzdB, H * es, (size_t)L * H * es); gr.add(ws + w.ctx, cctx, H * es, (size_t)L * H * es);
+        CK(gather_rows(gr, st));
+        GemmArgs wg[4] = {wgrad_args(3 * H, H, Tk, dqkv, 3 * H, ws + e->ws_x[l], H, G + o.wqkv, H),
+                          wgrad_args(H, I, Bk, cdzdA, H, cg, I, G + o.w2, I), wgrad_args(I, H, Bk, cdu, I, cy1, H, G + o.w1, H),
+                          wgrad_args(H, H, Bk, cdzdB, H, cctx, H, G + o.wo, H)};
+        if (grouped) {
+            const int wtile = e->group_wgrad == 64 ? 64 : e->top_cls_short_tile, qtile = e->group_wgrad == 64 ? 64 : e->top_cls_wq_tile;
+            for (GemmArgs& a : wg) a.overwrite = e->ow_pass ? 1 : 0;
+            if (!gemm_grouped_tn_ok(dt, wg + 1, 3, wtile) || !gemm_grouped_tn_ok(dt, wg, 1, qtile)) return MB_ERR_SHAPE;
+            CK(gemm_grouped_tn_launch(dt, wg + 1, 3, wtile, st));
+            CK(gemm_grouped_tn_launch(dt, wg, 1, qtile, st, e->top_cls_wq_stages));
+        } else {
+            for (const GemmArgs& a : wg) CK(wgrad(dt, a.M, a.N, a.K, a.A, a.lda, a.B, a.ldb, a.Cf, a.ldc, st));
+        }
+    }
+    if (grouped && e->prof) CK((int)hipEventRecord(e->pev[2 * l + 1], st));
+    return MB_OK;
+}
+
 int mb_bert_backward(mb_bert_engine* e, const float* dlogits, const float* labels, float loss_scale, int stage_begin,
                      int stage_end, void* stream) {
     hipStream_t st = (hipStream_t)stream;
@@ -644,9 +741,12 @@
     const GradAcc acc = e->acc_of(ws, G);
     for (int stage = stage_begin; stage < stage_end; ++stage) {
         if (stage == 0) {
+            const bool cls = e->top_cls != 0;
             CK(head_backward(dt, dlogits, e->logits, labels, loss_scale, (const float*)(ws + e->ws_head_pooled), P + e->wc,
                              ws + e->ws_dz, G + e->wc, G + e->bc, B, H, c.num_labels, e->key(SITE_HEAD, c.hidden_dropout),
-                             st, acc, G + e->bp, ws + e->ws_dxa, (size_t)T * H * esize(dt)));
+                             st, acc, G + e->bp, ws + e->ws_dxa, (size_t)T * H * esize(dt), cls ? ws + e->ws_dctx : nullptr,
+                             cls ? ws + e->ws_ds2[(NL - 1) & 1] : nullptr));
+            e->cls_grad = cls;
             const char* xf = ws + e->ws_x[NL];
             CK(gemm(dt, GEMM_TN, EPI_ACCUM_F32, H, H, B, ws + e->ws_dz, H, xf, L * H, nullptr, H, nullptr, G + e->wp, nullptr,
                     nullptr, 0, kNoDrop, 1, 64, st));
@@ -669,78 +769,84 @@
             float* lnp_a = (float*)(ws + e->ws_lnp_a) + (size_t)l * e->lnp_stride;
             float* lnp_b = (float*)(ws + e->ws_lnp_b) + (size_t)l * e->lnp_stride;
             const bool defer_ln = e->in_step && !e->stage_mode && NL + 2 <= MB_LN_MAX_LAYERS;
-            CK(ln_backward_partials(dt, dx, ws + w.s2, P + o.ln2w, (const float*)(ws + w.st2), (const float*)(ws + w.st2) + T, dsA,
-                                    hd ? dzdA : nullptr, lnp_a, &nblk, T, H, e->key(SITE_LAYER0 + 4 * l + 2, c.hidden_dropout), st,
-                                    Prefetch{e->prefetch ? e->W(o.w1) : nullptr, (size_t)2 * I * H * (dt == DT_BF16 ? 2 : 4), nullptr}));
-            GemmArgs wg[4] = {wgrad_args(H, I, Tk, dzdA, H, ws + w.g, I, G + o.w2, I),
-                              wgrad_args(I, H, Tk, du, I, ws + w.y1, H, G + o.w1, H),
-                              wgrad_args(H, H, Tk, dzdB, H, ws + w.ctx, H, G + o.wo, H),
-                              wgrad_args(3 * H, H, Tk, dqkv, 3 * H, ws + e->ws_x[l], H, G + o.wqkv, H)};
             const bool grouped = e->grouped;
-            const bool wfrozen = e->skipping() && e->unwritten(o.wqkv, e->layer_end(l));
-            if (wfrozen) ++e->frz_wgrad_skipped;
-            if (grouped)
-                for (GemmArgs& a : wg) a.overwrite = e->ow_pass ? 1 : 0;
             auto dgrad_ride = [&](int mode, int Mo, int No, int Ko, const void* dY, int ldy, const void* Wt, int ldw, void* dX, int ldx, const void* R, int ldr,
                                   float* colsum) -> int {
                 return dgrad_with_riders(dt, mode, Mo, No, Ko, dY, ldy, Wt, ldw, dX, ldx, R, ldr, colsum, kNoDrop, acc, st, grouped && e->ride_m != nullptr,
                                          e->ride_opts, e->cu_count(), [&](size_t budget, int blocks) { return take_ride(l, budget, blocks); });
             };
-            int wtile = e->group_wgrad;
-            if (grouped && wtile == 256 && !gemm_grouped_tn_ok(dt, wg, 4, 256)) wtile = 128;
-            if (grouped && !gemm_grouped_tn_ok(dt, wg, 4, wtile)) return MB_ERR_SHAPE;
-            if (!grouped && !wfrozen) CK(wgrad(dt, H, I, Tk, dzdA, H, ws + w.g, I, G + o.w2, I, st));
-            CK(dgrad_ride(EPI_DGELU, T, I, H, dzdA, H, e->W(o.w2), I, du, I, ws + w.u, I, G + o.b1));
-            if (!grouped && !wfrozen) CK(wgrad(dt, I, H, Tk, du, I, ws + w.y1, H, G + o.w1, H, st));
-            CK(dgrad_ride(EPI_ADD_RES, T, H, I, du, I, e->W(o.w1), H, dy1, H, dsA, H, nullptr));
-            Prefetch pf_attn = {e->prefetch ? e->W(o.wqkv) : nullptr, (size_t)4 * H * H * (dt == DT_BF16 ? 2 : 4), nullptr};
-            if (e->prefetch && e->pf_qkv > 0) {
-                const size_t es = dt == DT_BF16 ? 2 : 4, qb = (size_t)T * 3 * H * es;
-                pf_attn.p2 = ws + w.qkv;
-                pf_attn.bytes2 = (w.ctx - w.qkv) - qb <= 4096 ? (w.ctx - w.qkv) + (size_t)T * H * es : qb;
-                pf_attn.stride2 = (uint32_t)e->pf_qkv;
-            }
-            CK(ln_backward_partials(dt, dy1, ws + w.s1, P + o.ln1w, (const float*)(ws + w.st1), (const float*)(ws + w.st1) + T, dsB,
-                                    hd ? dzdB : nullptr, lnp_b, &nblk, T, H, e->key(SITE_LAYER0 + 4 * l + 1, c.hidden_dropout), st,
-                                    pf_attn));
-            if (!grouped && !wfrozen) CK(wgrad(dt, H, H, Tk, dzdB, H, ws + w.ctx, H, G + o.wo, H, st));
-            e->lnp_nblk = nblk;
-            if (!defer_ln) {
-                float* const dst6[6] = {G + o.ln2w, G + o.ln2b, G + o.b2, G + o.ln1w, G + o.ln1b, G + o.bo};
-                CK(ln_reduce_partials(lnp_a, lnp_b, nblk, H, dst6, st, acc));
-            }
-            CK(gemm(dt, GEMM_NN, EPI_ADD_RES, T, H, H, dzdB, H, e->W(o.wo), H, ws + e->ws_dctx, H, nullptr, nullptr, nullptr,
-                    nullptr, 0, kNoDrop, 1, 0, st));
-            AdamRide ra = {};
-            if (e->ride_opts.attn && grouped && e->ride_m && L <= 128) {
-                int free_slots = attention_backward_free_slots(dt, L, B * nh, e->cu_count());
-                if (e->ride_opts.attn_blocks > 0 && free_slots > 0) free_slots = e->ride_opts.attn_blocks;
-                const int blocks = std::min(free_slots, 2 * e->cu_count()) / 8 * 8;
-                if (blocks >= 8) {
-                    const size_t budget = e->ride_opts.attn_params > 0 ? (size_t)e->ride_opts.attn_params
-                                                                  : (L > 64 ? (size_t)blocks * 20480 : (size_t)1650 * (size_t)T);
-                    ra = take_ride(l, budget / 1024 * 1024, blocks);
+            const bool cls_path = l == NL - 1 && e->top_cls && e->cls_grad;
+            if (l == NL - 1) { e->top_cls_taken = cls_path ? 1 : 0; e->lnp_nblk_top = 0; e->cls_grad = false; }
+            if (cls_path) {
+                CK(top_backward_cls(e, acc, hd, defer_ln, st));
+            } else {
+                CK(ln_backward_partials(dt, dx, ws + w.s2, P + o.ln2w, (const float*)(ws + w.st2), (const float*)(ws + w.st2) + T, dsA,
+                                        hd ? dzdA : nullptr, lnp_a, &nblk, T, H, e->key(SITE_LAYER0 + 4 * l + 2, c.hidden_dropout), st,
+                                        Prefetch{e->prefetch ? e->W(o.w1) : nullptr, (size_t)2 * I * H * (dt == DT_BF16 ? 2 : 4), nullptr}));
+                GemmArgs wg[4] = {wgrad_args(H, I, Tk, dzdA, H, ws + w.g, I, G + o.w2, I),
+                                  wgrad_args(I, H, Tk, du, I, ws + w.y1, H, G + o.w1, H),
+                                  wgrad_args(H, H, Tk, dzdB, H, ws + w.ctx, H, G + o.wo, H),
+                                  wgrad_args(3 * H, H, Tk, dqkv, 3 * H, ws + e->ws_x[l], H, G + o.wqkv, H)};
+                const bool wfrozen = e->skipping() && e->unwritten(o.wqkv, e->layer_end(l));
+                if (wfrozen) ++e->frz_wgrad_skipped;
+                if (grouped)
+                    for (GemmArgs& a : wg) a.overwrite = e->ow_pass ? 1 : 0;
+                int wtile = e->group_wgrad;
+                if (grouped && wtile == 256 && !gemm_grouped_tn_ok(dt, wg, 4, 256)) wtile = 128;
+                if (grouped && !gemm_grouped_tn_ok(dt, wg, 4, wtile)) return MB_ERR_SHAPE;
+                if (!grouped && !wfrozen) CK(wgrad(dt, H, I, Tk, dzdA, H, ws + w.g, I, G + o.w2, I, st));
+                CK(dgrad_ride(EPI_DGELU, T, I, H, dzdA, H, e->W(o.w2), I, du, I, ws + w.u, I, G + o.b1));
+                if (!grouped && !wfrozen) CK(wgrad(dt, I, H, Tk, du, I, ws + w.y1, H, G + o.w1, H, st));
+                CK(dgrad_ride(EPI_ADD_RES, T, H, I, du, I, e->W(o.w1), H, dy1, H, dsA, H, nullptr));
+                Prefetch pf_attn = {e->prefetch ? e->W(o.wqkv) : nullptr, (size_t)4 * H * H * (dt == DT_BF16 ? 2 : 4), nullptr};
+                if (e->prefetch && e->pf_qkv > 0) {
+                    const size_t es = dt == DT_BF16 ? 2 : 4, qb = (size_t)T * 3 * H * es;
+                    pf_attn.p2 = ws + w.qkv;
+                    pf_attn.bytes2 = (w.ctx - w.qkv) - qb <= 4096 ? (w.ctx - w.qkv) + (size_t)T * H * es : qb;
+                    pf_attn.stride2 = (uint32_t)e->pf_qkv;
                 }
-            }
-            CK(attention_backward(dt, ws + w.qkv, e->mask, ws + w.ctx, ws + e->ws_dctx, dqkv, G + o.bqkv, B, L, nh,
-                                  e->key(SITE_LAYER0 + 4 * l + 0, c.attn_dropout), st,
-                                  e->head_mask ? e->head_mask + (size_t)l * nh : nullptr, acc, ra.blocks ? &ra : nullptr,
-                                  e->attn_stats(w)));
-            AdamRide ride = {};
-            if (grouped && !wfrozen) {
-                int tiles = 0;
-                const int bm = wtile == 256 ? 256 : wtile, bn = wtile == 256 ? 128 : wtile;
-                for (const GemmArgs& a : wg) tiles += (a.M / bm) * (a.N / bn);
-                const int slots = e->cu_count() * (wtile == 256 ? 1 : wtile == 128 ? 2 : 0);
-                const size_t budget = e->ride_params > 0 ? (size_t)e->ride_params : std::min((size_t)1000 * (size_t)Tk, (size_t)1100000 + (size_t)590 * (size_t)Tk);
-                ride = take_ride(l, budget, e->ride_blocks > 0 ? e->ride_blocks : (slots - tiles) / 8 * 8);
-            }
-            if (grouped) {
-                if (e->prof) CK((int)hipEventRecord(e->pev[2 * l], st));
-                if (!wfrozen) CK(gemm_grouped_tn_launch(dt, wg, 4, wtile, st, 0, ride.blocks ? &ride : nullptr));
-                if (e->prof) CK((int)hipEventRecord(e->pev[2 * l + 1], st));
-            } else if (!wfrozen) {
-                CK(wgrad(dt, 3 * H, H, Tk, dqkv, 3 * H, ws + e->ws_x[l], H, G + o.wqkv, H, st));
+                CK(ln_backward_partials(dt, dy1, ws + w.s1, P + o.ln1w, (const float*)(ws + w.st1), (const float*)(ws + w.st1) + T, dsB,
+                                        hd ? dzdB : nullptr, lnp_b, &nblk, T, H, e->key(SITE_LAYER0 + 4 * l + 1, c.hidden_dropout), st,
+                                        pf_attn));
+                if (!grouped && !wfrozen) CK(wgrad(dt, H, H, Tk, dzdB, H, ws + w.ctx, H, G + o.wo, H, st));
+                e->lnp_nblk = nblk;
+                if (!defer_ln) {
+                    float* const dst6[6] = {G + o.ln2w, G + o.ln2b, G + o.b2, G + o.ln1w, G + o.ln1b, G + o.bo};
+                    CK(ln_reduce_partials(lnp_a, lnp_b, nblk, H, dst6, st, acc));
+                }
+                CK(gemm(dt, GEMM_NN, EPI_ADD_RES, T, H, H, dzdB, H, e->W(o.wo), H, ws + e->ws_dctx, H, nullptr, nullptr, nullptr,
+                        nullptr, 0, kNoDrop, 1, 0, st));
+                AdamRide ra = {};
+                if (e->ride_opts.attn && grouped && e->ride_m && L <= 128) {
+                    int free_slots = attention_backward_free_slots(dt, L, B * nh, e->cu_count());
+                    if (e->ride_opts.attn_blocks > 0 && free_slots > 0) free_slots = e->ride_opts.attn_blocks;
+                    const int blocks = std::min(free_slots, 2 * e->cu_count()) / 8 * 8;
+                    if (blocks >= 8) {
+                        const size_t budget = e->ride_opts.attn_params > 0 ? (size_t)e->ride_opts.attn_params
+                                                                      : (L > 64 ? (size_t)blocks * 20480 : (size_t)1650 * (size_t)T);
+                        ra = take_ride(l, budget / 1024 * 1024, blocks);
+                    }
+                }
+                CK(attention_backward(dt, ws + w.qkv, e->mask, ws + w.ctx, ws + e->ws_dctx, dqkv, G + o.bqkv, B, L, nh,
+                                      e->key(SITE_LAYER0 + 4 * l + 0, c.attn_dropout), st,
+                                      e->head_mask ? e->head_mask + (size_t)l * nh : nullptr, acc, ra.blocks ? &ra : nullptr,
+                                      e->attn_stats(w)));
+                AdamRide ride = {};
+                if (grouped && !wfrozen) {
+                    int tiles = 0;
+                    const int bm = wtile == 256 ? 256 : wtile, bn = wtile == 256 ? 128 : wtile;
+                    for (const GemmArgs& a : wg) tiles += (a.M / bm) * (a.N / bn);
+                    const int slots = e->cu_count() * (wtile == 256 ? 1 : wtile == 128 ? 2 : 0);
+                    const size_t budget = e->ride_params > 0 ? (size_t)e->ride_params : std::min((size_t)1000 * (size_t)Tk, (size_t)1100000 + (size_t)590 * (size_t)Tk);
+                    ride = take_ride(l, budget, e->ride_blocks > 0 ? e->ride_blocks : (slots - tiles) / 8 * 8);
+                }
+                if (grouped) {
+                    if (e->prof) CK((int)hipEventRecord(e->pev[2 * l], st));
+                    if (!wfrozen) CK(gemm_grouped_tn_launch(dt, wg, 4, wtile, st, 0, ride.blocks ? &ride : nullptr));
+                    if (e->prof) CK((int)hipEventRecord(e->pev[2 * l + 1], st));
+                } else if (!wfrozen) {
+                    CK(wgrad(dt, 3 * H, H, Tk, dqkv, 3 * H, ws + e->ws_x[l], H, G + o.wqkv, H, st));
+                }
             }
             CK(dgrad_ride(EPI_ADD_RES, T, H, 3 * H, dqkv, 3 * H, e->W(o.wqkv), H, dx, H, dsB, H, nullptr));
             if (l == c.injection_index && l >= 1) {
@@ -795,6 +901,7 @@
                 float* const m6[6] = {G + e->mag_bhv, G + e->mag_bha, G + e->mag_bv, G + e->mag_ba, G + e->mag_lnw, G + e->mag_lnb};
                 if (mag_here || defer_ln) for (int q = 0; q < 6; ++q) dst.d[NL - first][q] = m6[q];
                 dst.nblk[NL - first] = mblk; dst.nblk[NL + 1 - first] = eblk;
+                if (defer_ln && e->lnp_nblk_top > 0) dst.nblk[NL - 1] = e->lnp_nblk_top;
                 if (!emb_frozen) { dst.d[NL + 1 - first][0] = G + e->emb_lnw; dst.d[NL + 1 - first][1] = G + e->emb_lnb; }
                 if (e->pos_ids == nullptr && !emb_frozen) {
                     dst.d[NL + 1 - first][2] = G + e->type; dst.d[NL + 1 - first][3] = G + e->type + H;
@@ -952,6 +1059,7 @@
     float* keep_attn = e->attn_out;
     e->attn_out = nullptr;
     struct Restore { mb_bert_engine* e; float* p; ~Restore() { e->attn_out = p; } } restore{e, keep_attn};
+    e->cls_grad = false;
     return e->run_stage_graph(B, L, -1, 0, logits, loss, loss_run, 0.f, mode, st, [&](hipStream_t s) {
         return mb_bert_forward(e, (const int64_t*)(ws + e->ws_in_ids), (const float*)(ws + e->ws_in_vis), (const float*)(ws + e->ws_in_aco),
                                (const int64_t*)(ws + e->ws_in_mask), (const int64_t*)(ws + e->ws_in_seg), (const float*)(ws + e->ws_in_lab), B, L, 1,
@@ -965,9 +1073,12 @@
     if (e->prof) mode = 2;
     if (stage == 0) CK(e->begin_backward_pass(e->G, st));
     const float* lab = (const float*)(e->ws + e->ws_in_lab);
-    return e->run_stage_graph(e->B, e->L, stage, e->ow_pass ? 1 : 0, e->logits, nullptr, nullptr, loss_scale, mode, st, [&](hipStream_t s) {
-        return mb_bert_backward(e, nullptr, lab, loss_scale, stage, stage + 1, s);
-    });
+    const bool cls = stage == 1 && e->top_cls && e->cls_grad;
+    const int rc = e->run_stage_graph(e->B, e->L, stage, (e->ow_pass ? 1 : 0) | (cls ? 2 : 0), e->logits, nullptr, nullptr, loss_scale, mode, st,
+                                      [&](hipStream_t s) { return mb_bert_backward(e, nullptr, lab, loss_scale, stage, stage + 1, s); });
+    e->cls_grad = rc == MB_OK && stage == 0 && e->top_cls;
+    if (stage == 1) e->top_cls_taken = cls ? 1 : 0;
+    return rc;
 }
 
 const int64_t* mb_bert_staged_input_ids(const mb_bert_engine* e) { return (e && e->ws) ? (const int64_t*)(e->ws + e->ws_in_ids) : nullptr; }
@@ -998,6 +1109,20 @@
     return MB_OK;
 }
 
+int mb_bert_top_cls_stats(const mb_bert_engine* e, int* taken) {
+    if (!e || !taken) return MB_ERR_ARG;
+    *taken = e->top_cls_taken;
+    return MB_OK;
+}
+int mb_bert_top_scratch(const mb_bert_engine* e, int which, size_t* offset, int* cols) {
+    if (!e || !offset || !cols || which < 0 || which > 6) return MB_ERR_ARG;
+    const int par = (e->c.num_layers - 1) & 1, H = e->c.hidden_size;
+    const size_t off[7] = {e->ws_ds[par], e->ws_dzd[par], e->ws_du[par], e->ws_dxb, e->ws_ds2[par], e->ws_dzd2[par], e->ws_dctx};
+    *offset = off[which];
+    *cols = which == 2 ? e->c.intermediate_size : H;
+    return MB_OK;
+}
+
 int mb_bert_set_profiling(mb_bert_engine* e, int on) {
     if (!e) return MB_ERR_ARG;
     return e->set_profiling(on, e->c.num_layers);
@@ -1063,6 +1188,7 @@
     hipStream_t st = (hipStream_t)stream;
     if (!e || !e->G || !e->ran_forward) return MB_ERR_ARG;
     CK(e->begin_backward_pass(e->G, st));
+    e->cls_grad = false; e->top_cls_taken = 0;
     const mb_bert_config& c = e->c;
     const int dt = c.dtype, H = c.hidden_size, B = e->B, L = e->L, T = B * L, NL = c.num_layers;
     char* ws = e->ws;
diff --git a/bert_multimodal_transformer_amd/csrc/head.hip b/bert_multimodal_transformer_amd/csrc/head.hip
--- a/bert_multimodal_transformer_amd/csrc/head.hip
+++ b/bert_multimodal_transformer_amd/csrc/head.hip
@@ -70,10 +70,14 @@
                                                        const float* __restrict__ pooled, const float* __restrict__ Wc,
                                                        T* __restrict__ dz, float* dWc, float* dbc, int B, int nl,
                                                        DropKey drop, GradAcc acc, float* dbp, u32x4* __restrict__ zero_p,
-                                                       size_t zero_n16, int nb) {
+                                                       size_t zero_n16, int nb, u32x4* __restrict__ zero_p2, u32x4* __restrict__ zero_p3) {
     if ((int)blockIdx.x >= nb) {
         const u32x4 z = {0u, 0u, 0u, 0u};
-        for (size_t i = (size_t)(blockIdx.x - nb) * 256 + threadIdx.x; i < zero_n16; i += (size_t)(gridDim.x - nb) * 256) zero_p[i] = z;
+        for (size_t i = (size_t)(blockIdx.x - nb) * 256 + threadIdx.x; i < zero_n16; i += (size_t)(gridDim.x - nb) * 256) {
+            zero_p[i] = z;
+            if (zero_p2) zero_p2[i] = z;
+            if (zero_p3) zero_p3[i] = z;
+        }
         return;
     }
     drop.resolve();
@@ -154,17 +158,20 @@
 
 int head_backward(int dtype, const float* dlogits, const float* logits, const float* labels, float loss_scale,
                   const float* pooled, const float* Wc, void* dz, float* dWc, float* dbc, int B, int H, int nl,
-                  DropKey drop, hipStream_t st, GradAcc acc, float* dbp, void* zero_p, size_t zero_bytes) {
+                  DropKey drop, hipStream_t st, GradAcc acc, float* dbp, void* zero_p, size_t zero_bytes, void* zero_p2, void* zero_p3) {
     if (H != 256 && H != 512 && H != 768 && H != 1024) return MB_ERR_SHAPE;
     if (B <= 0) return MB_OK;
     if (!dlogits && !(logits && labels)) return MB_ERR_ARG;
-    if (zero_bytes % 16 || ((uintptr_t)zero_p & 15)) return MB_ERR_SHAPE;
+    if (zero_bytes % 16 || (((uintptr_t)zero_p | (uintptr_t)zero_p2 | (uintptr_t)zero_p3) & 15)) return MB_ERR_SHAPE;
+    if (!zero_p && (zero_p2 || zero_p3)) return MB_ERR_ARG;
     const int nb = (B + 3) / 4;
     const size_t n16 = zero_p ? zero_bytes / 16 : 0;
-    const int zb = n16 ? (int)std::min<size_t>((n16 + 1023) / 1024, 512) : 0;
+    const size_t nbuf = 1 + (zero_p2 ? 1 : 0) + (zero_p3 ? 1 : 0);
+    const int zb = n16 ? (int)std::min<size_t>((n16 * nbuf + 1023) / 1024, 512) : 0;
     if (dtype != DT_BF16 && dtype != DT_F32) return MB_ERR_DTYPE;
 #define MB_HEAD_BWD(T, CH) hipLaunchKernelGGL((head_bwd_kernel<T, CH>), dim3(nb + zb), dim3(256), 0, st, dlogits, logits, labels, loss_scale, \
-                                              pooled, Wc, (T*)dz, dWc, dbc, B, nl, drop, acc, dbp, (u32x4*)zero_p, n16, nb)
+                                              pooled, Wc, (T*)dz, dWc, dbc, B, nl, drop, acc, dbp, (u32x4*)zero_p, n16, nb, \
+                                              (u32x4*)zero_p2, (u32x4*)zero_p3)
 #define MB_HEAD_BWD_CH(CH) do { if (dtype == DT_BF16) MB_HEAD_BWD(bf16, CH); else MB_HEAD_BWD(float, CH); } while (0)
     switch (H / 256) { case 1: MB_HEAD_BWD_CH(1); break; case 2: MB_HEAD_BWD_CH(2); break; case 3: MB_HEAD_BWD_CH(3); break; default: MB_HEAD_BWD_CH(4); break; }
 #undef MB_HEAD_BWD_CH
diff --git a/bert_multimodal_transformer_amd/csrc/kernels.h b/bert_multimodal_transformer_amd/csrc/kernels.h
--- a/bert_multimodal_transformer_amd/csrc/kernels.h
+++ b/bert_multimodal_transformer_amd/csrc/kernels.h
@@ -97,7 +97,17 @@
 size_t ln_partials_floats(int rows, int H);
 int ln_backward_partials(int dtype, const void* dy, const void* x, const float* gamma, const float* mean, const float* rstd,
                          void* dx, void* dx_drop, float* partials, int* nblk, int rows, int H, DropKey drop_in, hipStream_t st,
-                         Prefetch pf = {nullptr, 0, nullptr});
+                         Prefetch pf = {nullptr, 0, nullptr},
+                         int row_stride = 1, DropKey drop_out = {0u, 0u, 0u, 1.0f});
+#define MB_GATHER_MAX 8
+struct GatherRows {
+    struct Job { const void* src; void* dst; uint32_t n16; size_t src_stride16; } job[MB_GATHER_MAX];
+    int n, rows, rows_pad;
+    void add(const void* src, void* dst, size_t row_bytes, size_t src_stride_bytes) {
+        if (n < MB_GATHER_MAX) { job[n] = Job{src, dst, (uint32_t)(row_bytes / 16), src_stride_bytes / 16}; ++n; }
+    }
+};
+int gather_rows(const GatherRows& g, hipStream_t st);
 int ln_reduce_partials(const float* partials_a, const float* partials_b, int nblk, int H, float* const* dst6, hipStream_t st, GradAcc acc = {});
 #define MB_LN_MAX_LAYERS 32
 struct LnReduceDst { float* d[MB_LN_MAX_LAYERS][6]; int nblk[MB_LN_MAX_LAYERS]; };
@@ -199,7 +209,8 @@
 int head_backward(int dtype, const float* dlogits, const float* logits, const float* labels, float loss_scale,
                   const float* pooled, const float* Wc, void* dz, float* dWc, float* dbc,
                   int B, int H, int nl, DropKey drop, hipStream_t st, GradAcc acc = {}, float* dbp = nullptr,
-                  void* zero_p = nullptr, size_t zero_bytes = 0);
+                  void* zero_p = nullptr, size_t zero_bytes = 0,
+                  void* zero_p2 = nullptr, void* zero_p3 = nullptr);
 
 int adamw_step(float* p, float* g, float* m, float* v, void* shadow, size_t n, size_t n_decay,
                size_t sh_begin, size_t sh_end, AdamArgs a, int zero_grad, hipStream_t st, const AdamArgs* dyn = nullptr,
diff --git a/bert_multimodal_transformer_amd/csrc/rowops.hip b/bert_multimodal_transformer_amd/csrc/rowops.hip
--- a/bert_multimodal_transformer_amd/csrc/rowops.hip
+++ b/bert_multimodal_transformer_amd/csrc/rowops.hip
@@ -84,12 +84,12 @@
     }
 }
 
-template <class T, int CH, int RPW, bool PARTIAL, int NWV = 4>
+template <class T, int CH, int RPW, bool PARTIAL, int NWV = 4, bool STRIDED = false>
 __global__ void __launch_bounds__(NWV * 64) ln_bwd_kernel(const T* __restrict__ dy, const T* __restrict__ x,
                                                      const float* __restrict__ gamma, const float* __restrict__ mean,
                                                      const float* __restrict__ rstd, T* __restrict__ dx,
                                                      T* __restrict__ dx_drop, float* dgamma, float* dbeta, float* dbias,
-                                                     int rows, DropKey drop_out, DropKey drop_in, Prefetch pf) {
+                                                     int rows, DropKey drop_out, DropKey drop_in, Prefetch pf, int rstride) {
     drop_out.resolve();
     drop_in.resolve();
     constexpr int H = CH * 256;
@@ -106,8 +106,9 @@
 #pragma unroll
     for (int c = 0; c < CH; ++c) g[c] = *(const f32x4*)(gamma + (c * 64 + lane) * 4);
     for (int i = 0; i < RPW; ++i) {
-        const int row = (blockIdx.x * NWV + wave) * RPW + i;
-        if (row >= rows) break;
+        const int lrow = (blockIdx.x * NWV + wave) * RPW + i;
+        if (lrow >= rows) break;
+        const int row = STRIDED ? lrow * rstride : lrow;
         const float mu = mean[row], rs = rstd[row];
         f32x4 dyv[CH], xh[CH];
         float s1 = 0.f, s2 = 0.f;
@@ -535,7 +536,7 @@
     MB_DISPATCH_T(dtype, MB_DISPATCH_CH(H, {
         hipLaunchKernelGGL((ln_bwd_kernel<T, CH, RPW, false>), dim3((rows + 4 * RPW - 1) / (4 * RPW)), dim3(256), 0, st,
                            (const T*)dy, (const T*)x, gamma, mean, rstd, (T*)dx, (T*)dx_drop, dgamma, dbeta, dbias, rows,
-                           drop_out, drop_in, Prefetch{nullptr, 0, nullptr});
+                           drop_out, drop_in, Prefetch{nullptr, 0, nullptr}, 1);
     }))
     return (int)hipGetLastError();
 }
@@ -545,15 +546,41 @@
 constexpr int LN_NWV = MB_LN_NWV;
 int ln_backward_partials(int dtype, const void* dy, const void* x, const float* gamma, const float* mean, const float* rstd,
                          void* dx, void* dx_drop, float* partials, int* nblk, int rows, int H, DropKey drop_in,
-                         hipStream_t st, Prefetch pf) {
+                         hipStream_t st, Prefetch pf, int row_stride, DropKey drop_out) {
     if (rows <= 0) { *nblk = 0; return MB_OK; }
+    if (row_stride < 1 || (size_t)rows * (size_t)row_stride * (size_t)H > 0xffffffffull) return MB_ERR_SHAPE;
     const int nb = (rows + LN_NWV * LN_RPW - 1) / (LN_NWV * LN_RPW);
     *nblk = nb;
-    const DropKey nodrop = {0u, 0u, 0u, 1.0f};
+    if (row_stride > 1) {
+        MB_DISPATCH_T(dtype, MB_DISPATCH_CH(H, {
+            hipLaunchKernelGGL((ln_bwd_kernel<T, CH, LN_RPW, true, LN_NWV, true>), dim3(nb), dim3(LN_NWV * 64), 0, st, (const T*)dy, (const T*)x,
+                               gamma, mean, rstd, (T*)dx, (T*)dx_drop, partials, (float*)nullptr, (float*)nullptr, rows, drop_out, drop_in, pf,
+                               row_stride);
+        }))
+        return (int)hipGetLastError();
+    }
     MB_DISPATCH_T(dtype, MB_DISPATCH_CH(H, {
         hipLaunchKernelGGL((ln_bwd_kernel<T, CH, LN_RPW, true, LN_NWV>), dim3(nb), dim3(LN_NWV * 64), 0, st, (const T*)dy, (const T*)x, gamma,
-                           mean, rstd, (T*)dx, (T*)dx_drop, partials, (float*)nullptr, (float*)nullptr, rows, nodrop, drop_in, pf);
+                           mean, rstd, (T*)dx, (T*)dx_drop, partials, (float*)nullptr, (float*)nullptr, rows, drop_out, drop_in, pf, 1);
     }))
+    return (int)hipGetLastError();
+}
+
+__global__ void __launch_bounds__(256) gather_rows_kernel(const GatherRows g) {
+    const GatherRows::Job& j = g.job[blockIdx.y];
+    const int r = blockIdx.x;
+    const u32x4* __restrict__ src = (const u32x4*)j.src + (size_t)r * j.src_stride16;
+    u32x4* __restrict__ dst = (u32x4*)j.dst + (size_t)r * j.n16;
+    const u32x4 zero = {0u, 0u, 0u, 0u};
+    const bool live = r < g.rows;
+    for (uint32_t i = threadIdx.x; i < j.n16; i += 256) dst[i] = live ? src[i] : zero;
+}
+int gather_rows(const GatherRows& g, hipStream_t st) {
+    if (g.n < 1 || g.n > MB_GATHER_MAX || g.rows < 0 || g.rows_pad < g.rows) return MB_ERR_ARG;
+    if (g.rows_pad == 0) return MB_OK;
+    for (int k = 0; k < g.n; ++k)
+        if (!g.job[k].src || !g.job[k].dst || (((uintptr_t)g.job[k].src | (uintptr_t)g.job[k].dst) & 15)) return MB_ERR_ARG;
+    hipLaunchKernelGGL(gather_rows_kernel, dim3(g.rows_pad, g.n), dim3(256), 0, st, g);
     return (int)hipGetLastError();
 }
 
diff --git a/include/magbert_hip.h b/include/magbert_hip.h
--- a/include/magbert_hip.h
+++ b/include/magbert_hip.h
@@ -50,6 +50,9 @@
 int mb_layernorm_backward(int dtype, const void* dy, const void* x, const float* gamma, const float* mean,
                           const float* rstd, void* dx, void* dx_drop, float* dgamma, float* dbeta, float* dbias,
                           int rows, int H, const mb_dropkey* drop_out, const mb_dropkey* drop_in, void* stream);
+int mb_layernorm_backward_rows(int dtype, const void* dy, const void* x, const float* gamma, const float* mean, const float* rstd,
+                               void* dx, void* dx_drop, float* partials, int* nblk, int rows, int row_stride, int H,
+                               const mb_dropkey* drop_out, const mb_dropkey* drop_in, void* stream);
 
 int mb_embed_forward(int dtype, const int64_t* ids, const int64_t* seg, const float* word, const float* pos,
                      const float* type, const float* gamma, const float* beta, float eps, void* out, float* mean,
@@ -133,6 +136,8 @@
 int mb_bert_set_position_ids(mb_bert_engine* e, const int64_t* position_ids);
 const float* mb_bert_inputs_embeds_grad(const mb_bert_engine* e);
 int mb_bert_backward_outputs(mb_bert_engine* e, const void* d_sequence_output, const void* d_pooler_preact, void* stream);
+int mb_bert_top_cls_stats(const mb_bert_engine* e, int* taken);
+int mb_bert_top_scratch(const mb_bert_engine* e, int which, size_t* offset, int* cols);
 int mb_bert_stage_grad_ranges(const mb_bert_engine* e, int stage, size_t* offs, size_t* lens, int cap);
 
 int mb_bert_mark_grads_zero(mb_bert_engine* e, int known_zero);
```

Result: no change. 15480 samples/s, median of 6 (+0.6%).
